# AlejandroSilvestri/os1

Measured on AMD Instinct MI355X. Metric: frames/sec extract+match, 1920x1080 @ 2000 ORB feats, higher is better.
Workload: dtype u8

## Files before the change

include/orbfe.h:

```cpp
#ifndef ORBFE_H_
#define ORBFE_H_

#include <stddef.h>
#include <stdint.h>

#ifdef __cplusplus
extern "C" {
#endif

#define ORBFE_OK 0
#define ORBFE_ERR_INVALID (-1)
#define ORBFE_ERR_NO_DEVICE (-2)
#define ORBFE_ERR_HIP (-3)
#define ORBFE_ERR_TOO_SMALL (-4)
#define ORBFE_ERR_OVERFLOW (-5)

typedef struct OrbfeKeyPoint {
  float x, y;
  float size;
  float angle;
  float response;
  int32_t octave;
  int32_t class_id;
} OrbfeKeyPoint;

typedef struct orbfe_extractor orbfe_extractor;
typedef struct orbfe_matcher orbfe_matcher;
typedef struct orbfe_vocabulary orbfe_vocabulary;
typedef struct orbfe_kfdb orbfe_kfdb;

const char* orbfe_last_error(void);
int orbfe_device_count(void);

int orbfe_device_malloc(int device_id, size_t bytes, void** out);
int orbfe_device_free(int device_id, void* ptr);
int orbfe_device_upload(int device_id, void* dst_device, const void* src_host, size_t bytes);
int orbfe_device_synchronize(int device_id);
int orbfe_host_alloc(size_t bytes, void** out);
int orbfe_host_free(void* ptr);
int orbfe_host_register(void* ptr, size_t bytes);
int orbfe_host_unregister(void* ptr);
int orbfe_device_numa_node(int device_id);
int orbfe_bind_thread_to_device(int device_id);
int orbfe_debug_h2d_rate(int device_id, const void* host, size_t bytes, int reps, double* gb_per_s);


int orbfe_extractor_create(int nfeatures, float scaleFactor, int nlevels, int iniThFAST, int minThFAST,
                           int device_id, orbfe_extractor** out);
void orbfe_extractor_destroy(orbfe_extractor* h);

int orbfe_extractor_levels(const orbfe_extractor* h);
int orbfe_extractor_device(const orbfe_extractor* h);
float orbfe_extractor_scale_factor(const orbfe_extractor* h);
int orbfe_extractor_scale_tables(const orbfe_extractor* h, float* scale, float* inv_scale, float* sigma2,
                                 float* inv_sigma2);
int orbfe_extractor_features_per_level(const orbfe_extractor* h, int32_t* out);
int orbfe_extractor_max_keypoints(const orbfe_extractor* h);
int orbfe_extractor_max_keypoints_for_size(const orbfe_extractor* h, int rows, int cols);

int orbfe_extractor_set_wait_mode(orbfe_extractor* h, int poll_us);

enum { ORBFE_INPUT_GRAY8 = 0, ORBFE_INPUT_RGB8 = 1, ORBFE_INPUT_BGR8 = 2, ORBFE_INPUT_RGBA8 = 3, ORBFE_INPUT_BGRA8 = 4 };
enum { ORBFE_GRAY_Q15 = 0, ORBFE_GRAY_Q14 = 1 };
int orbfe_extractor_set_input_format(orbfe_extractor* h, int format, int gray_variant);

enum { ORBFE_GAUSS_ED = 0, ORBFE_GAUSS_ROUNDED = 1 };
int orbfe_extractor_set_blur_variant(orbfe_extractor* h, int variant);

int orbfe_extract(orbfe_extractor* h, const uint8_t* gray, int rows, int cols, size_t stride_bytes,
                  OrbfeKeyPoint* kps, uint8_t* desc, int cap, int* n_out);

int orbfe_extract_batch(orbfe_extractor* h, int nframes, const uint8_t* const* gray, int in_device_memory,
                        int rows, int cols, size_t stride_bytes, OrbfeKeyPoint* kps, uint8_t* desc, int cap,
                        int* n_out);

int orbfe_extract_batch_submit(orbfe_extractor* h, int nframes, const uint8_t* const* gray, int in_device_memory,
                               int rows, int cols, size_t stride_bytes);
int orbfe_extract_batch_collect(orbfe_extractor* h, OrbfeKeyPoint* kps, uint8_t* desc, int cap, int* n_out);
int orbfe_extract_batch_wait(orbfe_extractor* h);

typedef struct orbfe_sfi_chain orbfe_sfi_chain;
int orbfe_sfi_chain_create(const orbfe_extractor* h, orbfe_sfi_chain** out);
void orbfe_sfi_chain_destroy(orbfe_sfi_chain* c);
int orbfe_sfi_chain_set_isolated(orbfe_sfi_chain* c, int isolated);
int orbfe_sfi_chain_restart(orbfe_sfi_chain* c);
int orbfe_extract_batch_submit_matched(orbfe_extractor* h, orbfe_sfi_chain* chain, int nframes, const uint8_t* const* gray,
                                       int in_device_memory, int rows, int cols, size_t stride_bytes, const float bounds[4],
                                       int window_size, float nnratio, int check_orientation);
int orbfe_extract_batch_collect_matched(orbfe_extractor* h, OrbfeKeyPoint* kps, uint8_t* desc, int cap, int* n_out,
                                        int32_t* matches12, int* nmatches);

int orbfe_debug_level_size(const orbfe_extractor* h, int level, int* w, int* hgt);
int orbfe_debug_level_copy(orbfe_extractor* h, int frame, int level, uint8_t* out );
int orbfe_debug_candidates(orbfe_extractor* h, int frame, int level, int32_t* xys, int cap, int* n_out);
int orbfe_debug_stage_ms(const orbfe_extractor* h, float out[5]);
int orbfe_debug_kernel_ms(orbfe_extractor* h, double out_ms[5], long long* batches, long long* frames, int reset);
int orbfe_debug_set_profiling(orbfe_extractor* h, int enable);
int orbfe_debug_fast_stamps(orbfe_extractor* h, unsigned long long out[8], int reset);
int orbfe_debug_sfi_records(orbfe_extractor* h, int32_t* out, int cap_records, int* n_out, int reset);
int orbfe_debug_sincos(orbfe_extractor* h, const float* angle_deg, int n, float* cos_out, float* sin_out);

int orbfe_debug_quadtree(const int16_t* x, const int16_t* y, const uint8_t* score, int n, int min_x, int max_x,
                         int min_y, int max_y, int n_target, int32_t* out_idx, int cap, int* n_out);
int orbfe_debug_sincos_host_check(uint32_t lo_bits, uint32_t hi_bits, uint32_t step, long long* mismatches);
int orbfe_debug_logf(orbfe_matcher* m, const float* x, int n, float* out);
int orbfe_debug_logf_host_check(uint32_t lo_bits, uint32_t hi_bits, uint32_t step, long long* mismatches);

typedef struct orbfe_stream orbfe_stream;
int orbfe_stream_create(int nfeatures, float scaleFactor, int nlevels, int iniThFAST, int minThFAST, int device_id,
                        int batch, int depth, orbfe_stream** out);
void orbfe_stream_destroy(orbfe_stream* s);
int orbfe_stream_set_matching(orbfe_stream* s, const float bounds[4], int window_size, float nnratio,
                              int check_orientation);
int orbfe_stream_set_isolated_batches(orbfe_stream* s, int isolated);
int orbfe_stream_batches_in_flight(const orbfe_stream* s);
int orbfe_stream_pop_hold(orbfe_stream* s, const OrbfeKeyPoint** kps, const uint8_t** desc, const int** n_kps, const int32_t** matches12,
                          const int** nmatches, int* ticket);
int orbfe_stream_release(orbfe_stream* s, int ticket);
int orbfe_stream_set_input_format(orbfe_stream* s, int format, int gray_variant);
int orbfe_stream_set_blur_variant(orbfe_stream* s, int variant);
int orbfe_stream_set_vocabulary(orbfe_stream* s, orbfe_vocabulary* v, int levelsup);
int orbfe_stream_bow_raw(orbfe_stream* s, int frame, const uint32_t** leaf_node, const uint32_t** level_node, int* n);
int orbfe_stream_capacity(const orbfe_stream* s);
int orbfe_stream_set_queue_slots(orbfe_stream* s, int nslots);
int orbfe_stream_queue_slots(const orbfe_stream* s);
int orbfe_stream_push(orbfe_stream* s, const uint8_t* const* gray, int in_device_memory, int rows, int cols,
                      size_t stride_bytes);
int orbfe_stream_pop(orbfe_stream* s, const OrbfeKeyPoint** kps, const uint8_t** desc, const int** n_kps,
                     const int32_t** matches12, const int** nmatches);
int orbfe_stream_stats(orbfe_stream* s, double out[4], int reset);
int orbfe_stream_kernel_ms(orbfe_stream* s, double out_ms[5], long long* batches, long long* frames, int reset);


int orbfe_hamming(const uint8_t a[32], const uint8_t b[32]);

int orbfe_matcher_create(int device_id, orbfe_matcher** out);
void orbfe_matcher_destroy(orbfe_matcher* m);
int orbfe_matcher_device(const orbfe_matcher* m);
int orbfe_matcher_upload_async(orbfe_matcher* m, void* dst_device, const void* src_host, size_t bytes);
int orbfe_matcher_synchronize(orbfe_matcher* m);

int orbfe_search_for_initialization(orbfe_matcher* m, const OrbfeKeyPoint* kps1, const uint8_t* desc1, int n1,
                                    const OrbfeKeyPoint* kps2, const uint8_t* desc2, int n2,
                                    const float bounds[4], float* prev_xy, int32_t* matches12, int window_size,
                                    float nnratio, int check_orientation, int* nmatches);

int orbfe_search_for_initialization_batch(orbfe_matcher* m, int npairs, const OrbfeKeyPoint* const* kps1,
                                          const uint8_t* const* desc1, const int* n1,
                                          const OrbfeKeyPoint* const* kps2, const uint8_t* const* desc2,
                                          const int* n2, const float bounds[4], float* const* prev_xy,
                                          int32_t* const* matches12, int window_size, float nnratio,
                                          int check_orientation, int* nmatches);

#define ORBFE_MP_IN_VIEW 1u
#define ORBFE_MP_BAD 2u
#define ORBFE_MP_CANDIDATO 4u
#define ORBFE_MP_OBSERVED 8u

int orbfe_search_by_projection(orbfe_matcher* m, const OrbfeKeyPoint* kps_un, const uint8_t* desc, int n,
                               const float bounds[4], const float* scale_factors, int nlevels,
                               const uint8_t* kp_occupied, const float* mp_proj_xy, const int32_t* mp_level,
                               const float* mp_viewcos, const uint8_t* mp_flags, const uint8_t* mp_desc, int n_mp,
                               float th, float nnratio, int32_t* kp_assigned, int* nmatches);

int orbfe_search_by_projection_uv(orbfe_matcher* m, const OrbfeKeyPoint* kps_un, const uint8_t* desc, int n,
                                  const float bounds[4], const float* scale_factors, int nlevels,
                                  const uint8_t* kp_occupied, const float* src_uv, const int32_t* src_level,
                                  const float* src_angle, const uint8_t* src_flags, const uint8_t* src_valid,
                                  const uint8_t* src_desc, int n_src, float th, int max_dist,
                                  int skip_any_occupied, int check_orientation, int32_t* kp_assigned,
                                  int* nmatches);

int orbfe_debug_matcher_ms(const orbfe_matcher* m, double out[3]);

int orbfe_window_candidates(orbfe_matcher* m, const OrbfeKeyPoint* kps_un, const uint8_t* desc, int n,
                            const float bounds[4], int nq, const float* qx, const float* qy, const float* qr,
                            const int32_t* qmin_level, const int32_t* qmax_level, const uint8_t* qdesc,
                            uint32_t* counts, uint32_t* offsets, uint32_t* pool, size_t pool_cap, size_t* pool_used);

int orbfe_search_projected(orbfe_matcher* m, const OrbfeKeyPoint* kps_un, const uint8_t* desc, int n, const float bounds[4],
                           int n_src, const float* src_uv, const float* src_radius, const int32_t* src_level,
                           const uint8_t* src_valid, const uint8_t* src_desc, const uint8_t* kp_skip, int claim,
                           const float* inv_level_sigma2, int nlevels, double chi2, int max_dist, int32_t* best_idx,
                           int32_t* best_dist, int* nmatches);

typedef struct orbfe_frame orbfe_frame;
int orbfe_frame_create(orbfe_matcher* m, const OrbfeKeyPoint* kps_un, const uint8_t* desc, int n, const float bounds[4],
                       orbfe_frame** out);
int orbfe_frame_create_from_extract(orbfe_extractor* h, int frame_index, const float bounds[4], const float* xy_un,
                                    orbfe_frame** out);
void orbfe_frame_destroy(orbfe_frame* f);
int orbfe_frame_size(const orbfe_frame* f);
int orbfe_frame_device(const orbfe_frame* f);
unsigned long long orbfe_resident_epoch(void);
unsigned long long orbfe_resident_invalidate(void);
const uint8_t* orbfe_frame_descriptors_device(orbfe_frame* f);
int orbfe_frame_download(orbfe_frame* f, OrbfeKeyPoint* kps_un, uint8_t* desc, int32_t* grid_order, int32_t* cell_start);

int orbfe_search_by_projection_frame(orbfe_matcher* m, orbfe_frame* f, const float* scale_factors, int nlevels,
                                     const uint8_t* kp_occupied, const float* mp_proj_xy, const int32_t* mp_level,
                                     const float* mp_viewcos, const uint8_t* mp_flags, const uint8_t* mp_desc, int n_mp,
                                     float th, float nnratio, int32_t* kp_assigned, int* nmatches);
int orbfe_search_by_projection_frame_rows(orbfe_matcher* m, orbfe_frame* f, const float* scale_factors, int nlevels,
                                          const uint8_t* kp_occupied, const float* mp_proj_xy, const int32_t* mp_level,
                                          const float* mp_viewcos, const uint8_t* mp_flags, const uint8_t* desc_table_device,
                                          const uint8_t* desc_table_host, const int32_t* mp_desc_row, int n_rows, int n_mp,
                                          float th, float nnratio, int32_t* kp_assigned, int* nmatches);
int orbfe_search_by_projection_uv_frame(orbfe_matcher* m, orbfe_frame* f, const float* scale_factors, int nlevels,
                                        const uint8_t* kp_occupied, const float* src_uv, const int32_t* src_level,
                                        const float* src_angle, const uint8_t* src_flags, const uint8_t* src_valid,
                                        const uint8_t* src_desc, int n_src, float th, int max_dist, int skip_any_occupied,
                                        int check_orientation, int32_t* kp_assigned, int* nmatches);
int orbfe_search_projected_frame(orbfe_matcher* m, orbfe_frame* f, int n_src, const float* src_uv, const float* src_radius,
                                 const int32_t* src_level, const uint8_t* src_valid, const uint8_t* src_desc,
                                 const uint8_t* kp_skip, int claim, const float* inv_level_sigma2, int nlevels, double chi2,
                                 int max_dist, int32_t* best_idx, int32_t* best_dist, int* nmatches);
typedef struct orbfe_local_map orbfe_local_map;
#define ORBFE_MP_SKIP 16u
typedef struct OrbfeCamera {
  float Rcw[9];
  float tcw[3];
  float Ow[3];
  float fx, fy, cx, cy;
  float logScaleFactor;
} OrbfeCamera;
int orbfe_local_map_create(orbfe_matcher* m, int capacity, orbfe_local_map** out);
void orbfe_local_map_destroy(orbfe_local_map* map);
int orbfe_local_map_capacity(const orbfe_local_map* map);
int orbfe_local_map_set_rows(orbfe_local_map* map, int n, const int32_t* rows, const float* pos, const float* normal,
                             const float* min_raw, const float* max_raw, const uint8_t* desc);
int orbfe_project_local_map(orbfe_matcher* m, orbfe_frame* f, orbfe_local_map* map, const OrbfeCamera* cam,
                            float view_cos_limit, const int32_t* rows, const uint8_t* flags, int n_mp, uint8_t* in_view,
                            float* proj_xy, int32_t* level, float* view_cos, int* n_in_view);
int orbfe_search_local_points_frame(orbfe_matcher* m, orbfe_frame* f, orbfe_local_map* map, const OrbfeCamera* cam,
                                    float view_cos_limit, const int32_t* rows, const uint8_t* flags, int n_mp,
                                    const float* scale_factors, int nlevels, const uint8_t* kp_occupied, float th, float nnratio,
                                    uint8_t* in_view, float* proj_xy, int32_t* level, float* view_cos, int32_t* kp_assigned,
                                    int* nmatches, int* n_in_view);
#define ORBFE_SRC_LAST_FRAME 0
#define ORBFE_SRC_KEYFRAME 1
int orbfe_project_sources(orbfe_matcher* m, orbfe_frame* cur_frame, orbfe_frame* src_frame, orbfe_local_map* map,
                          const OrbfeCamera* cam, int mode, const int32_t* rows, const uint8_t* flags, int n_src, uint8_t* valid,
                          float* uv, int32_t* level, int* n_valid);
int orbfe_search_by_projection_sources_frame(orbfe_matcher* m, orbfe_frame* cur_frame, orbfe_frame* src_frame,
                                             orbfe_local_map* map, const OrbfeCamera* cam, int mode, const int32_t* rows,
                                             const uint8_t* flags, int n_src, const float* scale_factors, int nlevels,
                                             const uint8_t* kp_occupied, float th, int max_dist, int check_orientation,
                                             uint8_t* valid, float* uv, int32_t* level, int32_t* kp_assigned, int* nmatches,
                                             int* n_valid);
typedef struct OrbfeKeyFrameProjection {
  float R[9];
  float t[3];
// ... 106 lines not shown
```

os1_amd/api.py:

```python
import ctypes as C
import os
import subprocess

import numpy as np

_HERE = os.path.dirname(os.path.abspath(__file__))
_SO = os.environ.get('ORBFE_LIB') or os.path.join(_HERE, 'liborbfe.so')

KP_DTYPE = np.dtype([('x', 'f4'), ('y', 'f4'), ('size', 'f4'), ('angle', 'f4'), ('response', 'f4'),
                     ('octave', 'i4'), ('class_id', 'i4')])

MP_IN_VIEW, MP_BAD, MP_CANDIDATO, MP_OBSERVED = 1, 2, 4, 8


class OrbfeError(RuntimeError):
    def __init__(self, code, msg):
        super().__init__('orbfe error %d: %s' % (code, msg))
        self.code = code


def lib_path():
    return _SO


# ... 52 lines not shown
    L.orbfe_frame_descriptors_device.restype = vp
    L.orbfe_frame_download.argtypes = [vp, vp, vp, vp, vp]
    L.orbfe_search_by_projection_frame.argtypes = [vp, vp, vp, ci, vp, vp, vp, vp, vp, vp, ci, cf, cf, vp, C.POINTER(ci)]
    L.orbfe_search_by_projection_frame_rows.argtypes = [vp, vp, vp, ci, vp, vp, vp, vp, vp, vp, vp, vp, ci, ci, cf, cf, vp,
                                                        C.POINTER(ci)]
    L.orbfe_matcher_upload_async.argtypes = [vp, vp, vp, C.c_size_t]
    L.orbfe_matcher_synchronize.argtypes = [vp]
    L.orbfe_matcher_device.argtypes = [vp]
    L.orbfe_extractor_device.argtypes = [vp]
    L.orbfe_frame_device.argtypes = [vp]
    L.orbfe_resident_epoch.restype = C.c_ulonglong
    L.orbfe_resident_invalidate.restype = C.c_ulonglong
    L.orbfe_search_by_projection_uv_frame.argtypes = [vp, vp, vp, ci, vp, vp, vp, vp, vp, vp, vp, ci, cf, ci, ci, ci, vp,
                                                      C.POINTER(ci)]
    L.orbfe_search_projected_frame.argtypes = [vp, vp, ci, vp, vp, vp, vp, vp, vp, ci, vp, ci, C.c_double, ci, vp, vp,
                                               C.POINTER(ci)]
    L.orbfe_debug_resolve_rounds.argtypes = [vp]
    L.orbfe_debug_resolve_route.argtypes = [vp]
    L.orbfe_debug_resolve_phases.argtypes = [vp, vp]
    L.orbfe_search_by_projection.argtypes = [vp, vp, vp, ci, vp, vp, ci, vp, vp, vp, vp, vp, vp, ci, cf, cf, vp,
                                             C.POINTER(ci)]
    L.orbfe_search_by_projection_uv.argtypes = [vp, vp, vp, ci, vp, vp, ci, vp, vp, vp, vp, vp, vp, vp, ci, cf, ci,
                                                ci, ci, vp, C.POINTER(ci)]
    L.orbfe_distinctive_descriptors.argtypes = [vp, ci, vp, vp, vp]
    L.orbfe_window_candidates.argtypes = [vp, vp, vp, ci, vp, ci, vp, vp, vp, vp, vp, vp, vp, vp, vp, C.c_size_t,
                                          C.POINTER(C.c_size_t)]
    L.orbfe_undistort_equidistant.argtypes = [vp, ci, cf, cf, cf, cf]
    L.orbfe_undistort_pinhole.argtypes = [vp, ci, cf, cf, cf, cf, vp, ci]
    L.orbfe_compute_image_bounds.argtypes = [ci, ci, ci, cf, cf, cf, cf, vp, ci, vp]
    L.orbfe_search_projected.argtypes = [vp, vp, vp, ci, vp, ci, vp, vp, vp, vp, vp, vp, ci, vp, ci, C.c_double, ci, vp, vp,
                                         C.POINTER(ci)]
    L.orbfe_search_for_triangulation.argtypes = [vp, vp, vp, vp, ci, vp, vp, vp, ci, vp, vp, vp, ci, vp, vp, vp, ci, vp, cf, cf,
                                                 vp, vp, ci, ci, vp, C.POINTER(ci)]
    L.orbfe_extractor_max_keypoints_for_size.argtypes = [vp, ci, ci]
    L.orbfe_extractor_set_vocabulary.argtypes = [vp, vp, ci]
    L.orbfe_extract_bow_raw.argtypes = [vp, ci, vp, vp, ci, C.POINTER(ci)]
    L.orbfe_bow_assemble.argtypes = [vp, vp, vp, ci, vp, vp, C.POINTER(ci), vp, vp, vp, C.POINTER(ci), vp]
    L.orbfe_stream_set_vocabulary.argtypes = [vp, vp, ci]
    L.orbfe_stream_bow_raw.argtypes = [vp, ci, C.POINTER(vp), C.POINTER(vp), C.POINTER(ci)]
    L.orbfe_extract_bow.argtypes = [vp, ci, vp, vp, C.POINTER(ci), vp, vp, vp, C.POINTER(ci), vp, vp]
    L.orbfe_extractor_set_input_format.argtypes = [vp, ci, ci]
    L.orbfe_stream_set_input_format.argtypes = [vp, ci, ci]
    L.orbfe_extractor_set_blur_variant.argtypes = [vp, ci]
    L.orbfe_stream_set_blur_variant.argtypes = [vp, ci]
    L.orbfe_vocabulary_create.argtypes = [ci, ci, ci, ci, ci, vp, ci, C.POINTER(vp)]
    L.orbfe_vocabulary_create_from_image.argtypes = [ci, vp, C.c_size_t, C.POINTER(vp)]
    L.orbfe_vocabulary_destroy.argtypes = [vp]
    L.orbfe_vocabulary_destroy.restype = None
    L.orbfe_vocabulary_info.argtypes = [vp] + [C.POINTER(ci)] * 6
    L.orbfe_bow_transform.argtypes = [vp, vp, ci, ci, ci, vp, vp, C.POINTER(ci), vp, vp, vp, C.POINTER(ci), vp, vp]
    L.orbfe_kfdb_create.argtypes = [ci, ci, ci, ci, ci, C.POINTER(vp)]
    L.orbfe_kfdb_destroy.argtypes = [vp]
    L.orbfe_kfdb_destroy.restype = None
    L.orbfe_kfdb_add.argtypes = [vp, C.c_uint64, vp, vp, ci]
    L.orbfe_kfdb_erase.argtypes = [vp, C.c_uint64]
    L.orbfe_kfdb_clear.argtypes = [vp]
    L.orbfe_kfdb_size.argtypes = [vp, C.POINTER(ci), C.POINTER(ci)]
    L.orbfe_kfdb_query.argtypes = [vp, vp, vp, ci, vp, vp, vp, ci, C.POINTER(ci)]
    L.orbfe_kfdb_score.argtypes = [vp, vp, vp, ci, vp, ci, vp]
    L.orbfe_search_by_bow.argtypes = [vp, vp, vp, vp, ci, vp, vp, vp, ci, vp, vp, vp, ci, vp, vp, vp, ci, cf, ci, ci, vp,
                                      C.POINTER(ci)]
    L.orbfe_search_by_bow_batch.argtypes = [vp, ci, vp, vp, vp, vp, vp, vp, vp, vp, vp, vp, vp, ci, vp, vp, vp, ci, cf, ci, ci, vp, vp]
    L.orbfe_debug_matcher_ms.argtypes = [vp, vp]
    L.orbfe_debug_features_in_area.argtypes = [vp, vp, ci, vp, cf, cf, cf, ci, ci, vp, ci, C.POINTER(ci)]
    L.orbfe_debug_kernel_ms.argtypes = [vp, vp, C.POINTER(C.c_longlong), C.POINTER(C.c_longlong), ci]
    L.orbfe_debug_set_profiling.argtypes = [vp, ci]
    L.orbfe_device_malloc.argtypes = [ci, C.c_size_t, C.POINTER(vp)]
    L.orbfe_device_free.argtypes = [ci, vp]
    L.orbfe_device_upload.argtypes = [ci, vp, vp, C.c_size_t]
    L.orbfe_host_alloc.argtypes = [C.c_size_t, C.POINTER(vp)]
    L.orbfe_host_free.argtypes = [vp]
    L.orbfe_host_register.argtypes = [vp, C.c_size_t]
    L.orbfe_host_unregister.argtypes = [vp]
    L.orbfe_device_synchronize.argtypes = [ci]
    L.orbfe_device_numa_node.argtypes = [ci]
    L.orbfe_bind_thread_to_device.argtypes = [ci]
    L.orbfe_debug_h2d_rate.argtypes = [ci, vp, C.c_size_t, ci, C.POINTER(C.c_double)]
    L.orbfe_stream_create.argtypes = [ci, cf, ci, ci, ci, ci, ci, ci, C.POINTER(vp)]
    L.orbfe_stream_destroy.argtypes = [vp]
    L.orbfe_stream_destroy.restype = None
    L.orbfe_stream_set_matching.argtypes = [vp, vp, ci, cf, ci]
    L.orbfe_stream_capacity.argtypes = [vp]
    L.orbfe_stream_set_queue_slots.argtypes = [vp, ci]
    L.orbfe_stream_queue_slots.argtypes = [vp]
    L.orbfe_stream_push.argtypes = [vp, vp, ci, ci, ci, C.c_size_t]
    L.orbfe_stream_pop.argtypes = [vp, C.POINTER(vp), C.POINTER(vp), C.POINTER(vp), C.POINTER(vp), C.POINTER(vp)]
    L.orbfe_stream_pop_hold.argtypes = [vp, C.POINTER(vp), C.POINTER(vp), C.POINTER(vp), C.POINTER(vp), C.POINTER(vp), C.POINTER(ci)]
    L.orbfe_stream_release.argtypes = [vp, ci]
    L.orbfe_stream_set_isolated_batches.argtypes = [vp, ci]
    L.orbfe_stream_batches_in_flight.argtypes = [vp]
    L.orbfe_stream_multi_create.argtypes = [ci, cf, ci, ci, ci, C.POINTER(ci), ci, ci, ci, C.POINTER(vp)]
    L.orbfe_stream_multi_destroy.argtypes = [vp]
    L.orbfe_stream_multi_destroy.restype = None
    L.orbfe_stream_multi_devices.argtypes = [vp]
    L.orbfe_stream_multi_capacity.argtypes = [vp]
    L.orbfe_stream_multi_device_of_next_push.argtypes = [vp]
    L.orbfe_stream_multi_set_matching.argtypes = [vp, vp, ci, cf, ci]
    L.orbfe_stream_multi_set_blur_variant.argtypes = [vp, ci]
    L.orbfe_stream_multi_push.argtypes = [vp, vp, ci, ci, ci, C.c_size_t]
    L.orbfe_stream_multi_pop.argtypes = [vp, C.POINTER(vp), C.POINTER(vp), C.POINTER(vp), C.POINTER(vp), C.POINTER(vp)]
    L.orbfe_stream_stats.argtypes = [vp, vp, ci]
    L.orbfe_stream_kernel_ms.argtypes = [vp, vp, C.POINTER(C.c_longlong), C.POINTER(C.c_longlong), ci]
    L.orbfe_debug_quadtree.argtypes = [vp, vp, vp, ci, ci, ci, ci, ci, ci, vp, ci, C.POINTER(ci)]
    L.orbfe_debug_sincos_host_check.argtypes = [C.c_uint32, C.c_uint32, C.c_uint32, C.POINTER(C.c_longlong)]
    L.orbfe_debug_logf.argtypes = [vp, vp, ci, vp]
    L.orbfe_debug_logf_host_check.argtypes = [C.c_uint32, C.c_uint32, C.c_uint32, C.POINTER(C.c_longlong)]
    L.orbfe_local_map_create.argtypes = [vp, ci, C.POINTER(vp)]
    L.orbfe_local_map_destroy.argtypes = [vp]
    L.orbfe_local_map_destroy.restype = None
    L.orbfe_local_map_capacity.argtypes = [vp]
    L.orbfe_local_map_set_rows.argtypes = [vp, ci, vp, vp, vp, vp, vp, vp]
    L.orbfe_project_local_map.argtypes = [vp, vp, vp, vp, cf, vp, vp, ci, vp, vp, vp, vp, C.POINTER(ci)]
    L.orbfe_search_local_points_frame.argtypes = [vp, vp, vp, vp, cf, vp, vp, ci, vp, ci, vp, cf, cf, vp, vp, vp, vp, vp,
                                                  C.POINTER(ci), C.POINTER(ci)]
    L.orbfe_project_sources.argtypes = [vp, vp, vp, vp, vp, ci, vp, vp, ci, vp, vp, vp, C.POINTER(ci)]
    L.orbfe_search_by_projection_sources_frame.argtypes = [vp, vp, vp, vp, vp, ci, vp, vp, ci, vp, ci, vp, cf, ci, ci, vp, vp, vp,
                                                           vp, C.POINTER(ci), C.POINTER(ci)]
    L.orbfe_project_keyframe.argtypes = [vp, vp, vp, vp, vp, vp, ci, vp, ci, cf, vp, vp, vp, vp, C.POINTER(ci)]
    L.orbfe_search_projected_keyframe_frame.argtypes = [vp, vp, vp, vp, vp, vp, ci, vp, ci, cf, vp, ci, vp, C.c_double, ci, vp, vp,
                                                        vp, vp, vp, C.POINTER(ci), C.POINTER(ci)]
    _lib = L
    return L


def _p(a):
    return a.ctypes.data_as(C.c_void_p)


class DeviceRows:

    def __init__(self, ptr, n):
        self.ptr, self.n = int(ptr), int(n)

    def __len__(self):
        return self.n


def _rows(a):
    if isinstance(a, DeviceRows):
        return C.c_void_p(a.ptr), a
    a = np.ascontiguousarray(a, np.uint8)
    return _p(a), a


def _check(rc):
    if rc != 0:
        raise OrbfeError(rc, load_library().orbfe_last_error().decode('utf-8', 'replace'))


def device_count():
    return load_library().orbfe_device_count()


def hamming(a, b):
    a = np.ascontiguousarray(a, np.uint8)
    b = np.ascontiguousarray(b, np.uint8)
    return load_library().orbfe_hamming(_p(a), _p(b))


class Extractor:

    def __init__(self, nfeatures=1000, scale=1.2, nlevels=8, ini_th=20, min_th=7, device=0):
        self.L = load_library()
        h = C.c_void_p()
        _check(self.L.orbfe_extractor_create(nfeatures, scale, nlevels, ini_th, min_th, device, C.byref(h)))
        self.h = h
        self.nlevels = nlevels
        self.cap = self.L.orbfe_extractor_max_keypoints(h)

    def close(self):
        if getattr(self, 'h', None):
            self.L.orbfe_extractor_destroy(self.h)
            self.h = None

    def __del__(self):
        try:
            self.close()
        except Exception:
            pass

    def tables(self):
        n = self.nlevels
        sf, isf, s2, is2 = (np.zeros(n, np.float32) for _ in range(4))
        nf = np.zeros(n, np.int32)
        _check(self.L.orbfe_extractor_scale_tables(self.h, _p(sf), _p(isf), _p(s2), _p(is2)))
        _check(self.L.orbfe_extractor_features_per_level(self.h, _p(nf)))
        return dict(sf=sf, isf=isf, s2=s2, is2=is2, nfeat=nf)

    def __call__(self, image):
        image = np.asarray(image)
        if image.size == 0:
            n = C.c_int(0)
            _check(self.L.orbfe_extract(self.h, None, 0, 0, 0, None, None, 0, C.byref(n)))
            return np.zeros(0, KP_DTYPE), np.zeros((0, 32), np.uint8)
        assert image.dtype == np.uint8 and image.ndim == 2 and image.strides[1] == 1
        cap = max(self.cap, self.L.orbfe_extractor_max_keypoints_for_size(self.h, image.shape[0], image.shape[1]))
        kps = np.zeros(cap, KP_DTYPE)
        desc = np.zeros((cap, 32), np.uint8)
        n = C.c_int(0)
        _check(self.L.orbfe_extract(self.h, _p(image), image.shape[0], image.shape[1], image.strides[0], _p(kps),
                                    _p(desc), cap, C.byref(n)))
        return kps[:n.value].copy(), desc[:n.value].copy()

    FORMATS = {'gray': 0, 'rgb': 1, 'bgr': 2, 'rgba': 3, 'bgra': 4}

    def set_blur_variant(self, variant):
        _check(self.L.orbfe_extractor_set_blur_variant(self.h, int(variant)))

    def set_input_format(self, fmt='gray', variant=0):
        _check(self.L.orbfe_extractor_set_input_format(self.h, self.FORMATS[fmt], variant))

    def extract_color(self, image):
        image = np.ascontiguousarray(image, np.uint8)
        kps = np.zeros(self.cap, KP_DTYPE)
        desc = np.zeros((self.cap, 32), np.uint8)
        n = C.c_int(0)
        _check(self.L.orbfe_extract(self.h, _p(image), image.shape[0], image.shape[1], image.strides[0], _p(kps),
                                    _p(desc), self.cap, C.byref(n)))
        return kps[:n.value].copy(), desc[:n.value].copy()

    def set_vocabulary(self, voc, levelsup=4):
        self._voc = voc
        _check(self.L.orbfe_extractor_set_vocabulary(self.h, voc.h if voc is not None else None, levelsup))

    def bow(self, frame, n):
        ids = np.zeros(max(n, 1), np.uint32)
        vals = np.zeros(max(n, 1), np.float64)
        fvn = np.zeros(max(n, 1), np.uint32)
        fvo = np.zeros(n + 1, np.uint32)
        fvf = np.zeros(max(n, 1), np.uint32)
        wof = np.zeros(max(n, 1), np.uint32)
        nof = np.zeros(max(n, 1), np.uint32)
        nw, nn = C.c_int(0), C.c_int(0)
        _check(self.L.orbfe_extract_bow(self.h, frame, _p(ids), _p(vals), C.byref(nw), _p(fvn), _p(fvo), _p(fvf), C.byref(nn),
                                        _p(wof), _p(nof)))
        nw, nn = nw.value, nn.value
        return ids[:nw], vals[:nw], (fvn[:nn], fvo[:nn + 1], fvf[:int(fvo[nn])]), wof[:n], nof[:n]

    def extract_batch_ptrs(self, ptrs, rows, cols, stride, on_device, kps=None, desc=None):
        B = len(ptrs)
        arr = (C.c_void_p * B)(*ptrs)
        if kps is None:
            kps = np.zeros((B, self.cap), KP_DTYPE)
        if desc is None:
            desc = np.zeros((B, self.cap, 32), np.uint8)
        n = np.zeros(B, np.int32)
        _check(self.L.orbfe_extract_batch(self.h, B, arr, int(on_device), rows, cols, stride, _p(kps), _p(desc),
                                          int(kps.shape[1]), _p(n)))
        return kps, desc, n

    def submit_ptrs(self, ptrs, rows, cols, stride, on_device):
        B = len(ptrs)
        self._pending = (C.c_void_p * B)(*ptrs)
        self._pendingB = B
        _check(self.L.orbfe_extract_batch_submit(self.h, B, self._pending, int(on_device), rows, cols, stride))

    def wait(self):
        _check(self.L.orbfe_extract_batch_wait(self.h))

    def collect(self, kps=None, desc=None):
        B = self._pendingB
        if kps is None:
            kps = np.zeros((B, self.cap), KP_DTYPE)
        if desc is None:
            desc = np.zeros((B, self.cap, 32), np.uint8)
        n = np.zeros(B, np.int32)
        _check(self.L.orbfe_extract_batch_collect(self.h, _p(kps), _p(desc), self.cap, _p(n)))
        return kps, desc, n

    def extract_batch(self, images):
        images = [np.ascontiguousarray(im, np.uint8) for im in images]
        rows, cols = images[0].shape
        assert all(im.shape == (rows, cols) for im in images)
        kps, desc, n = self.extract_batch_ptrs([im.ctypes.data for im in images], rows, cols, cols, False)
        return [(kps[i, :n[i]].copy(), desc[i, :n[i]].copy()) for i in range(len(images))]

    def level(self, level, frame=0):
        w, h = C.c_int(), C.c_int()
        _check(self.L.orbfe_debug_level_size(self.h, level, C.byref(w), C.byref(h)))
        out = np.zeros((h.value, w.value), np.uint8)
        _check(self.L.orbfe_debug_level_copy(self.h, frame, level, _p(out)))
        return out

    def candidates(self, level, frame=0):
        n = C.c_int(0)
        _check(self.L.orbfe_debug_candidates(self.h, frame, level, None, 0, C.byref(n)))
        out = np.zeros((max(n.value, 1), 3), np.int32)
        _check(self.L.orbfe_debug_candidates(self.h, frame, level, _p(out), n.value, C.byref(n)))
        return out[:n.value].copy()

    def stage_ms(self):
        out = np.zeros(5, np.float32)
        _check(self.L.orbfe_debug_stage_ms(self.h, _p(out)))
        return out

    def kernel_ms(self, reset=False):
        ms = np.zeros(5, np.float64)
        b, f = C.c_longlong(0), C.c_longlong(0)
        _check(self.L.orbfe_debug_kernel_ms(self.h, _p(ms), C.byref(b), C.byref(f), int(reset)))
        return ms, b.value, f.value

    def set_profiling(self, enable=True):
        _check(self.L.orbfe_debug_set_profiling(self.h, int(enable)))

    def sincos(self, angle_deg):
        a = np.ascontiguousarray(angle_deg, np.float32)
# ... 990 lines not shown
```

os1_amd/csrc/orbfe_extractor.hip:

```cpp
#include <hip/hip_runtime.h>
#include <unistd.h>
#include <sched.h>

#include <algorithm>
#include <cctype>
#include <chrono>
#include <cmath>
#include <cstdarg>
#include <cstdio>
#include <cstdlib>
#include <cstring>
#include <memory>
#include <mutex>
#include <string>
#include <thread>
#include <vector>

#include "../../include/orbfe.h"
#include "glibc_sincosf.h"
#include "host_pool.h"
#include "orbfe_internal.h"
#include "quadtree.h"

namespace orbfe {
int launch_pyramid(const PyramidParams& P, int nframes, hipStream_t st, const ConeParams* cone);
void launch_ingest(const uint8_t* src, long long sstride, uint8_t* dst, long long dpitch, int rowBytes, int rows, hipStream_t st);
void launch_to_gray(const uint8_t* const* raw, long long rawStride, const uint8_t* const* gray, long long grayPitch, int rows,
                    int cols, int channels, const int coef[3], int shift, bool aligned, int nframes, hipStream_t st);
void launch_fast(const PyramidParams& P, int nframes, hipStream_t st);
uint32_t fast_cell_geo(int wCell, int hCell);
void launch_compact(const PyramidParams& P, int nframes, hipStream_t st);
void launch_compact_local(const PyramidParams& P, int nframes, hipStream_t st, int level0, int level1);
void launch_describe(const PyramidParams& P, const SelKp* sel, int nsel, float* angle, uint8_t* desc,
                     hipStream_t st);
void launch_sincos(const float* deg, int n, float* c, float* s, hipStream_t st);
void launch_spin(unsigned long long ticks, hipStream_t st);
void launch_describe_slots(const PyramidParams& P, const SelKp* sel, int nslots, float* angle, uint8_t* desc,
                           const uint32_t* selCount, int selPerFrame, const int* selOff, hipStream_t st, bool fourWaves, float* angle2 = nullptr,
                           uint8_t* desc2 = nullptr);
int launch_quadtree(const QtParams& Q, int nframes, hipStream_t st, int ldsBudget);
int bow_launch_descend(orbfe_vocabulary* v, const uint8_t* d_desc, int n, int levelsup, uint2* d_out, hipStream_t st);
int bow_assemble(orbfe_vocabulary* v, const uint2* ln, int n, uint32_t* bow_ids, double* bow_values, int* n_words,
                 uint32_t* fv_nodes, uint32_t* fv_offsets, uint32_t* fv_features, int* n_fv_nodes,
                 uint32_t* word_of_feature, uint32_t* node_of_feature);
int bow_device(const orbfe_vocabulary* v);
void launch_sfi(const SfiParams& S, int nframes, hipStream_t st);
void launch_sfi_carry(const SfiParams& S, int lastFrame, SelKp* cSel, float* cAngle, uint8_t* cDesc, uint32_t* cCount,
                      hipStream_t st);

thread_local std::string g_err;
void set_err(const char* fmt, ...) {
  char buf[512];
  va_list ap;
  va_start(ap, fmt);
  vsnprintf(buf, sizeof buf, fmt, ap);
  va_end(ap);
  g_err = buf;
}
}

using namespace orbfe;

#define HIP_TRY(expr)                                                                        \
  do {                                                                                       \
    hipError_t e_ = (expr);                                                                  \
    if (e_ != hipSuccess) {                                                                  \
      set_err("%s failed: %s (%s:%d)", #expr, hipGetErrorString(e_), __FILE__, __LINE__);    \
      return ORBFE_ERR_HIP;                                                                  \
    }                                                                                        \
  } while (0)

namespace {
inline int cv_round_f(float v) { return (int)lrintf(v); }
inline int cv_floor_f(float v) { int i = (int)v; return i - (i > v); }
inline short sat_short(int v) { return (short)(v < -32768 ? -32768 : v > 32767 ? 32767 : v); }
inline long long align_up(long long v, long long a) { return (v + a - 1) / a * a; }
double now_ms() {
  return std::chrono::duration<double, std::milli>(std::chrono::steady_clock::now().time_since_epoch()).count();
}

template <class T>
struct DevBuf {
  T* p = nullptr;
  size_t n = 0;
  int ensure(size_t count) {
    if (count <= n) return ORBFE_OK;
    if (p) (void)hipFree(p);
    p = nullptr;
    n = 0;
    HIP_TRY(hipMalloc((void**)&p, count * sizeof(T)));
    n = count;
    return ORBFE_OK;
  }
  void release() { if (p) (void)hipFree(p); p = nullptr; n = 0; }
};
template <class T>
struct PinBuf {
  T* p = nullptr;
  size_t n = 0;
  int ensure(size_t count) {
    if (count <= n) return ORBFE_OK;
    if (p) (void)hipHostFree(p);
    p = nullptr;
    n = 0;
    HIP_TRY(hipHostMalloc((void**)&p, count * sizeof(T), hipHostMallocDefault));
    n = count;
    return ORBFE_OK;
  }
  void release() { if (p) (void)hipHostFree(p); p = nullptr; n = 0; }
};
}

struct orbfe_sfi_chain {
  int device = 0, n0cap = 0;
  DevBuf<SelKp> sel[2];
  DevBuf<float> angle[2];
  DevBuf<uint8_t> desc[2];
  DevBuf<uint32_t> count;
  hipEvent_t ready[2] = {};
  long long seq = 0;
  bool isolated = false;
  bool restart = false;
  orbfe_matcher* hostMatcher = nullptr;
  std::vector<OrbfeKeyPoint> hostPrevKps;
  std::vector<uint8_t> hostPrevDesc;
  bool hostPrevValid = false;
  ~orbfe_sfi_chain() {
    (void)hipSetDevice(device);
    if (hostMatcher) orbfe_matcher_destroy(hostMatcher);
    for (int i = 0; i < 2; i++) { sel[i].release(); angle[i].release(); desc[i].release(); if (ready[i]) (void)hipEventDestroy(ready[i]); }
    count.release();
  }
};

struct UploadLane {
  std::mutex mu;
  hipStream_t stream = nullptr;
};
static UploadLane* upload_lane(int device) {
  static std::mutex mu;
  static UploadLane* lanes[64] = {};
  if (device < 0 || device >= 64) return nullptr;
  std::lock_guard<std::mutex> lk(mu);
  if (!lanes[device]) {
    UploadLane* l = new UploadLane;
    if (hipStreamCreateWithFlags(&l->stream, hipStreamNonBlocking) != hipSuccess) { delete l; return nullptr; }
    lanes[device] = l;
  }
  return lanes[device];
}

struct orbfe_extractor {
  int nfeatures, nlevels, iniTh, minTh, device;
  double scaleFactor;
  std::vector<float> sf, isf, sigma2, isigma2;
  std::vector<int> nfeat;
  static constexpr int kMaxSub = 4;
  hipStream_t stream = nullptr;
  hipStream_t streams[kMaxSub] = {};
  static constexpr int subBatches = 4;
  hipEvent_t evUpload = nullptr;
  bool lastLocalCand = false, submitLocalCand = false;
  bool localLists = true;
  hipEvent_t evFrame0 = nullptr, evS1[kMaxSub] = {};
  int subSel[kMaxSub] = {};
  size_t candHostCap = 0;
  bool gpuQuadtree = true;
  orbfe_vocabulary* voc = nullptr;
  int vocLevelsup = 4;
  bool pendingBow = false;
  DevBuf<uint2> d_bow;
  PinBuf<uint2> h_bow;
  std::vector<std::vector<uint2>> bowKp;
  int kpPerFrameCap = 0;
  bool geomGpuQtOk = true;
  QtParams QP{};
  int selOff[kMaxLevels + 1] = {};
  int selPerFrame = 0;
  DevBuf<uint16_t> d_own;
  hipEvent_t evQt[2] = {};
  std::vector<int> frameKpBase, frameKpCount;

  int rows = 0, cols = 0, batchCap = 0;
  PyramidParams P{};
  DevBuf<uint8_t> d_tables, d_slab, d_in;
  DevBuf<ConeRange> d_coneTab, d_coneTailTab;
  ConeParams coneTail{};
  bool tailOk = false;
  int tailBase = 0, tailTile = 48;
  ConeParams cone{};
  bool coneOk = false;
  bool qtJump = true;
  int qtLdsBudget = 120 * 1024;
  int pollWaitUs = 0;
  bool zeroCopyOut = true;
  bool zeroCopyBatches = false;
  bool ingestKernel = true;
  int coneTile = 0;
  int coneMaxFrames = 2;
  DevBuf<FastCell> d_cells;
  DevBuf<uint8_t> d_zeros;
  DevBuf<uint32_t> d_cellCount, d_slots, d_cand;
  DevBuf<const uint8_t*> d_frame0;
  template <class T> struct View { T* p = nullptr; };
  DevBuf<uint8_t> d_outArena;
  PinBuf<uint8_t> h_outArena;
  size_t outArenaBytes = 0;
  View<uint32_t> d_levelStart, d_selCount, h_levelStart, h_selCount;
  View<SelKp> d_sel, h_sel;
  View<float> d_angle, h_angle;
  View<uint8_t> d_desc, h_desc;
  View<int32_t> d_m12, h_m12, d_nm, h_nm;
  DevBuf<uint16_t> d_sfiOrder;
  DevBuf<int> d_sfiOrderCount;
  DevBuf<uint32_t> d_sfiPool, d_sfiPcount;
  bool pendingMatched = false;
  DevBuf<float> d_f32tmp;
  bool profileKernels = false;
  PinBuf<const uint8_t*> h_frame0;
  PinBuf<uint32_t> h_cand;
  long long inPitch = 0;
  int inFormat = ORBFE_INPUT_GRAY8, grayVariant = ORBFE_GRAY_Q15;
  int gaussVariant = ORBFE_GAUSS_ED;
  long long grayPitch = 0;
  DevBuf<uint8_t> d_gray;
  bool inLinear = false;
  int lastFrames = 0;
  int deferredFrames = 0, deferredCap = 0;
  bool deferredMatched = false;
  std::vector<OrbfeKeyPoint> defKps;
  std::vector<uint8_t> defDesc;
  std::vector<int> defN, defNm;
  std::vector<int32_t> defM12;
  bool lastGpuQt = false, lastZeroCopy = false, submitZeroCopy = false;
  bool describe4 = true;
  float stageMs[5] = {0, 0, 0, 0, 0};
  hipEvent_t ev[kMaxSub][6] = {};
  double kernMs[5] = {0, 0, 0, 0, 0};
  long long kernBatches = 0, kernFrames = 0;

  struct Meta { int16_t x, y; uint8_t score, level; };
  struct Worker {
    QuadTree qt;
    std::vector<int16_t> qx, qy;
    std::vector<uint8_t> qs;
    std::vector<int> qsel;
  };
  std::unique_ptr<HostPool> pool;
  int hostThreads = 1;
  std::vector<Worker> workers;
  std::vector<std::vector<Meta>> taskOut;
  std::vector<Meta> meta;

  ~orbfe_extractor() {
    (void)hipSetDevice(device);
    for (auto& st : streams) if (st) (void)hipStreamSynchronize(st);
    d_bow.release(); h_bow.release();
    d_tables.release(); d_coneTab.release(); d_coneTailTab.release(); d_slab.release(); d_in.release(); d_cellCount.release();
    d_sfiOrder.release(); d_sfiOrderCount.release(); d_sfiPool.release(); d_sfiPcount.release();
    d_cells.release(); d_zeros.release(); d_slots.release(); d_cand.release(); d_frame0.release(); d_gray.release(); d_outArena.release(); h_outArena.release();
    d_f32tmp.release();
    h_frame0.release(); h_cand.release();
    for (auto& es : ev) for (auto& e : es) if (e) (void)hipEventDestroy(e);
    for (auto& e : evS1) if (e) (void)hipEventDestroy(e);
    for (auto& e : evQt) if (e) (void)hipEventDestroy(e);
    d_own.release();
    if (evFrame0) (void)hipEventDestroy(evFrame0);
    if (evUpload) (void)hipEventDestroy(evUpload);

    for (auto& st : streams) if (st) (void)hipStreamDestroy(st);
  }

  int setGeometry(int r, int c) {
    if (r == rows && c == cols) return ORBFE_OK;
    if (c > 4095 || r > 4095) {
      set_err("image %dx%d exceeds the 4095-pixel coordinate packing limit", c, r);
      return ORBFE_ERR_INVALID;
    }
    bool qtOk = true;
    int kpSum = 8;
    PyramidParams Q{};
    Q.nlevels = nlevels;
    Q.iniTh = iniTh;
// ... 286 lines not shown
    const size_t lastBytes = stride * (size_t)(r - 1) + c;
    if (nf > 1 && nf <= 64) {
      const uint8_t* lo = gray[f0];
      for (int f = f0 + 1; f < f0 + nf; f++) lo = std::min(lo, gray[f]);
      uint64_t seen = 0;
      bool tile = true;
      for (int f = f0; f < f0 + nf && tile; f++) {
        const size_t d = (size_t)(gray[f] - lo);
        const size_t k = d / frameBytes;
        tile = d % frameBytes == 0 && k < (size_t)nf && !(seen >> k & 1);
        seen |= (uint64_t)1 << k;
      }
      if (tile) {
        uint8_t* base = d_in.p + frameBytes * f0;
        HIP_TRY(hipMemcpyAsync(base, lo, frameBytes * (size_t)(nf - 1) + lastBytes, hipMemcpyHostToDevice, st));
        for (int f = f0; f < f0 + nf; f++) devAt[f] = base + (size_t)(gray[f] - lo);
        return ORBFE_OK;
      }
    }
    for (int f = f0; f < f0 + nf;) {
      int g = f + 1;
      while (g < f0 + nf && gray[g] == gray[g - 1] + frameBytes) g++;
      HIP_TRY(hipMemcpyAsync(d_in.p + frameBytes * f, gray[f], frameBytes * (size_t)(g - f - 1) + lastBytes, hipMemcpyHostToDevice, st));
      for (int k = f; k < g; k++) devAt[k] = d_in.p + frameBytes * k;
      f = g;
    }
    return ORBFE_OK;
  }

  int uploadSlots(int f0, int nf, const uint8_t* const* gray, size_t stride, int r, int c, hipStream_t st) {
    for (int f = f0; f < f0 + nf; f++) {
      if (inLinear)
        HIP_TRY(hipMemcpyAsync(d_in.p + (size_t)inPitch * rows * f, gray[f], stride * (size_t)(r - 1) + c, hipMemcpyHostToDevice, st));
      else
        HIP_TRY(hipMemcpy2DAsync(d_in.p + (size_t)inPitch * rows * f, inPitch, gray[f], stride, c, r, hipMemcpyHostToDevice, st));
    }
    return ORBFE_OK;
  }

  int runGpuQt(int nframes, const uint8_t* const* gray, bool onDevice, int r, int c, size_t stride, OrbfeKeyPoint* kps,
               uint8_t* desc, int cap, int* n_out) {
    int rc = submitGpuQt(nframes, gray, onDevice, r, c, stride);
    if (rc) return rc;
    return waitGpuQt(kps, desc, cap, n_out);
  }

  bool submitProfiled = false, fastTimed = false;
  std::vector<const uint8_t*> devAt;
  int pendingFrames = 0;
  double tSubmit0 = 0, tSubmit1 = 0;

  struct MatchSpec { orbfe_sfi_chain* chain; float bounds[4]; int window; float nnratio; int checkOri; };

  int submitGpuQt(int nframes, const uint8_t* const* gray, bool onDevice, int r, int c, size_t stride,
                  const MatchSpec* ms = nullptr) {
    if (pendingFrames) { set_err("a submitted batch has not been collected yet"); return ORBFE_ERR_INVALID; }
    HIP_TRY(hipSetDevice(device));
    int rc;
    if ((rc = setGeometry(r, c))) return rc;
    if (!geomGpuQtOk) {
      set_err("image %dx%d: a pyramid level has more than 4 (or no) quadtree root nodes; only the blocking "
              "orbfe_extract / orbfe_extract_batch calls (host quadtree path) handle such aspect ratios", c, r);
      return ORBFE_ERR_INVALID;
    }
    if ((rc = setBatch(nframes, !onDevice, stride))) return rc;
    const double t0 = now_ms();
    hipStream_t st = streams[0];
    const int ch = inChannels();
    const int rowBytes = c * ch;
    for (int f = 0; f < nframes; f++)
      if (!gray[f]) { set_err("frame %d is NULL", f); return ORBFE_ERR_INVALID; }
    devAt.resize(nframes);
    bool pinned = !onDevice;
    std::vector<const uint8_t*>& mappedAt = devAt;
    if (!onDevice) {
      const size_t extent = stride * (size_t)(r - 1) + (size_t)rowBytes;
      const int ncheck = nframes <= coneMaxFrames ? nframes : 1;
      for (int f = 0; f < ncheck && pinned; f++) {
        void* dp = nullptr;
        void* dpEnd = nullptr;
        const bool ok = hipHostGetDevicePointer(&dp, const_cast<uint8_t*>(gray[f]), 0) == hipSuccess && dp &&
                        hipHostGetDevicePointer(&dpEnd, const_cast<uint8_t*>(gray[f]) + extent - 1, 0) == hipSuccess &&
                        (const uint8_t*)dpEnd - (const uint8_t*)dp == (ptrdiff_t)(extent - 1);
        if (!ok) { (void)hipGetLastError(); pinned = false; break; }
        mappedAt[f] = static_cast<const uint8_t*>(dp);
      }
    }
    if (!onDevice && !pinned) {
      if ((rc = uploadFrames(0, nframes, gray, stride, r, rowBytes, st, devAt.data()))) return rc;
    } else if (!onDevice && ingestKernel && nframes <= coneMaxFrames &&
               ((((uintptr_t)gray[0] | (uintptr_t)gray[nframes - 1] | (uintptr_t)stride | (uintptr_t)rowBytes) & 3) == 0)) {
      for (int f = 0; f < nframes; f++) {
        uint8_t* d = d_in.p + (size_t)inPitch * rows * f;
        launch_ingest(mappedAt[f], (long long)stride, d, inPitch, rowBytes, r, st);
        devAt[f] = d;
      }
      HIP_TRY(hipGetLastError());
    } else if (!onDevice) {
      UploadLane* lane = upload_lane(device);
      if (!lane) { set_err("cannot create the upload stream"); return ORBFE_ERR_HIP; }
      std::lock_guard<std::mutex> lk(lane->mu);
      if ((rc = uploadFrames(0, nframes, gray, stride, r, rowBytes, lane->stream, devAt.data()))) return rc;
      HIP_TRY(hipEventRecord(evUpload, lane->stream));
      HIP_TRY(hipStreamWaitEvent(st, evUpload, 0));
    }
    bool rawAligned = ((onDevice ? (long long)stride : inPitch) & 3) == 0;
    for (int f = 0; f < nframes; f++) {
      const uint8_t* raw = onDevice ? gray[f] : devAt[f];
      rawAligned = rawAligned && ((uintptr_t)raw & (ch == 4 ? 15 : 3)) == 0;
      h_frame0.p[f] = ch == 1 ? raw : d_gray.p + (size_t)grayPitch * rows * f;
      h_frame0.p[nframes + f] = raw;
    }
    const long long rawStride = onDevice ? (long long)stride : inPitch;
    P.stride0 = ch == 1 ? rawStride : grayPitch;
    P.frameBase = 0;
    P.gaussVariant = gaussVariant;
    if (ch == 1 && nframes <= 2) {
      P.frame0 = nullptr;
      P.frameInline[0] = h_frame0.p[0];
      P.frameInline[1] = h_frame0.p[nframes - 1];
    } else {
      P.frame0 = d_frame0.p;
      HIP_TRY(hipMemcpyAsync(d_frame0.p, h_frame0.p, sizeof(void*) * nframes * (ch == 1 ? 1 : 2), hipMemcpyHostToDevice, st));
    }
    if (ch > 1) {
      const bool q15 = grayVariant == ORBFE_GRAY_Q15;
      const int cr = q15 ? 9798 : 4899, cg = q15 ? 19235 : 9617, cb = q15 ? 3735 : 1868;
      const bool rgb = inFormat == ORBFE_INPUT_RGB8 || inFormat == ORBFE_INPUT_RGBA8;
      const int coef[3] = {rgb ? cr : cb, cg, rgb ? cb : cr};
      launch_to_gray(d_frame0.p + nframes, rawStride, d_frame0.p, grayPitch, r, c, ch, coef, q15 ? 15 : 14, rawAligned, nframes, st);
    }
    const bool prof = profileKernels;
    QP.cand = d_cand.p; QP.levelStart = d_levelStart.p; QP.candCap = P.candCap; QP.nlevels = nlevels; QP.frameBase = 0;
    QP.own = d_own.p;
    QP.sel = d_sel.p; QP.selCount = d_selCount.p; QP.selPerFrame = selPerFrame;
    const bool small = nframes <= coneMaxFrames;
    const bool zeroCopy = zeroCopyOut && small && !voc && !(ms && ms->chain);
    submitZeroCopy = zeroCopy;
    QP.jump = qtJump ? 1 : 0;
    const bool kernelOut = zeroCopyBatches && !small;
    QP.selHost = (zeroCopy || kernelOut) ? h_sel.p : nullptr;
    QP.selCountHost = (zeroCopy || kernelOut) ? h_selCount.p : nullptr;
    for (int l = 0; l < nlevels; l++) {
      QP.levW[l] = P.lv[l].w; QP.levH[l] = P.lv[l].h; QP.nfeat[l] = nfeat[l]; QP.selOff[l] = selOff[l];
      QP.candBase[l] = P.lv[l].slotBase;
    }
    float* angOut = zeroCopy ? h_angle.p : d_angle.p;
    uint8_t* descOut = zeroCopy ? h_desc.p : d_desc.p;
    const int qtLds = small ? qtLdsBudget : 0;
    const bool four = describe4 && small;
    const bool localCand = small && localLists;
    submitLocalCand = localCand;
    QP.levelLocal = localCand ? 1 : 0;
    {
      if (prof) HIP_TRY(hipEventRecord(ev[0][0], st));
      if (launch_pyramid(P, nframes, st, coneOk && small ? &cone : (tailOk && !small ? &coneTail : nullptr))) { set_err("cannot configure the pyramid kernel"); return ORBFE_ERR_HIP; }
      const bool timeFast = prof || !small;
      fastTimed = timeFast;
      if (timeFast) HIP_TRY(hipEventRecord(ev[0][1], st));
      launch_fast(P, nframes, st);
      if (timeFast) HIP_TRY(hipEventRecord(ev[0][2], st));
      if (localCand) launch_compact_local(P, nframes, st, 0, nlevels);
      else launch_compact(P, nframes, st);
      if (prof) HIP_TRY(hipEventRecord(ev[0][3], st));
      if (prof) HIP_TRY(hipEventRecord(evQt[0], st));
      if (launch_quadtree(QP, nframes, st, qtLds)) { set_err("cannot configure the quadtree kernel"); return ORBFE_ERR_HIP; }
      if (prof) HIP_TRY(hipEventRecord(evQt[1], st));
      if (prof) HIP_TRY(hipEventRecord(ev[0][4], st));
      launch_describe_slots(P, d_sel.p, nframes * selPerFrame, angOut, descOut, d_selCount.p, selPerFrame, selOff, st, four,
                            kernelOut ? h_angle.p : nullptr, kernelOut ? h_desc.p : nullptr);
      if (prof) HIP_TRY(hipEventRecord(ev[0][5], st));
      HIP_TRY(hipGetLastError());
    }
    const int nslots = nframes * selPerFrame;
    pendingBow = false;
    if (voc) {
      if ((rc = d_bow.ensure(nslots)) || (rc = h_bow.ensure(nslots))) return rc;
      if ((rc = bow_launch_descend(voc, d_desc.p, nslots, vocLevelsup, d_bow.p, st))) return rc;
      HIP_TRY(hipMemcpyAsync(h_bow.p, d_bow.p, sizeof(uint2) * nslots, hipMemcpyDeviceToHost, st));
      pendingBow = true;
    }
    pendingMatched = false;
    if (ms && ms->chain) {
      orbfe_sfi_chain& ch = *ms->chain;
      const int n0cap = selOff[1] - selOff[0];
      if (ch.n0cap != n0cap || ch.device != device) { set_err("match chain belongs to a different extractor configuration"); return ORBFE_ERR_INVALID; }
      if ((rc = d_sfiOrder.ensure((size_t)batchCap * n0cap))) return rc;
      if ((rc = d_sfiOrderCount.ensure(batchCap))) return rc;
      if ((rc = d_sfiPool.ensure((size_t)batchCap * n0cap * n0cap))) return rc;
      if ((rc = d_sfiPcount.ensure((size_t)batchCap * n0cap))) return rc;
      SfiParams SP{};
      SP.sel = d_sel.p; SP.angle = d_angle.p; SP.desc = d_desc.p; SP.selCount = d_selCount.p;
      SP.selPerFrame = selPerFrame; SP.n0cap = n0cap; SP.frameBase = 0;
      const int prev = (int)((ch.seq + 1) & 1), cur = (int)(ch.seq & 1);
      SP.carrySel = ch.sel[prev].p; SP.carryAngle = ch.angle[prev].p; SP.carryDesc = ch.desc[prev].p;
      const bool iso = ch.isolated;
      SP.carryCount = ch.count.p + ((ch.seq == 0 || iso || ch.restart) ? 2 : prev);
      ch.restart = false;
      SP.minX = ms->bounds[0]; SP.minY = ms->bounds[2];
      SP.invW = static_cast<float>(64) / static_cast<float>(ms->bounds[1] - ms->bounds[0]);
      SP.invH = static_cast<float>(48) / static_cast<float>(ms->bounds[3] - ms->bounds[2]);
      SP.window = (float)ms->window; SP.nnratio = ms->nnratio; SP.checkOri = ms->checkOri;
      SP.order = d_sfiOrder.p; SP.orderCount = d_sfiOrderCount.p; SP.pool = d_sfiPool.p; SP.pcount = d_sfiPcount.p;
      SP.matches12 = kernelOut ? h_m12.p : d_m12.p; SP.nmatches = kernelOut ? h_nm.p : d_nm.p;
      if (ch.seq > 0 && !iso) HIP_TRY(hipStreamWaitEvent(st, ch.ready[prev], 0));
      launch_sfi(SP, nframes, st);
      HIP_TRY(hipGetLastError());
      if (!iso) {
        launch_sfi_carry(SP, nframes - 1, ch.sel[cur].p, ch.angle[cur].p, ch.desc[cur].p, ch.count.p + cur, st);
        HIP_TRY(hipGetLastError());
        HIP_TRY(hipEventRecord(ch.ready[cur], st));
      }
      ch.seq++;
      pendingMatched = true;
    }
    if (!zeroCopy && !kernelOut) HIP_TRY(hipMemcpyAsync(h_outArena.p, d_outArena.p, outArenaBytes, hipMemcpyDeviceToHost, st));
    submitProfiled = prof;
    tSubmit0 = t0;
    tSubmit1 = now_ms();
    pendingFrames = nframes;
    return ORBFE_OK;
  }

  int waitOnly() {
    if (!pendingFrames) return ORBFE_OK;
    HIP_TRY(hipSetDevice(device));
    hipStream_t st = streams[0];
    if (pollWaitUs > 0) {
      hipError_t q;
      while ((q = hipStreamQuery(st)) == hipErrorNotReady) usleep((useconds_t)pollWaitUs);
      if (q != hipSuccess) HIP_TRY(q);
    }
    HIP_TRY(hipStreamSynchronize(st));
    return ORBFE_OK;
  }

  int waitGpuQt(OrbfeKeyPoint* kps, uint8_t* desc, int cap, int* n_out, int32_t* matches12 = nullptr,
                int* nmatches = nullptr) {
    if (!pendingFrames) { set_err("no submitted batch to collect"); return ORBFE_ERR_INVALID; }
    HIP_TRY(hipSetDevice(device));
    const int nframes = pendingFrames;
    pendingFrames = 0;
    hipStream_t st = streams[0];
    const double t0 = tSubmit0, t1 = tSubmit1;
    const double t1b = now_ms();
    if (pollWaitUs > 0) {
      hipError_t q;
      while ((q = hipStreamQuery(st)) == hipErrorNotReady) usleep((useconds_t)pollWaitUs);
      if (q != hipSuccess) HIP_TRY(q);
    }
    HIP_TRY(hipStreamSynchronize(st));
    const double t2 = now_ms();
    {
      float ms = 0;
      if (fastTimed && hipEventElapsedTime(&ms, ev[0][1], ev[0][2]) == hipSuccess) kernMs[1] += ms;
      if (submitProfiled) {
        if (hipEventElapsedTime(&ms, ev[0][0], ev[0][1]) == hipSuccess) kernMs[0] += ms;
        if (hipEventElapsedTime(&ms, ev[0][2], ev[0][3]) == hipSuccess) kernMs[2] += ms;
        if (hipEventElapsedTime(&ms, ev[0][4], ev[0][5]) == hipSuccess) kernMs[3] += ms;
        if (hipEventElapsedTime(&ms, evQt[0], evQt[1]) == hipSuccess) kernMs[4] += ms;
      }
      if (fastTimed) {
        kernBatches++;
        kernFrames += nframes;
      }
    }
    int status = ORBFE_OK;
    if (pendingBow) bowKp.resize(nframes);
    else bowKp.clear();
    for (int f = 0; f < nframes; f++) {
      OrbfeKeyPoint* ko = kps + (size_t)f * cap;
      uint8_t* dout = desc + (size_t)f * cap * 32;
      if (pendingBow) bowKp[f].clear();
      int n = 0;
      for (int l = 0; l < nlevels; l++) {
        const int cnt = (int)h_selCount.p[(size_t)f * kMaxLevels + l];
        const size_t base = (size_t)f * selPerFrame + selOff[l];
        const float scale = sf[l];
        const float size = (float)(int)(31 * sf[l]);
        for (int i = 0; i < cnt; i++) {
          if (n >= cap) { n++; continue; }
          const SelKp s = h_sel.p[base + i];
          OrbfeKeyPoint kp;
          kp.x = (float)(s.xy & 0xffff);
          kp.y = (float)(s.xy >> 16);
          if (l != 0) { kp.x *= scale; kp.y *= scale; }
          kp.size = size;
          kp.angle = h_angle.p[base + i];
          kp.response = (float)(s.lf >> 24);
          kp.octave = l;
          kp.class_id = -1;
          ko[n] = kp;
          memcpy(dout + (size_t)n * 32, h_desc.p + (base + i) * 32, 32);
          if (pendingBow) bowKp[f].push_back(h_bow.p[base + i]);
          n++;
        }
      }
      n_out[f] = n;
      if (n > cap) {
        set_err("frame %d produced %d keypoints, cap is %d", f, n, cap);
        status = ORBFE_ERR_OVERFLOW;
      }
    }
    if (matches12 && nmatches) {
      const int n0cap = selOff[1] - selOff[0];
      for (int f = 0; f < nframes; f++) {
        int32_t* row = matches12 + (size_t)f * cap;
        const int m = std::min(cap, n0cap);
        if (pendingMatched) {
          memcpy(row, h_m12.p + (size_t)f * n0cap, sizeof(int32_t) * m);
          nmatches[f] = h_nm.p[f];
        } else {
          nmatches[f] = 0;
        }
        for (int i = pendingMatched ? m : 0; i < cap; i++) row[i] = -1;
      }
    }
    const double t3 = now_ms();
    stageMs[0] = (float)(t1 - t0);
    stageMs[1] = (float)(t2 - t1b);
    stageMs[2] = 0;
    stageMs[3] = (float)(t3 - t2);
    stageMs[4] = (float)(t3 - t0);
    lastFrames = nframes;
    lastGpuQt = true;
    lastZeroCopy = submitZeroCopy;
    lastLocalCand = submitLocalCand;
    return status;
  }

  int run(int nframes, const uint8_t* const* gray, bool onDevice, int r, int c, size_t stride, OrbfeKeyPoint* kps,
          uint8_t* desc, int cap, int* n_out) {
    if (pendingFrames) { set_err("a submitted batch has not been collected yet"); return ORBFE_ERR_INVALID; }
    HIP_TRY(hipSetDevice(device));
    int rc;
    if ((rc = setGeometry(r, c))) return rc;
    if ((rc = setBatch(nframes, !onDevice, stride))) return rc;
    const double t0 = now_ms();
    if (!pool) {
      pool.reset(new HostPool(hostThreads));
      workers.resize(hostThreads);
    }
    if (inChannels() != 1) { set_err("colour input needs the GPU quadtree path (unset ORBFE_HOST_QUADTREE)"); return ORBFE_ERR_INVALID; }
    const int nsub = std::min(nframes, std::min(kMaxSub, std::max(1, subBatches)));
    const int maxKp = kpPerFrameCap;
    if ((rc = ensureSubStreams(nsub))) return rc;
    int subF0[kMaxSub + 1];
    for (int s = 0; s <= nsub; s++) subF0[s] = (int)((long long)nframes * s / nsub);

    devAt.resize(nframes);
    for (int f = 0; f < nframes; f++) {
      if (!gray[f]) { set_err("frame %d is NULL", f); return ORBFE_ERR_INVALID; }
      h_frame0.p[f] = onDevice ? gray[f] : d_in.p + (size_t)inPitch * rows * f;
    }
    P.stride0 = onDevice ? (long long)stride : inPitch;
    P.gaussVariant = gaussVariant;
    P.frame0 = d_frame0.p;
    HIP_TRY(hipMemcpyAsync(d_frame0.p, h_frame0.p, sizeof(void*) * nframes, hipMemcpyHostToDevice, streams[0]));
    HIP_TRY(hipEventRecord(evFrame0, streams[0]));
    for (int s = 0; s < nsub; s++) {
      hipStream_t st = streams[s];
      const int f0 = subF0[s], nf = subF0[s + 1] - f0;
      if (s) HIP_TRY(hipStreamWaitEvent(st, evFrame0, 0));
      if (!onDevice && (rc = uploadSlots(f0, nf, gray, stride, r, c, st))) return rc;
      PyramidParams Q = P;
      Q.frameBase = f0;
// ... 325 lines not shown
  h->batchCap = 0;
  return ORBFE_OK;
}

int orbfe_extractor_create(int nfeatures, float scaleFactor, int nlevels, int iniThFAST, int minThFAST, int device_id,
                           orbfe_extractor** out) {
  if (!out) { set_err("out is NULL"); return ORBFE_ERR_INVALID; }
  *out = nullptr;
  if (nfeatures <= 0 || nlevels < 1 || nlevels > kMaxLevels || !(scaleFactor > 1.0f) || iniThFAST < 1 ||
      minThFAST < 1 || iniThFAST > 255 || minThFAST > 255) {
    set_err("invalid extractor parameters (nfeatures=%d scale=%g nlevels=%d ini=%d min=%d; nlevels<=%d)", nfeatures,
            scaleFactor, nlevels, iniThFAST, minThFAST, kMaxLevels);
    return ORBFE_ERR_INVALID;
  }
  int ndev = 0;
  if (hipGetDeviceCount(&ndev) != hipSuccess || ndev <= 0 || device_id < 0 || device_id >= ndev) {
    set_err("no usable HIP device (count=%d, requested %d): this library has no CPU fallback", ndev, device_id);
    return ORBFE_ERR_NO_DEVICE;
  }
  HIP_TRY(hipSetDevice(device_id));
  orbfe_extractor* h = new orbfe_extractor();
  h->nfeatures = nfeatures;
  h->scaleFactor = scaleFactor;
  h->nlevels = nlevels;
  h->iniTh = iniThFAST;
  h->minTh = minThFAST;
  h->device = device_id;
  h->sf.resize(nlevels);
  h->sigma2.resize(nlevels);
  h->sf[0] = 1.0f;
  h->sigma2[0] = 1.0f;
  for (int i = 1; i < nlevels; i++) {
    h->sf[i] = (float)(h->sf[i - 1] * h->scaleFactor);
    h->sigma2[i] = h->sf[i] * h->sf[i];
  }
  h->isf.resize(nlevels);
  h->isigma2.resize(nlevels);
  for (int i = 0; i < nlevels; i++) {
    h->isf[i] = 1.0f / h->sf[i];
    h->isigma2[i] = 1.0f / h->sigma2[i];
  }
  h->nfeat.resize(nlevels);
  const float factor = (float)(1.0f / h->scaleFactor);
  float nDesired = nfeatures * (1 - factor) / (1 - (float)pow((double)factor, (double)nlevels));
  int sum = 0;
  for (int l = 0; l < nlevels - 1; l++) {
    h->nfeat[l] = cv_round_f(nDesired);
    sum += h->nfeat[l];
    nDesired *= factor;
  }
  h->nfeat[nlevels - 1] = nfeatures - sum > 0 ? nfeatures - sum : 0;
  {
    hipError_t e = hipStreamCreateWithFlags(&h->streams[0], hipStreamNonBlocking);
    if (e != hipSuccess) {
      set_err("hipStreamCreate failed: %s", hipGetErrorString(e));
      delete h;
      return ORBFE_ERR_HIP;
    }
  }
  h->stream = h->streams[0];
  bool evOk = hipEventCreate(&h->evFrame0) == hipSuccess &&
              hipEventCreateWithFlags(&h->evUpload, hipEventDisableTiming) == hipSuccess;
  for (auto& e : h->evS1) evOk = evOk && hipEventCreateWithFlags(&e, hipEventDisableTiming) == hipSuccess;
  for (auto& es : h->ev) for (auto& e : es) evOk = evOk && hipEventCreate(&e) == hipSuccess;
  if (!evOk) { set_err("hipEventCreate failed"); delete h; return ORBFE_ERR_HIP; }
  for (auto& e : h->evQt) evOk = evOk && hipEventCreate(&e) == hipSuccess;
  if (!evOk) { set_err("hipEventCreate failed"); delete h; return ORBFE_ERR_HIP; }
  if (const char* hv = getenv("ORBFE_HOST_QUADTREE")) h->gpuQuadtree = atoi(hv) == 0;
  if (const char* cv = getenv("ORBFE_CONE_MAX_FRAMES")) h->coneMaxFrames = atoi(cv);
  if (const char* pv = getenv("ORBFE_POLL_WAIT_US")) h->pollWaitUs = atoi(pv);
  if (const char* dw = ORBFE_EXP_ENV("ORBFE_DESCRIBE_WAVES")) h->describe4 = atoi(dw) != 1;
  if (const char* zv = getenv("ORBFE_ZERO_COPY")) { h->zeroCopyOut = atoi(zv) != 0; h->zeroCopyBatches = atoi(zv) == 2; }
  if (const char* iv = getenv("ORBFE_INGEST_KERNEL")) h->ingestKernel = atoi(iv) != 0;
  if (const char* gv = ORBFE_EXP_ENV("ORBFE_LOCAL_LISTS")) h->localLists = atoi(gv) != 0;
  if (const char* qv = getenv("ORBFE_QT_LDS_BYTES")) h->qtLdsBudget = atoi(qv);
  if (const char* qj = getenv("ORBFE_QT_JUMP")) h->qtJump = atoi(qj) != 0;
  if (const char* tb = ORBFE_EXP_ENV("ORBFE_TAIL_CONE_BASE")) h->tailBase = atoi(tb);
  if (const char* tt = ORBFE_EXP_ENV("ORBFE_TAIL_CONE_TILE")) h->tailTile = std::max(8, atoi(tt)) & ~3;
  if (const char* cv = ORBFE_EXP_ENV("ORBFE_CONE_TILE")) h->coneTile = atoi(cv) <= 0 ? 0 : std::max(8, atoi(cv));
  if (const char* pv = ORBFE_EXP_ENV("ORBFE_PROFILE_KERNELS")) h->profileKernels = atoi(pv) != 0;
  if (const char* gv = getenv("ORBFE_GAUSS_VARIANT")) h->gaussVariant = atoi(gv) == ORBFE_GAUSS_ROUNDED ? ORBFE_GAUSS_ROUNDED : ORBFE_GAUSS_ED;
  h->selPerFrame = 0;
  for (int l = 0; l < nlevels; l++) {
    h->selOff[l] = h->selPerFrame;
    h->selPerFrame += std::max(h->nfeat[l] + 4, 16);
    if (h->nfeat[l] + 4 > kQtNodeCap) h->gpuQuadtree = false;
  }
  h->selOff[nlevels] = h->selPerFrame;
  int nthreads = (int)std::thread::hardware_concurrency();
  if (nthreads > 16) nthreads = 16;
  if (const char* ev = getenv("ORBFE_HOST_THREADS")) nthreads = atoi(ev);
  if (nthreads < 1) nthreads = 1;
  h->hostThreads = nthreads;
  *out = h;
  return ORBFE_OK;
}

void orbfe_extractor_destroy(orbfe_extractor* h) { delete h; }
int orbfe_extractor_levels(const orbfe_extractor* h) { return h ? h->nlevels : 0; }
int orbfe_extractor_device(const orbfe_extractor* h) { return h ? h->device : -1; }

extern "C++" int orbfe_concurrent_streams(orbfe_extractor* const* hs, int n) {
  if (!hs || n < 1) return ORBFE_ERR_INVALID;
  HIP_TRY(hipSetDevice(hs[0]->device));
  constexpr unsigned long long kTicks = 20000;
  for (int i = 0; i < n; i++) launch_spin(100, hs[i]->streams[0]);
  for (int i = 0; i < n; i++) HIP_TRY(hipStreamSynchronize(hs[i]->streams[0]));
  auto overlap = [&](int k, bool& yes) -> int {
    double best = 1e30;
    for (int rep = 0; rep < 3 && best >= 0.2 * 1.6; rep++) {
      const double t0 = now_ms();
      for (int i = 0; i < k; i++) launch_spin(kTicks, hs[i]->streams[0]);
      HIP_TRY(hipGetLastError());
      for (int i = 0; i < k; i++) HIP_TRY(hipStreamSynchronize(hs[i]->streams[0]));
      best = std::min(best, now_ms() - t0);
    }
    yes = best < 0.2 * 1.6;
    return ORBFE_OK;
  };
  int k = 1;
  while (k < n) {
    bool yes = false;
    int rc = overlap(k + 1, yes);
    if (rc) return rc;
    for (int attempt = 0; !yes && attempt < 6; attempt++) {
      orbfe_extractor* h = hs[k];
      hipStream_t fresh = nullptr;
      HIP_TRY(hipStreamCreateWithFlags(&fresh, hipStreamNonBlocking));
      HIP_TRY(hipStreamSynchronize(h->streams[0]));
      (void)hipStreamDestroy(h->streams[0]);
      h->streams[0] = fresh;
      h->stream = fresh;
      launch_spin(100, fresh);
      HIP_TRY(hipStreamSynchronize(fresh));
      if ((rc = overlap(k + 1, yes))) return rc;
    }
    if (!yes) break;
    k++;
  }
  return k;
}
extern "C++" { namespace orbfe { int fast_stamps(unsigned long long out[8], int reset); } }
int orbfe_debug_fast_stamps(orbfe_extractor* h, unsigned long long out[8], int reset) {
  if (!h || !out) { set_err("NULL argument"); return ORBFE_ERR_INVALID; }
  HIP_TRY(hipSetDevice(h->device));
  HIP_TRY(hipDeviceSynchronize());
#ifndef ORBFE_EXPERIMENTS
  set_err("orbfe_debug_fast_stamps needs a library built with make EXPERIMENTS=1");
  return ORBFE_ERR_INVALID;
#endif
  if (orbfe::fast_stamps(out, reset)) { set_err("reading the stamp counters failed"); return ORBFE_ERR_HIP; }
  return ORBFE_OK;
}
extern "C++" { namespace orbfe { int sfi_debug_read(int* out, int capRecords, int reset); } }
int orbfe_debug_sfi_records(orbfe_extractor* h, int32_t* out, int cap_records, int* n_out, int reset) {
  if (!h || !out || !n_out || cap_records < 0) { set_err("NULL argument"); return ORBFE_ERR_INVALID; }
  HIP_TRY(hipSetDevice(h->device));
  HIP_TRY(hipDeviceSynchronize());
  const int n = orbfe::sfi_debug_read(out, cap_records, reset);
  if (n < 0) { set_err("reading the SearchForInitialization records failed"); return ORBFE_ERR_HIP; }
  *n_out = n;
  return ORBFE_OK;
}
float orbfe_extractor_scale_factor(const orbfe_extractor* h) { return h ? (float)h->scaleFactor : 0.f; }
int orbfe_extractor_scale_tables(const orbfe_extractor* h, float* a, float* b, float* c, float* d) {
  if (!h) { set_err("handle is NULL"); return ORBFE_ERR_INVALID; }
  for (int i = 0; i < h->nlevels; i++) {
    if (a) a[i] = h->sf[i];
    if (b) b[i] = h->isf[i];
    if (c) c[i] = h->sigma2[i];
    if (d) d[i] = h->isigma2[i];
  }
  return ORBFE_OK;
}
int orbfe_extractor_features_per_level(const orbfe_extractor* h, int32_t* out) {
  if (!h || !out) { set_err("NULL argument"); return ORBFE_ERR_INVALID; }
  for (int i = 0; i < h->nlevels; i++) out[i] = h->nfeat[i];
  return ORBFE_OK;
}
int orbfe_extractor_max_keypoints(const orbfe_extractor* h) {
  if (!h) return 0;
  int n = 0;
  for (int l = 0; l < h->nlevels; l++) n += std::max(h->nfeat[l] + 2, 16);
  return n;
}

int orbfe_extractor_set_vocabulary(orbfe_extractor* h, orbfe_vocabulary* v, int levelsup) {
  if (!h) { set_err("extractor is NULL"); return ORBFE_ERR_INVALID; }
  if (h->pendingFrames) { set_err("a submitted batch has not been collected yet"); return ORBFE_ERR_INVALID; }
  if (v && bow_device(v) != h->device) { set_err("vocabulary lives on device %d, extractor on %d", bow_device(v), h->device); return ORBFE_ERR_INVALID; }
  if (v && !h->gpuQuadtree) { set_err("the fused bag-of-words path needs the GPU quadtree path"); return ORBFE_ERR_INVALID; }
  h->voc = v;
  h->vocLevelsup = levelsup;
  return ORBFE_OK;
}

int orbfe_extract_bow(orbfe_extractor* h, int frame, uint32_t* bow_ids, double* bow_values, int* n_words, uint32_t* fv_nodes,
                      uint32_t* fv_offsets, uint32_t* fv_features, int* n_fv_nodes, uint32_t* word_of_feature,
                      uint32_t* node_of_feature) {
  if (!h || !bow_ids || !bow_values || !n_words || !fv_nodes || !fv_offsets || !fv_features || !n_fv_nodes) {
    set_err("bad argument");
    return ORBFE_ERR_INVALID;
  }
  if (!h->voc || frame < 0 || frame >= (int)h->bowKp.size()) {
    set_err("no bag-of-words result for frame %d (set a vocabulary before extracting)", frame);
    return ORBFE_ERR_INVALID;
  }
  const std::vector<uint2>& ln = h->bowKp[frame];
  return bow_assemble(h->voc, ln.data(), (int)ln.size(), bow_ids, bow_values, n_words, fv_nodes, fv_offsets, fv_features,
                      n_fv_nodes, word_of_feature, node_of_feature);
}

int orbfe_extract_bow_raw(orbfe_extractor* h, int frame, uint32_t* leaf_node, uint32_t* level_node, int cap, int* n_out) {
  if (!h || !leaf_node || !level_node || !n_out || cap < 0) { set_err("bad argument"); return ORBFE_ERR_INVALID; }
  if (!h->voc || frame < 0 || frame >= (int)h->bowKp.size()) {
    set_err("no bag-of-words result for frame %d (set a vocabulary before extracting)", frame);
    return ORBFE_ERR_INVALID;
  }
  const std::vector<uint2>& ln = h->bowKp[frame];
  *n_out = (int)ln.size();
  const int m = std::min(cap, (int)ln.size());
  for (int i = 0; i < m; i++) { leaf_node[i] = ln[i].x; level_node[i] = ln[i].y; }
  return ORBFE_OK;
}

int orbfe_extractor_max_keypoints_for_size(const orbfe_extractor* h, int rows, int cols) {
  if (!h || rows <= 0 || cols <= 0) return 0;
  int n = 0;
  for (int l = 0; l < h->nlevels; l++) {
    const int w = cv_round_f((float)cols * h->isf[l]), hh = cv_round_f((float)rows * h->isf[l]);
    int roots = hh > 2 * kBorder ? (int)roundf(static_cast<float>(w - 2 * kBorder) / (hh - 2 * kBorder)) : 0;
    if (roots < 0) roots = 0;
    n += std::max(h->nfeat[l] + 2, 4 * roots);
  }
  return n;
}

int orbfe_extract_batch(orbfe_extractor* h, int nframes, const uint8_t* const* gray, int in_device_memory, int rows,
                        int cols, size_t stride_bytes, OrbfeKeyPoint* kps, uint8_t* desc, int cap, int* n_out) {
  if (!h || !n_out) { set_err("NULL argument"); return ORBFE_ERR_INVALID; }
  if (nframes <= 0) return ORBFE_OK;
  for (int f = 0; f < nframes; f++) n_out[f] = 0;
  if (rows == 0 || cols == 0 || !gray) return ORBFE_OK;
  if (rows < 0 || cols < 0 || stride_bytes < (size_t)cols * h->inChannels() || !kps || !desc || cap <= 0) {
    set_err("invalid image / output arguments");
    return ORBFE_ERR_INVALID;
  }
  if (h->pendingFrames) { set_err("a submitted batch has not been collected yet"); return ORBFE_ERR_INVALID; }
  {
    HIP_TRY(hipSetDevice(h->device));
    const int rc = h->setGeometry(rows, cols);
    if (rc) return rc;
  }
  if (h->gpuQuadtree && h->geomGpuQtOk)
    return h->runGpuQt(nframes, gray, in_device_memory != 0, rows, cols, stride_bytes, kps, desc, cap, n_out);
  return h->run(nframes, gray, in_device_memory != 0, rows, cols, stride_bytes, kps, desc, cap, n_out);
}

static bool gpu_route_ok(orbfe_extractor* h, int rows, int cols, int* rc) {
  *rc = ORBFE_OK;
  if (!h->gpuQuadtree) return false;
  if (hipSetDevice(h->device) != hipSuccess) { set_err("hipSetDevice failed"); *rc = ORBFE_ERR_HIP; return false; }
  if (h->pendingFrames || h->deferredFrames) return true;
  *rc = h->setGeometry(rows, cols);
  return *rc == ORBFE_OK && h->geomGpuQtOk;
}

static int deferred_extract(orbfe_extractor* h, int nframes, const uint8_t* const* gray, int in_device_memory, int rows, int cols,
                            size_t stride_bytes) {
  if (h->pendingFrames || h->deferredFrames) { set_err("a submitted batch has not been collected yet"); return ORBFE_ERR_INVALID; }
  const int cap = orbfe_extractor_max_keypoints_for_size(h, rows, cols);
  h->deferredCap = cap;
  h->defKps.resize((size_t)nframes * cap);
  h->defDesc.resize((size_t)nframes * cap * 32);
  h->defN.assign(nframes, 0);
  const int rc = orbfe_extract_batch(h, nframes, gray, in_device_memory, rows, cols, stride_bytes, h->defKps.data(), h->defDesc.data(),
                                     cap, h->defN.data());
  if (rc) return rc;
  h->deferredFrames = nframes;
  h->deferredMatched = false;
  return ORBFE_OK;
}

static int deferred_collect(orbfe_extractor* h, OrbfeKeyPoint* kps, uint8_t* desc, int cap, int* n_out, int32_t* matches12,
                            int* nmatches) {
  const int nframes = h->deferredFrames, dcap = h->deferredCap;
  h->deferredFrames = 0;
  int status = ORBFE_OK;
  for (int f = 0; f < nframes; f++) {
    const int n = h->defN[f];
    n_out[f] = n;
    if (n > cap) { set_err("frame %d produced %d keypoints, cap is %d", f, n, cap); status = ORBFE_ERR_OVERFLOW; }
    const int m = std::min(n, cap);
    memcpy(kps + (size_t)f * cap, h->defKps.data() + (size_t)f * dcap, sizeof(OrbfeKeyPoint) * (size_t)m);
    memcpy(desc + (size_t)f * cap * 32, h->defDesc.data() + (size_t)f * dcap * 32, 32 * (size_t)m);
    if (matches12 && nmatches) {
      int32_t* row = matches12 + (size_t)f * cap;
      for (int i = 0; i < cap; i++) row[i] = -1;
      nmatches[f] = 0;
      if (h->deferredMatched) {
        memcpy(row, h->defM12.data() + (size_t)f * dcap, sizeof(int32_t) * (size_t)std::min(cap, dcap));
        nmatches[f] = h->defNm[f];
      }
    }
  }
  return status;
}

int orbfe_extract_batch_submit(orbfe_extractor* h, int nframes, const uint8_t* const* gray, int in_device_memory,
                               int rows, int cols, size_t stride_bytes) {
  if (!h || !gray || nframes <= 0 || rows <= 0 || cols <= 0 || stride_bytes < (size_t)cols * h->inChannels()) {
    set_err("invalid arguments");
    return ORBFE_ERR_INVALID;
  }
  int rc;
  if (!gpu_route_ok(h, rows, cols, &rc)) {
    if (rc) return rc;
    return deferred_extract(h, nframes, gray, in_device_memory, rows, cols, stride_bytes);
  }
  if (h->deferredFrames) { set_err("a submitted batch has not been collected yet"); return ORBFE_ERR_INVALID; }
  return h->submitGpuQt(nframes, gray, in_device_memory != 0, rows, cols, stride_bytes);
}

int orbfe_extract_batch_wait(orbfe_extractor* h) {
  if (!h) { set_err("invalid arguments"); return ORBFE_ERR_INVALID; }
  if (h->deferredFrames) return ORBFE_OK;
  return h->waitOnly();
}

int orbfe_extract_batch_collect(orbfe_extractor* h, OrbfeKeyPoint* kps, uint8_t* desc, int cap, int* n_out) {
  if (!h || !kps || !desc || !n_out || cap <= 0) { set_err("invalid arguments"); return ORBFE_ERR_INVALID; }
  if (h->deferredFrames) return deferred_collect(h, kps, desc, cap, n_out, nullptr, nullptr);
  return h->waitGpuQt(kps, desc, cap, n_out);
}

int orbfe_sfi_chain_create(const orbfe_extractor* h, orbfe_sfi_chain** out) {
  if (!h || !out) { set_err("NULL argument"); return ORBFE_ERR_INVALID; }
  *out = nullptr;
  HIP_TRY(hipSetDevice(h->device));
  orbfe_sfi_chain* c = new orbfe_sfi_chain();
  c->device = h->device;
  c->n0cap = h->selOff[1] - h->selOff[0];
  int rc = ORBFE_OK;
  for (int i = 0; i < 2 && rc == ORBFE_OK; i++) {
    if ((rc = c->sel[i].ensure(c->n0cap))) break;
    if ((rc = c->angle[i].ensure(c->n0cap))) break;
    if ((rc = c->desc[i].ensure((size_t)c->n0cap * 32))) break;
    if (hipEventCreateWithFlags(&c->ready[i], hipEventDisableTiming) != hipSuccess) { set_err("hipEventCreate failed"); rc = ORBFE_ERR_HIP; }
  }
  if (rc == ORBFE_OK) rc = c->count.ensure(4);
  if (rc == ORBFE_OK) {
    const uint32_t init[4] = {0xffffffffu, 0xffffffffu, 0xffffffffu, 0xffffffffu};
    if (hipMemcpy(c->count.p, init, sizeof init, hipMemcpyHostToDevice) != hipSuccess) { set_err("hipMemcpy failed"); rc = ORBFE_ERR_HIP; }
  }
  if (rc != ORBFE_OK) { delete c; return rc; }
  *out = c;
  return ORBFE_OK;
}

void orbfe_sfi_chain_destroy(orbfe_sfi_chain* c) { delete c; }

int orbfe_sfi_chain_set_isolated(orbfe_sfi_chain* c, int isolated) {
  if (!c) { set_err("chain is NULL"); return ORBFE_ERR_INVALID; }
  if (c->isolated != (isolated != 0)) {
    c->seq = 0;
    c->hostPrevValid = false;
  }
  c->isolated = isolated != 0;
  return ORBFE_OK;
}

int orbfe_sfi_chain_restart(orbfe_sfi_chain* c) {
  if (!c) { set_err("chain is NULL"); return ORBFE_ERR_INVALID; }
  c->restart = true;
  return ORBFE_OK;
}

int orbfe_extract_batch_submit_matched(orbfe_extractor* h, orbfe_sfi_chain* chain, int nframes, const uint8_t* const* gray,
                                       int in_device_memory, int rows, int cols, size_t stride_bytes, const float bounds[4],
                                       int window_size, float nnratio, int check_orientation) {
  if (!h || !chain || !gray || !bounds || nframes <= 0 || rows <= 0 || cols <= 0 || stride_bytes < (size_t)cols * h->inChannels() || window_size <= 0) {
    set_err("invalid arguments");
    return ORBFE_ERR_INVALID;
  }
  int rc;
  if (!gpu_route_ok(h, rows, cols, &rc)) {
    if (rc) return rc;
    if ((rc = deferred_extract(h, nframes, gray, in_device_memory, rows, cols, stride_bytes))) return rc;
    if (!chain->hostMatcher && (rc = orbfe_matcher_create(h->device, &chain->hostMatcher))) { h->deferredFrames = 0; return rc; }
    const int cap = h->deferredCap;
    h->defM12.assign((size_t)nframes * cap, -1);
    h->defNm.assign(nframes, 0);
    std::vector<const OrbfeKeyPoint*> k1, k2;
    std::vector<const uint8_t*> d1, d2;
    std::vector<int> n1, n2, frameOf, nm;
    std::vector<std::vector<float>> pxy;
    std::vector<float*> prev;
    std::vector<int32_t*> m12;
    for (int f = 0; f < nframes; f++) {
      const OrbfeKeyPoint* pk;
      const uint8_t* pd;
      int pn;
      if (f == 0) {
        if (!chain->hostPrevValid || chain->isolated || chain->restart) continue;
        pk = chain->hostPrevKps.data(); pd = chain->hostPrevDesc.data(); pn = (int)chain->hostPrevKps.size();
      } else {
        pk = h->defKps.data() + (size_t)(f - 1) * cap; pd = h->defDesc.data() + (size_t)(f - 1) * cap * 32; pn = h->defN[f - 1];
      }
      pxy.emplace_back((size_t)std::max(pn, 1) * 2);
      for (int j = 0; j < pn; j++) { pxy.back()[2 * j] = pk[j].x; pxy.back()[2 * j + 1] = pk[j].y; }
      k1.push_back(pk); d1.push_back(pd); n1.push_back(pn);
      k2.push_back(h->defKps.data() + (size_t)f * cap); d2.push_back(h->defDesc.data() + (size_t)f * cap * 32); n2.push_back(h->defN[f]);
      m12.push_back(h->defM12.data() + (size_t)f * cap);
      frameOf.push_back(f);
    }
    for (auto& v : pxy) prev.push_back(v.data());
    nm.assign(k1.size(), 0);
    if (!k1.empty()) {
      rc = orbfe_search_for_initialization_batch(chain->hostMatcher, (int)k1.size(), k1.data(), d1.data(), n1.data(), k2.data(), d2.data(),
                                                 n2.data(), bounds, prev.data(), m12.data(), window_size, nnratio, check_orientation,
                                                 nm.data());
      if (rc) { h->deferredFrames = 0; return rc; }
      for (size_t p = 0; p < frameOf.size(); p++) h->defNm[frameOf[p]] = nm[p];
    }
    const int last = nframes - 1, ln = h->defN[last];
    chain->hostPrevKps.assign(h->defKps.begin() + (size_t)last * cap, h->defKps.begin() + (size_t)last * cap + ln);
    chain->hostPrevDesc.assign(h->defDesc.begin() + (size_t)last * cap * 32, h->defDesc.begin() + ((size_t)last * cap + ln) * 32);
    chain->hostPrevValid = !chain->isolated;
    chain->restart = false;
    h->deferredMatched = true;
    return ORBFE_OK;
  }
  if (h->deferredFrames) { set_err("a submitted batch has not been collected yet"); return ORBFE_ERR_INVALID; }
  orbfe_extractor::MatchSpec ms;
  ms.chain = chain;
  memcpy(ms.bounds, bounds, sizeof ms.bounds);
  ms.window = window_size;
  ms.nnratio = nnratio;
  ms.checkOri = check_orientation;
  return h->submitGpuQt(nframes, gray, in_device_memory != 0, rows, cols, stride_bytes, &ms);
}

int orbfe_extract_batch_collect_matched(orbfe_extractor* h, OrbfeKeyPoint* kps, uint8_t* desc, int cap, int* n_out,
                                        int32_t* matches12, int* nmatches) {
  if (!h || !kps || !desc || !n_out || !matches12 || !nmatches || cap <= 0) { set_err("invalid arguments"); return ORBFE_ERR_INVALID; }
  if (h->deferredFrames) return deferred_collect(h, kps, desc, cap, n_out, matches12, nmatches);
  return h->waitGpuQt(kps, desc, cap, n_out, matches12, nmatches);
}

int orbfe_extract(orbfe_extractor* h, const uint8_t* gray, int rows, int cols, size_t stride_bytes, OrbfeKeyPoint* kps,
                  uint8_t* desc, int cap, int* n_out) {
  if (!n_out) { set_err("n_out is NULL"); return ORBFE_ERR_INVALID; }
  *n_out = 0;
  if (!gray || rows == 0 || cols == 0) return ORBFE_OK;
  const uint8_t* frames[1] = {gray};
  return orbfe_extract_batch(h, 1, frames, 0, rows, cols, stride_bytes, kps, desc, cap, n_out);
}

int orbfe_debug_level_size(const orbfe_extractor* h, int level, int* w, int* hgt) {
  if (!h || level < 0 || level >= h->nlevels || h->rows == 0) { set_err("bad level / no frame yet"); return ORBFE_ERR_INVALID; }
  *w = h->P.lv[level].w;
  *hgt = h->P.lv[level].h;
  return ORBFE_OK;
}

int orbfe_debug_level_copy(orbfe_extractor* h, int frame, int level, uint8_t* out) {
  if (!h || level < 0 || level >= h->nlevels || frame < 0 || frame >= h->lastFrames) {
    set_err("bad frame/level");
    return ORBFE_ERR_INVALID;
  }
  HIP_TRY(hipSetDevice(h->device));
  const LevelGeom& L = h->P.lv[level];
  const uint8_t* src;
  size_t pitch;
  if (level == 0) {
    src = h->h_frame0.p[frame];
    pitch = (size_t)h->P.stride0;
  } else {
    src = h->d_slab.p + (size_t)h->P.slabBytes * frame + L.off;
    pitch = L.pitch;
  }
  HIP_TRY(hipMemcpy2D(out, L.w, src, pitch, L.w, L.h, hipMemcpyDeviceToHost));
  return ORBFE_OK;
}

int orbfe_debug_candidates(orbfe_extractor* h, int frame, int level, int32_t* xys, int cap, int* n_out) {
  if (!h || !n_out || level < 0 || level >= h->nlevels || frame < 0 || frame >= h->lastFrames) {
    set_err("bad frame/level");
    return ORBFE_ERR_INVALID;
  }
  HIP_TRY(hipSetDevice(h->device));
  uint32_t ls[kMaxLevels + 1];
  HIP_TRY(hipMemcpy(ls, h->d_levelStart.p + (size_t)frame * (kMaxLevels + 1), sizeof(ls), hipMemcpyDeviceToHost));
  const size_t start = h->lastLocalCand ? (size_t)h->P.lv[level].slotBase : (size_t)ls[level];
  const int n = h->lastLocalCand ? (int)ls[level] : (int)(ls[level + 1] - ls[level]);
  *n_out = n;
  if (n <= 0 || !xys) return ORBFE_OK;
  std::vector<uint32_t> tmp(n);
  HIP_TRY(hipMemcpy(tmp.data(), h->d_cand.p + (size_t)h->P.candCap * frame + start, sizeof(uint32_t) * n,
                    hipMemcpyDeviceToHost));
  for (int i = 0; i < n && i < cap; i++) {
    xys[3 * i] = (int)(tmp[i] & 0xfff) - kBorder;
    xys[3 * i + 1] = (int)((tmp[i] >> 12) & 0xfff) - kBorder;
    xys[3 * i + 2] = (int)(tmp[i] >> 24);
  }
// ... 73 lines not shown
```

os1_amd/csrc/orbfe_internal.h:

```cpp
#pragma once
#include <cstddef>
#include <cstdint>

namespace orbfe {

constexpr int kMaxLevels = 12;
constexpr int kEdge = 19;
constexpr int kBorder = 16;
constexpr int kHalfPatch = 15;
constexpr int kBlurRad = 18;
constexpr int kRawRad = kBlurRad + 3;

struct LevelGeom {
  int w, h;
  int pitch;
  long long off;
  int nCols, nRows;
  int wCell, hCell;
  int cellBase;
  int slotCap;
  long long slotBase;
  const int* xofs;
  const short* xalpha;
  const int* yofs;
  const short* ybeta;
  const unsigned* yofc;
  int rzPitch, rzRows;
};

struct FastCell {
  uint16_t ex0, ey0;
  uint8_t ew, pad0;
  uint8_t eh, level;
  uint32_t cell;
  uint32_t slotOff;
  uint32_t roiOff;
  uint32_t pitch;
  uint8_t wCell, hCell;
  uint16_t pad1;
  uint32_t geo;
};
static_assert(sizeof(FastCell) == 32, "one s_load_dwordx8 per FAST wave");

struct PyramidParams {
  LevelGeom lv[kMaxLevels];
  int nlevels;
  int ncells;
  long long slabBytes;
  long long slotsPerFrame;
  long long candCap;
  const uint8_t* const* frame0;
  const uint8_t* frameInline[2];
  long long stride0;
  uint8_t* slab;
  uint32_t* cellCount;
  uint32_t* slots;
  uint32_t* cand;
  uint32_t* levelStart;
  const FastCell* cells;
  const uint8_t* zeros;
  int iniTh, minTh;
  int frameBase;
  int gaussVariant;
  int fastLean;
};

struct ConeRange { int lo, hi; };
struct ConeParams {
  int base, top;
  int tile, tilesX, tilesY;
  int offB, offH, offC, coefLen;
  int ldsBytes;
  const ConeRange* regX;
  const ConeRange* regY;
};

#ifdef ORBFE_EXPERIMENTS
#define ORBFE_EXP_ENV(name) getenv(name)
#else
#define ORBFE_EXP_ENV(name) (static_cast<const char*>(nullptr))
#endif
#ifdef __HIPCC__
__device__ __forceinline__ const uint8_t* level0_of(const PyramidParams& P, int f) {
  const uint8_t* p = P.frame0 ? P.frame0[f] : P.frameInline[f & 1];
  const unsigned long long v = reinterpret_cast<unsigned long long>(p);
  const unsigned lo = __builtin_amdgcn_readfirstlane((unsigned)v), hi = __builtin_amdgcn_readfirstlane((unsigned)(v >> 32));
  return reinterpret_cast<const uint8_t*>(((unsigned long long)hi << 32) | lo);
}
#endif

struct SelKp {
  uint32_t xy;
  uint32_t lf;
};

struct ExtractView {
  const SelKp* sel;
  const float* angle;
  const uint8_t* desc;
  int selOff[kMaxLevels + 1];
  int count[kMaxLevels];
  float sf[kMaxLevels];
  int nlevels, n, device;
  void* stream;
};

struct SfiParams {
  const SelKp* sel;
  const float* angle;
  const uint8_t* desc;
  const uint32_t* selCount;
  int selPerFrame, n0cap, frameBase;
  const SelKp* carrySel;
  const float* carryAngle;
  const uint8_t* carryDesc;
  const uint32_t* carryCount;
  float minX, minY, invW, invH;
  float window, nnratio;
  int checkOri;
  uint16_t* order;
  int* orderCount;
  uint32_t* pool;
  uint32_t* pcount;
  int32_t* matches12;
  int32_t* nmatches;
};

constexpr int kQtNodeCap = 2048;

struct QtParams {
  const uint32_t* cand;
  const uint32_t* levelStart;
  long long candCap;
  int nlevels, frameBase;
  int levW[kMaxLevels], levH[kMaxLevels], nfeat[kMaxLevels];
  int selOff[kMaxLevels];
  int selPerFrame;
  uint16_t* own;
  SelKp* sel;
  uint32_t* selCount;
  SelKp* selHost;
  uint32_t* selCountHost;
  int jump;
  int levelLocal;
  long long candBase[kMaxLevels];
};


}
```

os1_amd/csrc/orbfe_kernels.hip:

```cpp
#include <mutex>
#include <hip/hip_runtime.h>

#include <type_traits>

#include "glibc_sincosf.h"
#include "orbfe_internal.h"

namespace orbfe {

__device__ __forceinline__ int m24(int a, int b) { return __mul24(a, b); }
__device__ __forceinline__ unsigned mulu24(unsigned a, unsigned b) {
  unsigned r;
  asm("v_mul_u32_u24 %0, %1, %2" : "=v"(r) : "v"(a), "v"(b));
  return r;
}

constexpr int kRzTile = 64;

__global__ __launch_bounds__(256) void k_resize(PyramidParams P, int level) {
  extern __shared__ __align__(16) uint8_t rz[];
  const LevelGeom& D = P.lv[level];
  const LevelGeom& S = P.lv[level - 1];
  const int f = P.frameBase + blockIdx.z;
  const int tx0 = blockIdx.x * kRzTile, ty0 = blockIdx.y * kRzTile;
// ... 606 lines not shown
  if (y < 0) a = 360.f - a;
  return a;
}

__device__ __forceinline__ int reflect101(int i, int n) {
  if (i < 0) i = -i;
  if (i >= n) i = 2 * n - 2 - i;
  return i;
}

constexpr int kRawW = 2 * kRawRad + 1;
constexpr int kBlurW = 2 * kBlurRad + 1;
constexpr int kRawP = 48;
constexpr int kHPT = 50;
constexpr int kBPT = 40;

constexpr int kIcCount = 749;
constexpr int kIcItems = 31 * 8;
struct IcW { uint32_t w1, w2, w3, pad; };
struct IcTab { IcW e[256]; };
constexpr IcTab make_ic_tab() {
  IcTab t{};
  const int um[16] = {15, 15, 15, 15, 14, 14, 14, 13, 13, 12, 11, 10, 9, 8, 6, 3};
  for (int r = 0; r < 31; r++) {
    const int v = r - 15, d = um[v < 0 ? -v : v];
    for (int k = 0; k < 8; k++) {
      uint32_t w1 = 0, w2 = 0, w3 = 0;
      for (int j = 0; j < 4; j++) {
        const int u = 4 * k + j - 15;
        if (u >= -d && u <= d) {
          w1 |= 1u << (8 * j);
          w2 |= (uint32_t)(u + 15) << (8 * j);
          w3 |= (uint32_t)(v + 15) << (8 * j);
        }
      }
      t.e[r * 8 + k] = IcW{w1, w2, w3, 0};
    }
  }
  return t;
}
constexpr int ic_count() {
  const IcTab t = make_ic_tab();
  int n = 0;
  for (int i = 0; i < kIcItems; i++)
    for (int j = 0; j < 4; j++) n += (t.e[i].w1 >> (8 * j)) & 1;
  return n;
}
static_assert(ic_count() == kIcCount, "circular patch must have 749 pixels");
__constant__ IcTab c_icTab = make_ic_tab();

constexpr int kDiscR2x4 = 1458;
constexpr bool in_disc(int x, int yb) { return 4 * ((x - kBlurRad) * (x - kBlurRad) + (yb - kBlurRad) * (yb - kBlurRad)) <= kDiscR2x4; }
struct BlurItems { uint16_t h[448]; uint16_t v[320]; int nh, nv; };
constexpr BlurItems make_blur_items() {
  BlurItems t{};
  bool vneed[kBlurW][10] = {};
  for (int x = 0; x < kBlurW; x++)
    for (int yq = 0; yq < 10; yq++)
      for (int j = 0; j < 4; j++)
        if (4 * yq + j < kBlurW && in_disc(x, 4 * yq + j)) vneed[x][yq] = true;
  for (int x = 0; x < kBlurW; x++)
    for (int yq = 0; yq < 10; yq++)
      if (vneed[x][yq]) t.v[t.nv++] = (uint16_t)(x << 4 | yq);
  bool hneed[kRawW][10] = {};
  for (int x = 0; x < kBlurW; x++)
    for (int yb = 0; yb < kBlurW; yb++)
      if (in_disc(x, yb))
        for (int r = yb; r < yb + 7; r++) hneed[r][x >> 2] = true;
  for (int r = 0; r < kRawW; r++)
    for (int g = 0; g < 10; g++)
      if (hneed[r][g]) t.h[t.nh++] = (uint16_t)(r << 4 | g);
  for (int i = t.nh; i < 448; i++) t.h[i] = t.h[0];
  for (int i = t.nv; i < 320; i++) t.v[i] = t.v[0];
  return t;
}
constexpr BlurItems kBlurItemsHost = make_blur_items();
static_assert(kBlurItemsHost.nh == 368 && kBlurItemsHost.nv == 308, "blur item lists: 6 and 5 wave iterations");
struct BlurCodes { uint32_t h[512], v[512]; };
constexpr BlurCodes make_blur_codes() {
  BlurCodes t{};
  const BlurItems b = make_blur_items();
  for (int i = 0; i < 512; i++) {
    const int hc = b.h[i < b.nh ? i : 0], y = hc >> 4, g = hc & 15;
    t.h[i] = (uint32_t)(y * kRawP + 4 * g) | ((uint32_t)((4 * g * kHPT + y) * 2) << 16);
    const int vc = b.v[i < b.nv ? i : 0], x = vc >> 4, yq = vc & 15;
    t.v[i] = (uint32_t)((x * kHPT + 4 * yq) * 2) | ((uint32_t)(x * kBPT + 4 * yq) << 16);
  }
  return t;
}
__constant__ BlurCodes c_blurCodes = make_blur_codes();


template <int GAUSS> constexpr unsigned blur_tap(int t) {
  constexpr unsigned ed[7] = {18, 34, 48, 56, 48, 34, 18}, rounded[7] = {18, 34, 49, 55, 49, 34, 18};
  return GAUSS == 1 ? rounded[t] : ed[t];
}
template <int GAUSS> constexpr unsigned blur_tap_word(int s, int q) {
  unsigned w = 0;
  for (int b = 0; b < 4; b++) {
    const int t = 4 * q + b - s;
    if (t >= 0 && t <= 6) w |= blur_tap<GAUSS>(t) << (8 * b);
  }
  return w;
}

template <int S, int GAUSS>
__device__ __forceinline__ unsigned blur_row_out(const uint32_t (&d)[4]) {
  constexpr unsigned w0 = blur_tap_word<GAUSS>(S, 0), w1 = blur_tap_word<GAUSS>(S, 1), w2 = blur_tap_word<GAUSS>(S, 2), w3 = blur_tap_word<GAUSS>(S, 3);
  unsigned acc = 0u;
  if constexpr (w0 != 0u) acc = __builtin_amdgcn_udot4(d[0], w0, acc, false);
  if constexpr (w1 != 0u) acc = __builtin_amdgcn_udot4(d[1], w1, acc, false);
  if constexpr (w2 != 0u) acc = __builtin_amdgcn_udot4(d[2], w2, acc, false);
  if constexpr (w3 != 0u) acc = __builtin_amdgcn_udot4(d[3], w3, acc, false);
  return acc;
}

__device__ __forceinline__ int wave_sum_i32(int v) {
  v += __builtin_amdgcn_update_dpp(v, v, 0x128, 0xf, 0xf, false);
  v += __builtin_amdgcn_update_dpp(v, v, 0x124, 0xf, 0xf, false);
  v += __builtin_amdgcn_update_dpp(v, v, 0x122, 0xf, 0xf, false);
  v += __builtin_amdgcn_update_dpp(v, v, 0x121, 0xf, 0xf, false);
  return __builtin_amdgcn_readlane(v, 0) + __builtin_amdgcn_readlane(v, 16) + __builtin_amdgcn_readlane(v, 32) +
         __builtin_amdgcn_readlane(v, 48);
}

__device__ __forceinline__ void wave_sum3_i32(int& a, int& b, int& c) {
#define ORBFE_ROR3(n)                                                          \
  "v_add_u32_dpp %0, %0, %0 row_ror:" #n " row_mask:0xf bank_mask:0xf\n\t"     \
  "v_add_u32_dpp %1, %1, %1 row_ror:" #n " row_mask:0xf bank_mask:0xf\n\t"     \
  "v_add_u32_dpp %2, %2, %2 row_ror:" #n " row_mask:0xf bank_mask:0xf\n\t"
  asm volatile("s_nop 1\n\t" ORBFE_ROR3(8) ORBFE_ROR3(4) ORBFE_ROR3(2) ORBFE_ROR3(1) : "+v"(a), "+v"(b), "+v"(c));
#undef ORBFE_ROR3
  a = __builtin_amdgcn_readlane(a, 0) + __builtin_amdgcn_readlane(a, 16) + __builtin_amdgcn_readlane(a, 32) + __builtin_amdgcn_readlane(a, 48);
  b = __builtin_amdgcn_readlane(b, 0) + __builtin_amdgcn_readlane(b, 16) + __builtin_amdgcn_readlane(b, 32) + __builtin_amdgcn_readlane(b, 48);
  c = __builtin_amdgcn_readlane(c, 0) + __builtin_amdgcn_readlane(c, 16) + __builtin_amdgcn_readlane(c, 32) + __builtin_amdgcn_readlane(c, 48);
}

struct SlotInfo {
  const uint32_t* selCount;
  int selPerFrame;
  int selOff[kMaxLevels + 1];
  int nlevels;
};

struct DescribeLevel { int w, h, pitch, pad; long long off, pad2; };
struct DescribeArgs {
  DescribeLevel lv[kMaxLevels];
  const SelKp* sel;
  const uint32_t* selCount;
  float* angleOut;
  uint8_t* descOut;
  float* angleOut2;
  uint8_t* descOut2;
  const uint8_t* const* frame0;
  const uint8_t* frameInline[2];
  long long stride0;
  uint8_t* slab;
  long long slabBytes;
  int nsel, selPerFrame, nlevels, frameBase, dma;
  int selOff[kMaxLevels + 1];
  int gauss;
};

template <int WAVES, int GAUSS>
__global__ __launch_bounds__(64 * WAVES) void k_describe(DescribeArgs A) {
  constexpr int NT = 64 * WAVES;
  constexpr int NIC = (kIcItems + NT - 1) / NT, NH = (kBlurItemsHost.nh + NT - 1) / NT, NV = (kBlurItemsHost.nv + NT - 1) / NT;
  static_assert(NIC * NT <= 256 && NH * NT <= 512 && NV <= NH, "table padding");
  uint32_t icw[NIC][3], bh[NH], bv[NV];
#pragma unroll
  for (int it = 0; it < NIC; it++) {
    const IcW w = c_icTab.e[it * NT + threadIdx.x];
    icw[it][0] = w.w1; icw[it][1] = w.w2; icw[it][2] = w.w3;
  }
#pragma unroll
  for (int it = 0; it < NH; it++) bh[it] = c_blurCodes.h[it * NT + threadIdx.x];
#pragma unroll
  for (int it = 0; it < NV; it++) bv[it] = c_blurCodes.v[it * NT + threadIdx.x];
  __shared__ int icSum[3 * WAVES];
  __shared__ __align__(16) uint8_t raw[kRawW * kRawP + 16];
  __shared__ __align__(16) uint16_t hbT[40 * kHPT];
  static_assert(kBlurW * kBPT <= kRawW * kRawP, "the blurred patch must fit into the raw patch");
  uint8_t* blT = raw;
  asm volatile("" ::"s"(A.sel), "s"(A.selCount), "s"(A.angleOut), "s"(A.descOut), "s"(A.frame0), "s"(A.frameInline[0]), "s"(A.frameInline[1]),
               "s"(A.stride0), "s"(A.slab), "s"(A.slabBytes), "s"(A.nsel), "s"(A.selPerFrame), "s"(A.nlevels), "s"(A.frameBase), "s"(A.dma),
               "s"(A.selOff[1]), "s"(A.selOff[2]), "s"(A.selOff[3]), "s"(A.selOff[4]), "s"(A.selOff[5]), "s"(A.selOff[6]), "s"(A.selOff[7]));
  const int nsel = A.nsel, dma = A.dma;
  const SelKp* sel = A.sel;
  float* angleOut = A.angleOut;
  uint8_t* descOut = A.descOut;
  const int chunk = (nsel + 7) >> 3;
  const int k = (blockIdx.x & 7) * chunk + (blockIdx.x >> 3);
  if (k >= nsel) return;
  const int tid = threadIdx.x, lane = tid & 63, wave = WAVES == 1 ? 0 : __builtin_amdgcn_readfirstlane(tid >> 6);
  typedef uint32_t u32x2 __attribute__((ext_vector_type(2)));
  typedef uint32_t u32x8 __attribute__((ext_vector_type(8)));
  const char __attribute__((address_space(4)))* ka = (const char __attribute__((address_space(4)))*)__builtin_amdgcn_kernarg_segment_ptr();
  int level, f;
  u32x2 sw, fpw = {0u, 0u};
  u32x8 lw;
  auto frame_ptr_words = [&](int fa) -> u32x2 {
    u32x2 r;
    if (A.frame0) {
      r = *reinterpret_cast<const u32x2 __attribute__((address_space(4)))*>(reinterpret_cast<uintptr_t>(A.frame0 + fa));
    } else {
      const unsigned long long v = reinterpret_cast<unsigned long long>((fa & 1) ? A.frameInline[1] : A.frameInline[0]);
      r.x = (uint32_t)v;
      r.y = (uint32_t)(v >> 32);
    }
    return r;
  };
  if (A.selCount) {
    const int fr = k / A.selPerFrame, within = k - fr * A.selPerFrame;
    int l = 0, lbase = 0;
#pragma unroll
    for (int j = 1; j < kMaxLevels; j++) {
      const int o = A.selOff[j];
      if (j < A.nlevels && within >= o) { l = j; lbase = o; }
    }
    level = l;
    f = A.frameBase + fr;
    const uint32_t live = *reinterpret_cast<const uint32_t __attribute__((address_space(4)))*>(
        reinterpret_cast<uintptr_t>(A.selCount + (long long)f * kMaxLevels + l));
    sw = *reinterpret_cast<const u32x2 __attribute__((address_space(4)))*>(reinterpret_cast<uintptr_t>(sel + k));
    fpw = frame_ptr_words(f);
    lw = *reinterpret_cast<const u32x8 __attribute__((address_space(4)))*>(ka + offsetof(DescribeArgs, lv) + 32 * (unsigned)l);
    asm volatile("" ::"s"(sw.x), "s"(live), "s"(fpw.x), "s"(lw[0]));
    if ((uint32_t)(within - lbase) >= live) return;
  } else {
    sw = *reinterpret_cast<const u32x2 __attribute__((address_space(4)))*>(reinterpret_cast<uintptr_t>(sel + k));
    level = (int)(sw.y & 0xffu);
    f = (int)((sw.y >> 8) & 0xffffu);
    fpw = frame_ptr_words(f);
    lw = *reinterpret_cast<const u32x8 __attribute__((address_space(4)))*>(ka + offsetof(DescribeArgs, lv) + 32 * (unsigned)level);
  }
  const int cx = (int)(sw.x & 0xffffu), cy = (int)(sw.x >> 16);
  struct { int w, h; } L = {(int)lw[0], (int)lw[1]};
  const uint8_t* img;
  long long stride;
  if (level == 0) {
    img = reinterpret_cast<const uint8_t*>(((unsigned long long)fpw.y << 32) | fpw.x);
    stride = A.stride0;
  } else {
    img = A.slab + (long long)f * A.slabBytes + (long long)(((unsigned long long)lw[5] << 32) | lw[4]);
    stride = (long long)(int)lw[2];
  }
  int pa = 0;
  const int istr = (int)stride;
  const bool interior = cx >= kRawRad && cy >= kRawRad && cx + kRawRad < L.w && cy + kRawRad < L.h && (stride & 3) == 0;
  if (interior && dma && (level != 0 || cy + kRawRad < L.h - 1)) {
    const uint8_t* rbase = uniform_ptr(img + m24(cy - kRawRad, istr) + (cx - kRawRad));
    pa = (int)(reinterpret_cast<uintptr_t>(rbase) & 3);
    const uint8_t* gb = rbase - pa;
    constexpr int RPI = WAVES == 1 ? 21 : 11, NI = WAVES == 1 ? 3 : 1;
    static_assert(RPI * NI * WAVES >= kRawW && 3 * RPI <= 64 && kRawP == 48, "LDS-DMA patch layout");
    const int lrow = (lane * 171) >> 9, lcol = lane - 3 * lrow;
    const unsigned voff = (unsigned)(m24(lrow, istr) + 16 * lcol);
#pragma unroll
    for (int u = 0; u < NI; u++) {
      const int r = (wave * NI + u) * RPI;
      if (lrow < RPI && r + lrow < kRawW)
        __builtin_amdgcn_global_load_lds((const __attribute__((address_space(1))) void*)(gb + (voff + (unsigned)m24(r, istr))),
                                         (__attribute__((address_space(3))) void*)(raw + r * kRawP), 16, 0, 0);
    }
    asm volatile("s_waitcnt vmcnt(0)" ::: "memory");
  } else if (interior) {
    const uint8_t* rbase = img + m24(cy - kRawRad, istr) + (cx - kRawRad);
    pa = (int)(reinterpret_cast<uintptr_t>(rbase) & 3);
    const int ndw = (pa + kRawW + 3) >> 2;
    constexpr int RS = NT / 16, NL = (kRawW + RS - 1) / RS;
    const int c = tid & 15, r0 = tid >> 4;
    if (c < ndw) {
      const uint8_t* g = rbase - pa + 4 * c + m24(r0, istr);
      uint8_t* l = raw + 4 * c + m24(r0, kRawP);
      const int gstep = RS * istr;
      uint32_t v[NL];
#pragma unroll
      for (int u = 0; u < NL; u++) v[u] = (r0 + RS * u < kRawW) ? *reinterpret_cast<const uint32_t*>(g + u * gstep) : 0u;
#pragma unroll
      for (int u = 0; u < NL; u++)
        if (r0 + RS * u < kRawW) *reinterpret_cast<uint32_t*>(l + u * RS * kRawP) = v[u];
    }
  } else {
    for (int i0 = tid; i0 < kRawW * kRawW; i0 += NT * 8) {
      uint8_t v[8];
#pragma unroll
      for (int u = 0; u < 8; u++) {
        const int i = i0 + u * NT;
        v[u] = 0;
        if (i < kRawW * kRawW) {
          const int y = i / kRawW, x = i - y * kRawW;
          const int gx = reflect101(cx - kRawRad + x, L.w), gy = reflect101(cy - kRawRad + y, L.h);
          v[u] = img[m24(gy, istr) + gx];
        }
      }
#pragma unroll
      for (int u = 0; u < 8; u++) {
        const int i = i0 + u * NT;
        if (i < kRawW * kRawW) {
          const int y = i / kRawW, x = i - y * kRawW;
          raw[y * kRawP + x] = v[u];
        }
      }
    }
  }
  __syncthreads();

  const int sIc = (pa + 6) & 3, qIc = (pa + 6) & ~3;
  int S1 = 0, S2 = 0, S3 = 0;
  const uint8_t* icBase = raw + m24((tid >> 3) + (kRawRad - 15), kRawP) + qIc + 4 * (tid & 7);
#pragma unroll
  for (int it = 0; it < NIC; it++) {
    const uint32_t* rp = reinterpret_cast<const uint32_t*>(icBase + it * (NT / 8) * kRawP);
    const uint32_t e = __builtin_amdgcn_alignbyte(rp[1], rp[0], sIc);
    S1 = (int)__builtin_amdgcn_udot4(e, icw[it][0], (unsigned)S1, false);
    S2 = (int)__builtin_amdgcn_udot4(e, icw[it][1], (unsigned)S2, false);
    S3 = (int)__builtin_amdgcn_udot4(e, icw[it][2], (unsigned)S3, false);
  }
  wave_sum3_i32(S1, S2, S3);
  if (WAVES > 1) {
    if (lane == 0) { icSum[3 * wave] = S1; icSum[3 * wave + 1] = S2; icSum[3 * wave + 2] = S3; }
    __syncthreads();
    S1 = 0; S2 = 0; S3 = 0;
#pragma unroll
    for (int w = 0; w < WAVES; w++) { S1 += icSum[3 * w]; S2 += icSum[3 * w + 1]; S3 += icSum[3 * w + 2]; }
  }
  const int m10 = S2 - 15 * S1, m01 = S3 - 15 * S1;
  const float angle = fast_atan2_deg((float)m01, (float)m10);

  {
    auto hpass = [&](auto paTag) {
      constexpr int PA = decltype(paTag)::value;
#pragma unroll
      for (int it = 0; it < NH; it++) {
        if ((it + 1) * NT > kBlurItemsHost.nh && it * NT + tid >= kBlurItemsHost.nh) break;
        const uint32_t* rp = reinterpret_cast<const uint32_t*>(raw + (bh[it] & 0xffffu));
        const uint32_t d[4] = {rp[0], rp[1], rp[2], rp[3]};
        uint16_t* o = reinterpret_cast<uint16_t*>(reinterpret_cast<uint8_t*>(hbT) + (bh[it] >> 16));
        o[0] = (uint16_t)blur_row_out<PA + 0, GAUSS>(d);
        o[kHPT] = (uint16_t)blur_row_out<PA + 1, GAUSS>(d);
        o[2 * kHPT] = (uint16_t)blur_row_out<PA + 2, GAUSS>(d);
        o[3 * kHPT] = (uint16_t)blur_row_out<PA + 3, GAUSS>(d);
      }
    };
    switch (pa) {
      case 0: hpass(std::integral_constant<int, 0>{}); break;
      case 1: hpass(std::integral_constant<int, 1>{}); break;
      case 2: hpass(std::integral_constant<int, 2>{}); break;
      default: hpass(std::integral_constant<int, 3>{}); break;
    }
  }
  __syncthreads();
  {
    constexpr uint16_t T0 = blur_tap<GAUSS>(0), T1 = blur_tap<GAUSS>(1), T2 = blur_tap<GAUSS>(2), T3 = blur_tap<GAUSS>(3);
    const u16x2 E0 = {T0, T1}, E1 = {T2, T3}, E2 = {T2, T1}, E3 = {T0, 0};
    const u16x2 O0 = {0, T0}, O1 = {T1, T2}, O2 = {T3, T2}, O3 = {T1, T0};
#pragma unroll
    for (int it = 0; it < NV; it++) {
      if ((it + 1) * NT > kBlurItemsHost.nv && it * NT + tid >= kBlurItemsHost.nv) break;
      const uint32_t* cp = reinterpret_cast<const uint32_t*>(reinterpret_cast<const uint8_t*>(hbT) + (bv[it] & 0xffffu));
      u16x2 p[5];
#pragma unroll
      for (int t = 0; t < 5; t++) p[t] = as_u16x2(cp[t]);
      unsigned r4[4];
#pragma unroll
      for (int h = 0; h < 2; h++) {
        unsigned e = 32768u, o = 32768u;
        e = __builtin_amdgcn_udot2(p[h], E0, e, false);     o = __builtin_amdgcn_udot2(p[h], O0, o, false);
        e = __builtin_amdgcn_udot2(p[h + 1], E1, e, false); o = __builtin_amdgcn_udot2(p[h + 1], O1, o, false);
        e = __builtin_amdgcn_udot2(p[h + 2], E2, e, false); o = __builtin_amdgcn_udot2(p[h + 2], O2, o, false);
        e = __builtin_amdgcn_udot2(p[h + 3], E3, e, false); o = __builtin_amdgcn_udot2(p[h + 3], O3, o, false);
        if constexpr (GAUSS == 1) {
          e = e < 0x00ffffffu ? e : 0x00ffffffu;
          o = o < 0x00ffffffu ? o : 0x00ffffffu;
        }
        r4[2 * h] = e;
        r4[2 * h + 1] = o;
      }
      const unsigned packed = __builtin_amdgcn_perm(r4[1], r4[0], 0x0c0c0602u) | __builtin_amdgcn_perm(r4[3], r4[2], 0x06020c0cu);
      *reinterpret_cast<uint32_t*>(blT + (bv[it] >> 16)) = packed;
    }
  }
  __syncthreads();

  const float factorPI = (float)(3.1415926535897932384626433832795 / 180.f);
  float a, b;
  const float rad = __builtin_bit_cast(float, __builtin_amdgcn_readfirstlane(__builtin_bit_cast(int, angle * factorPI)));
  sincosf_glibc(rad, &b, &a);
  const uint8_t* center = blT + kBlurRad * kBPT + kBlurRad;
  typedef float f32x2 __attribute__((ext_vector_type(2)));
  const f32x2 AB = {a, b}, NBA = {-b, a}, kRoundMagic = {12582912.0f, 12582912.0f};
  unsigned long long words[4] = {0ull, 0ull, 0ull, 0ull};
#pragma unroll
  for (int j = 0; j < 4; j++) {
    if (WAVES == 4 && j != wave) continue;
    const int bit = j * 64 + lane;
    const float4 p = *reinterpret_cast<const float4*>(&c_patternF.v[4 * bit]);
    const f32x2 c1 = (f32x2){p.x, p.x} * AB + (f32x2){p.y, p.y} * NBA + kRoundMagic;
    const f32x2 c2 = (f32x2){p.z, p.z} * AB + (f32x2){p.w, p.w} * NBA + kRoundMagic;
    constexpr unsigned K = 0x400000u * (unsigned)kBPT + 0x4B400000u;
    const float c1x = c1.x, c1y = c1.y, c2x = c2.x, c2y = c2.y;
    const int i1 = (int)(__umul24(__float_as_uint(c1x), (unsigned)kBPT) + __float_as_uint(c1y) - K);
    const int i2 = (int)(__umul24(__float_as_uint(c2x), (unsigned)kBPT) + __float_as_uint(c2y) - K);
    const int t0 = center[i1], t1 = center[i2];
    words[j] = __ballot(t0 < t1);
  }
  uint8_t* descOut2 = A.descOut2;
  if (WAVES == 4) {
    if (lane == 0) {
      reinterpret_cast<unsigned long long*>(descOut + (long long)k * 32)[wave] = words[wave];
      if (descOut2) reinterpret_cast<unsigned long long*>(descOut2 + (long long)k * 32)[wave] = words[wave];
    }
  } else if (lane < 4) {
    reinterpret_cast<unsigned long long*>(descOut + (long long)k * 32)[lane] = words[lane];
    if (descOut2) reinterpret_cast<unsigned long long*>(descOut2 + (long long)k * 32)[lane] = words[lane];
  }
  if (tid == 0) {
    angleOut[k] = angle;
    if (A.angleOut2) A.angleOut2[k] = angle;
  }
}

__global__ void k_sincos(const float* deg, int n, float* c, float* s) {
  const int i = blockIdx.x * blockDim.x + threadIdx.x;
  if (i >= n) return;
  const float factorPI = (float)(3.1415926535897932384626433832795 / 180.f);
  sincosf_glibc(deg[i] * factorPI, &s[i], &c[i]);
}

template <int CH>
__global__ void __launch_bounds__(256) k_to_gray(const uint8_t* const* __restrict__ raw, long long rawStride,
                                                 const uint8_t* const* __restrict__ gray, long long grayPitch, int cols,
                                                 int c0, int c1, int c2, int shift, int aligned) {
  const int x = (int)(blockIdx.x * 256 + threadIdx.x) * 4;
  if (x >= cols) return;
  const int y = blockIdx.y, f = blockIdx.z;
  const uint8_t* src = raw[f] + (long long)y * rawStride + (long long)x * CH;
  uint8_t* dst = const_cast<uint8_t*>(gray[f]) + (long long)y * grayPitch + x;
  const int rnd = 1 << (shift - 1);
  if (aligned && x + 4 <= cols) {
    uint32_t w[CH];
    if (CH == 3) {
      const uint32_t* s32 = (const uint32_t*)src;
      w[0] = s32[0]; w[1] = s32[1]; w[2] = s32[2];
    } else {
      const uint4 q = *(const uint4*)src;
      w[0] = q.x; w[1] = q.y; w[2] = q.z; w[CH - 1] = q.w;
    }
    uint32_t out = 0;
#pragma unroll
    for (int i = 0; i < 4; i++) {
      uint32_t a, b, c;
      if (CH == 3) {
        a = (w[(3 * i) >> 2] >> (((3 * i) & 3) * 8)) & 255u;
        b = (w[(3 * i + 1) >> 2] >> (((3 * i + 1) & 3) * 8)) & 255u;
        c = (w[(3 * i + 2) >> 2] >> (((3 * i + 2) & 3) * 8)) & 255u;
      } else {
        a = w[i] & 255u; b = (w[i] >> 8) & 255u; c = (w[i] >> 16) & 255u;
      }
      out |= ((uint32_t)(m24((int)a, c0) + m24((int)b, c1) + m24((int)c, c2) + rnd) >> shift) << (8 * i);
    }
    *(uint32_t*)dst = out;
  } else {
    for (int i = 0; i < 4 && x + i < cols; i++)
      dst[i] = (uint8_t)((m24(src[CH * i], c0) + m24(src[CH * i + 1], c1) + m24(src[CH * i + 2], c2) + rnd) >> shift);
  }
}

void launch_to_gray(const uint8_t* const* raw, long long rawStride, const uint8_t* const* gray, long long grayPitch, int rows,
                    int cols, int channels, const int coef[3], int shift, bool aligned, int nframes, hipStream_t st) {
  dim3 grid((cols + 1023) / 1024, rows, nframes);
  if (channels == 3)
    hipLaunchKernelGGL(k_to_gray<3>, grid, dim3(256), 0, st, raw, rawStride, gray, grayPitch, cols, coef[0], coef[1], coef[2],
                       shift, aligned ? 1 : 0);
  else
    hipLaunchKernelGGL(k_to_gray<4>, grid, dim3(256), 0, st, raw, rawStride, gray, grayPitch, cols, coef[0], coef[1], coef[2],
                       shift, aligned ? 1 : 0);
}

static int lds_dma_enabled() {
  static const int v = [] { const char* e = getenv("ORBFE_LDS_DMA"); return e ? (atoi(e) != 0 ? 1 : 0) : 1; }();
  return v;
}

template <int V, int U>
__global__ __launch_bounds__(256) void k_ingest(const uint8_t* __restrict__ src, long long sstride, uint8_t* __restrict__ dst, long long dpitch,
                                                int rowBytes, int rows) {
  typedef uint32_t u32x4 __attribute__((ext_vector_type(4)));
  typedef typename std::conditional<V == 16, u32x4, typename std::conditional<V == 4, uint32_t, uint8_t>::type>::type T;
  const int perRow = (rowBytes + V - 1) / V;
  const int total = perRow * rows;
  const float rcpRow = 1.0f / (float)perRow;
  const int i0 = blockIdx.x * 256 + threadIdx.x, step = gridDim.x * 256;
  long long so[U], dof[U];
  bool ok[U];
  T v[U];
#pragma unroll
  for (int u = 0; u < U; u++) {
    const int i = i0 + u * step;
    ok[u] = i < total;
    const int ii = ok[u] ? i : 0;
    int yy = (int)(((float)ii + 0.5f) * rcpRow);
    int xx = ii - yy * perRow;
    if (xx < 0) { yy--; xx += perRow; }
    if (xx >= perRow) { yy++; xx -= perRow; }
    so[u] = (long long)yy * sstride + (long long)V * xx;
    dof[u] = (long long)yy * dpitch + (long long)V * xx;
  }
#pragma unroll
  for (int u = 0; u < U; u++)
    if (ok[u]) v[u] = __builtin_nontemporal_load(reinterpret_cast<const T*>(src + so[u]));
#pragma unroll
  for (int u = 0; u < U; u++)
    if (ok[u]) *reinterpret_cast<T*>(dst + dof[u]) = v[u];
}

void launch_ingest(const uint8_t* src, long long sstride, uint8_t* dst, long long dpitch, int rowBytes, int rows, hipStream_t st) {
  const uintptr_t all = (uintptr_t)src | (uintptr_t)dst | (uintptr_t)sstride | (uintptr_t)dpitch | (uintptr_t)rowBytes;
  const int V = (all & 15) == 0 ? 16 : (all & 3) == 0 ? 4 : 1;
  constexpr int U = 4;
  const long long total = (long long)((rowBytes + V - 1) / V) * rows;
  const int blocks = (int)std::max<long long>(1, (total + 256 * U - 1) / (256 * U));
#define ORBFE_INGEST(VV, UU) hipLaunchKernelGGL((k_ingest<VV, UU>), dim3(blocks), dim3(256), 0, st, src, sstride, dst, dpitch, rowBytes, rows)
  if (V == 16) ORBFE_INGEST(16, 4);
  else if (V == 4) ORBFE_INGEST(4, 4);
  else ORBFE_INGEST(1, 4);
#undef ORBFE_INGEST
}

int launch_pyramid(const PyramidParams& P, int nframes, hipStream_t st, const ConeParams* cone) {
  const int last = cone ? cone->base : P.nlevels - 1;
  if (cone) {
    static std::mutex mu;
    static int attrBytes[64] = {};
    int dev = 0;
    if (hipGetDevice(&dev) != hipSuccess || dev < 0 || dev >= 64) return 1;
    std::lock_guard<std::mutex> lk(mu);
    if (cone->ldsBytes > attrBytes[dev]) {
      if (hipFuncSetAttribute(reinterpret_cast<const void*>(k_pyramid_cone), hipFuncAttributeMaxDynamicSharedMemorySize,
                              cone->ldsBytes) != hipSuccess)
        return 1;
      attrBytes[dev] = cone->ldsBytes;
    }
  }
  for (int l = 1; l <= last; l++) {
    dim3 grid((P.lv[l].w + kRzTile - 1) / kRzTile, (P.lv[l].h + kRzTile - 1) / kRzTile, nframes);
    if (P.lv[l].rzPitch <= 96 && P.lv[l].rzRows <= 80 && grid.x >= 2) {
      const int tilesX = (int)grid.x, ntiles = (int)(grid.x * grid.y);
      const unsigned rcp = (unsigned)(0x100000000ull / (unsigned)tilesX) + 1u;
      if ((unsigned long long)ntiles * tilesX < (1ull << 31)) {
        const int dma = lds_dma_enabled();
        ResizeLevel R{};
        R.dw = P.lv[l].w; R.dh = P.lv[l].h; R.dpitch = P.lv[l].pitch;
        R.sw = P.lv[l - 1].w; R.sh = P.lv[l - 1].h;
        R.sstride = l == 1 ? P.stride0 : (long long)P.lv[l - 1].pitch;
        R.doff = P.lv[l].off; R.soff = P.lv[l - 1].off;
        R.xofs = P.lv[l].xofs; R.xalpha = P.lv[l].xalpha; R.yofc = P.lv[l].yofc; R.ybeta = P.lv[l].ybeta;
        R.frame0 = P.frame0; R.frameInline[0] = P.frameInline[0]; R.frameInline[1] = P.frameInline[1];
        R.slab = P.slab; R.slabBytes = P.slabBytes; R.frameBase = P.frameBase; R.fromLevel0 = l == 1;
        hipLaunchKernelGGL((k_resize_fixed<96, 80>), dim3(8 * ((ntiles + 7) / 8), nframes), dim3(256), 0, st, R, tilesX, ntiles, rcp, dma);
        continue;
      }
    }
    hipLaunchKernelGGL(k_resize, grid, dim3(256), (((size_t)P.lv[l].rzPitch * P.lv[l].rzRows + 15) & ~(size_t)15) + (size_t)P.lv[l].rzRows * 64 * 2, st,
                       P, l);
  }
  if (cone)
    hipLaunchKernelGGL(k_pyramid_cone, dim3(cone->tilesX, cone->tilesY, nframes), dim3(kConeThreads), cone->ldsBytes, st, P, *cone);
  return 0;
}

void launch_compact(const PyramidParams& P, int nframes, hipStream_t st) {
  hipLaunchKernelGGL(k_compact, dim3((P.ncells + 63) / 64, nframes), dim3(64), 0, st, P);
}
void launch_compact_local(const PyramidParams& P, int nframes, hipStream_t st, int level0, int level1) {
  if (level1 > P.nlevels) level1 = P.nlevels;
  int maxCells = 0;
  for (int l = level0; l < level1; l++) maxCells = std::max(maxCells, P.lv[l].nCols * P.lv[l].nRows);
  if (maxCells <= 0) return;
  hipLaunchKernelGGL(k_compact_local, dim3((maxCells + 63) / 64, level1 - level0, nframes), dim3(64), 0, st, P, level0);
}

static DescribeArgs describe_args(const PyramidParams& P, const SelKp* sel, int nsel, float* angle, uint8_t* desc) {
  DescribeArgs A{};
  for (int l = 0; l < kMaxLevels; l++) {
    A.lv[l].w = P.lv[l].w; A.lv[l].h = P.lv[l].h; A.lv[l].pitch = P.lv[l].pitch; A.lv[l].off = P.lv[l].off;
  }
  A.sel = sel; A.selCount = nullptr; A.angleOut = angle; A.descOut = desc; A.angleOut2 = nullptr; A.descOut2 = nullptr;
  A.frame0 = P.frame0; A.frameInline[0] = P.frameInline[0]; A.frameInline[1] = P.frameInline[1];
  A.stride0 = P.stride0; A.slab = P.slab; A.slabBytes = P.slabBytes;
  A.nsel = nsel; A.selPerFrame = 1; A.nlevels = P.nlevels; A.frameBase = P.frameBase; A.dma = lds_dma_enabled();
  A.gauss = P.gaussVariant;
  return A;
}

void launch_describe(const PyramidParams& P, const SelKp* sel, int nsel, float* angle, uint8_t* desc,
                     hipStream_t st) {
  if (nsel <= 0) return;
  const DescribeArgs A = describe_args(P, sel, nsel, angle, desc);
  if (A.gauss == 1) hipLaunchKernelGGL((k_describe<1, 1>), dim3(8 * ((nsel + 7) / 8)), dim3(64), 0, st, A);
  else hipLaunchKernelGGL((k_describe<1, 0>), dim3(8 * ((nsel + 7) / 8)), dim3(64), 0, st, A);
}

void launch_describe_slots(const PyramidParams& P, const SelKp* sel, int nslots, float* angle, uint8_t* desc,
                           const uint32_t* selCount, int selPerFrame, const int* selOff, hipStream_t st, bool fourWaves, float* angle2,
                           uint8_t* desc2) {
  if (nslots <= 0) return;
  DescribeArgs A = describe_args(P, sel, nslots, angle, desc);
  A.angleOut2 = angle2;
  A.descOut2 = desc2;
  A.selCount = selCount;
  A.selPerFrame = selPerFrame;
  for (int l = 0; l <= P.nlevels; l++) A.selOff[l] = selOff[l];
  const dim3 grid(8 * ((nslots + 7) / 8));
  if (fourWaves) {
    if (A.gauss == 1) hipLaunchKernelGGL((k_describe<4, 1>), grid, dim3(256), 0, st, A);
    else hipLaunchKernelGGL((k_describe<4, 0>), grid, dim3(256), 0, st, A);
  } else {
    if (A.gauss == 1) hipLaunchKernelGGL((k_describe<1, 1>), grid, dim3(64), 0, st, A);
    else hipLaunchKernelGGL((k_describe<1, 0>), grid, dim3(64), 0, st, A);
  }
}

__global__ void k_spin(unsigned long long ticks, unsigned* sink) {
  const unsigned long long t0 = __builtin_amdgcn_s_memrealtime();
  unsigned n = 0;
  while (__builtin_amdgcn_s_memrealtime() - t0 < ticks) { __builtin_amdgcn_s_sleep(32); n++; }
  if (sink && n == 0xffffffffu) *sink = n;
}
void launch_spin(unsigned long long ticks, hipStream_t st) {
  hipLaunchKernelGGL(k_spin, dim3(1), dim3(64), 0, st, ticks, (unsigned*)nullptr);
}

void launch_sincos(const float* deg, int n, float* c, float* s, hipStream_t st) {
  if (n <= 0) return;
  hipLaunchKernelGGL(k_sincos, dim3((n + 255) / 256), dim3(256), 0, st, deg, n, c, s);
}

}

#ifdef ORBFE_EXPERIMENTS
extern "C" int orbfe_exp_cone_stamps(unsigned long long* out ) {
  if (hipDeviceSynchronize() != hipSuccess) return 1;
  return hipMemcpyFromSymbol(out, HIP_SYMBOL(orbfe::g_coneStamps), sizeof(unsigned long long) * 32) == hipSuccess ? 0 : 1;
}
#endif
```

os1_amd/csrc/orbfe_quadtree.hip:

```cpp
#include <mutex>
#include <hip/hip_runtime.h>

#include <cstdlib>

#include "orbfe_internal.h"

namespace orbfe {

constexpr int kQt3Threads = 512;

#ifdef ORBFE_EXPERIMENTS
__device__ unsigned long long g_qtStamps[kMaxLevels][32];
#define QT_STAMP(i)                                                                                         \
  do {                                                                                                      \
    if (threadIdx.x == 0 && blockIdx.y == 0) g_qtStamps[blockIdx.x][i] = __builtin_amdgcn_s_memrealtime(); \
  } while (0)
#else
#define QT_STAMP(i) ((void)0)
#endif
constexpr int kQtEpt = 8;

struct Qt3Node {
  short x0, x1, y0, y1;
  uint32_t size;
  uint32_t seq;
};

template <int CAP>
struct Qt3Shared {
  Qt3Node nodes[2][CAP];
  unsigned short proc[CAP];
  uint32_t ninfo[CAP];
  uint16_t cpos[CAP][4];
  alignas(16) uint32_t cnt[CAP * 4];
  alignas(16) unsigned long long sortKeys[CAP];
  short tproc[CAP];
  int wsumI[kQt3Threads / 64];
  int s_int[4];
};

__device__ __forceinline__ int wave_incl_scan_i(int x) {
  x += __builtin_amdgcn_update_dpp(0, x, 0x111, 0xf, 0xf, true);
  x += __builtin_amdgcn_update_dpp(0, x, 0x112, 0xf, 0xf, true);
  x += __builtin_amdgcn_update_dpp(0, x, 0x114, 0xf, 0xf, true);
  x += __builtin_amdgcn_update_dpp(0, x, 0x118, 0xf, 0xf, true);
  x += __builtin_amdgcn_update_dpp(0, x, 0x142, 0xa, 0xf, false);
  x += __builtin_amdgcn_update_dpp(0, x, 0x143, 0xc, 0xf, false);
  return x;
}

template <int CAP>
__device__ int blockScanInt3(Qt3Shared<CAP>& sh, int v, int& total) {
  const int lane = threadIdx.x & 63, wv = threadIdx.x >> 6;
  const int iv = wave_incl_scan_i(v);
  __syncthreads();
  if (lane == 63) sh.wsumI[wv] = iv;
  __syncthreads();
  int base = 0, tot = 0;
#pragma unroll
  for (int w = 0; w < kQt3Threads / 64; w++) {
    if (w < wv) base += sh.wsumI[w];
    tot += sh.wsumI[w];
  }
  total = tot;
  return base + iv - v;
}

template <int CAP>
__device__ void blockSortDesc3(Qt3Shared<CAP>& sh, int n) {
  int m = 1;
  while (m < n) m <<= 1;
  if (n <= kQt3Threads) {
    const int t = threadIdx.x, i = t & (m - 1), part = t / m, parts = kQt3Threads / m;
    const unsigned long long key = i < n ? sh.sortKeys[i] : 0ull;
    uint32_t* rankAcc = sh.cnt;
    if (t < n) rankAcc[t] = 0u;
    __syncthreads();
    if (i < n) {
      const int per = ((n + parts - 1) / parts + 15) & ~15;
      const int j1 = min(n, (part + 1) * per);
      int rank = 0;
      for (int j0 = part * per; j0 < j1; j0 += 16) {
        ulonglong2 kk[8];
#pragma unroll
        for (int u = 0; u < 8; u++) kk[u] = *reinterpret_cast<const ulonglong2*>(&sh.sortKeys[min(j0 + 2 * u, CAP - 2)]);
#pragma unroll
        for (int u = 0; u < 8; u++) {
          rank += (j0 + 2 * u < j1) && (kk[u].x > key);
          rank += (j0 + 2 * u + 1 < j1) && (kk[u].y > key);
        }
      }
      if (rank) atomicAdd(&rankAcc[i], (uint32_t)rank);
    }
    __syncthreads();
    const int pos = (t < n) ? (int)rankAcc[t] : 0;
    const unsigned long long mine = (t < n) ? sh.sortKeys[t] : 0ull;
    __syncthreads();
    if (t < n) sh.sortKeys[pos] = mine;
    __syncthreads();
    return;
  }
  for (int i = n + threadIdx.x; i < m; i += kQt3Threads) sh.sortKeys[i] = 0ull;
  __syncthreads();
  for (int k = 2; k <= m; k <<= 1) {
    for (int j = k >> 1; j > 0; j >>= 1) {
      for (int i = threadIdx.x; i < m; i += kQt3Threads) {
        const int p = i ^ j;
        if (p > i) {
          const unsigned long long a = sh.sortKeys[i], b = sh.sortKeys[p];
          const bool desc = ((i & k) == 0);
          if (desc ? (a < b) : (a > b)) { sh.sortKeys[i] = b; sh.sortKeys[p] = a; }
        }
      }
      __syncthreads();
    }
  }
}

template <bool LC>
struct Qt3Cands {
  const uint32_t* cg;
  uint16_t* og;
  uint32_t* cl;
  uint16_t* ol;
  __device__ __forceinline__ uint32_t cand(int p) const { return LC ? cl[p] : cg[p]; }
  __device__ __forceinline__ unsigned own(int p) const { return LC ? ol[p] : og[p]; }
  __device__ __forceinline__ void setOwn(int p, unsigned v) const {
    if (LC) ol[p] = (uint16_t)v;
    else og[p] = (uint16_t)v;
  }
};

template <int CAP, bool LC>
__device__ __forceinline__ void qt3_problem(const QtParams& Q, Qt3Shared<CAP>& sh, uint32_t* candL, uint16_t* ownL, const int level, const int f,
                                            const long long first, const int n) {
  constexpr int IPT = CAP >= kQt3Threads ? CAP / kQt3Threads : 1;
  const int tid = threadIdx.x;
  const int N = Q.nfeat[level];
  uint32_t* selCount = Q.selCount + (long long)f * kMaxLevels + level;
  uint32_t* selCountHost = Q.selCountHost ? Q.selCountHost + (long long)f * kMaxLevels + level : nullptr;
  SelKp* selHost = Q.selHost ? Q.selHost + (long long)f * Q.selPerFrame + Q.selOff[level] : nullptr;
  SelKp* selOut = Q.sel + (long long)f * Q.selPerFrame + Q.selOff[level];
  QT_STAMP(0);
  if (n <= 0) {
    if (tid == 0) {
      *selCount = 0;
      if (selCountHost) *selCountHost = 0;
    }
    return;
  }
  const long long eo = (long long)f * Q.candCap + first;
  const uint32_t* cand = Q.cand + eo;
  const Qt3Cands<LC> ca{cand, Q.own + eo, candL, ownL};
  Qt3Node* cur = sh.nodes[0];
  Qt3Node* nxt = sh.nodes[1];
  unsigned short* proc = sh.proc;
  const int maxX = Q.levW[level] - kBorder, maxY = Q.levH[level] - kBorder;
  const int nIni = (int)roundf(static_cast<float>(maxX - kBorder) / (maxY - kBorder));
  const float hX = static_cast<float>(maxX - kBorder) / nIni;
  int rootB[3];
#pragma unroll
  for (int k = 1; k <= 3; k++) {
    int b = 0x7fffffff;
    if (k < nIni) {
      b = (int)(hX * static_cast<float>(k));
      while (b > 0 && (int)((float)(b - 1) / hX) >= k) b--;
      while ((int)((float)b / hX) < k) b++;
    }
    rootB[k - 1] = b;
  }
  auto rootOf = [&](int x) { return (x >= rootB[0]) + (x >= rootB[1]) + (x >= rootB[2]); };
  int m = 0;
  uint32_t seq = 0;
  bool finalPhase = false;
  int nRec = 0;
  bool jumped = false;
  int T = 0, mT = nIni;
  if (Q.jump) {
    int mt = nIni;
    while (T < 3 && (T == 0 || 4 * mt <= N) && mt * 4 <= CAP) { mt *= 4; T++; }
    mT = mt;
  }
  QT_STAMP(1);
  if (T >= 2 && n >= 8 * mT) {
    int rl = 5;
    while (rl > 0 && (mT << rl) > CAP * 4) rl--;
    for (int i = tid; i < (mT << rl); i += kQt3Threads) sh.cnt[i] = 0u;
    const int yTop = maxY - kBorder;
    uint8_t* lutX = reinterpret_cast<uint8_t*>(sh.nodes[1]);
    uint8_t* lutY = lutX + ((Q.levW[level] + 15) & ~15);
    static_assert(sizeof(sh.nodes[1]) >= 8192 || CAP < 512, "axis tables of a 4095-pixel level");
    uint16_t* lutC = reinterpret_cast<uint16_t*>(sh.proc);
    const bool lutFits = ((Q.levW[level] + 15) & ~15) + Q.levH[level] <= (int)sizeof(sh.nodes[1]);
    uint32_t vNext[kQtEpt];
    auto loadJump = [&](int b) {
#pragma unroll
      for (int j = 0; j < kQtEpt; j++) vNext[j] = cand[min(b + j * kQt3Threads + tid, n - 1)];
    };
    loadJump(0);
    if (lutFits) {
      for (int xr = kBorder + tid; xr < maxX; xr += kQt3Threads) {
        const int x = xr - kBorder, r = rootOf(x);
        int x0 = (int)(hX * static_cast<float>(r)), x1 = (int)(hX * static_cast<float>(r + 1)), bits = 0;
        for (int t = 1; t <= T; t++) {
          const int midX = x0 + ((x1 - x0 + 1) >> 1), qx = x < midX ? 0 : 1;
          x0 = qx ? midX : x0; x1 = qx ? x1 : midX;
          bits = bits * 2 + qx;
        }
        lutX[xr] = (uint8_t)((r << 3) | bits);
      }
      for (int yr = kBorder + tid; yr < maxY; yr += kQt3Threads) {
        const int y = yr - kBorder;
        int y0 = 0, y1 = yTop, bits = 0;
        for (int t = 1; t <= T; t++) {
          const int midY = y0 + ((y1 - y0 + 1) >> 1), qy = y < midY ? 0 : 1;
          y0 = qy ? midY : y0; y1 = qy ? y1 : midY;
          bits = bits * 2 + qy;
        }
        lutY[yr] = (uint8_t)bits;
      }
      if (tid < 256) {
        const int r = tid >> 6, bx = (tid >> 3) & 7, by = tid & 7;
        int pos = r, mt = nIni, created = 0;
        for (int t = 1; t <= T; t++) {
          const int q = ((bx >> (T - t)) & 1) + 2 * ((by >> (T - t)) & 1);
          created = 4 * pos + q;
          mt *= 4;
          if (t < T) pos = (mt - 1) - created;
        }
        lutC[tid] = (uint16_t)created;
      }
    }
    __syncthreads();
    for (int b = 0; b < n; b += kQtEpt * kQt3Threads) {
      uint32_t v[kQtEpt];
#pragma unroll
      for (int j = 0; j < kQtEpt; j++) v[j] = vNext[j];
      if (b + kQtEpt * kQt3Threads < n) loadJump(b + kQtEpt * kQt3Threads);
      if (lutFits) {
        unsigned ex[kQtEpt], ey[kQtEpt], cr[kQtEpt];
#pragma unroll
        for (int j = 0; j < kQtEpt; j++) { ex[j] = lutX[v[j] & 0xfff]; ey[j] = lutY[(v[j] >> 12) & 0xfff]; }
#pragma unroll
        for (int j = 0; j < kQtEpt; j++) cr[j] = lutC[((ex[j] << 3) | ey[j]) & 255u];
#pragma unroll
        for (int j = 0; j < kQtEpt; j++) {
          const int p = b + j * kQt3Threads + tid;
          if (p < n) {
            if (LC) candL[p] = v[j];
            ca.setOwn(p, cr[j]);
            atomicAdd(&sh.cnt[(((unsigned)(mT - 1) - cr[j]) << rl) + (tid & ((1 << rl) - 1))], 1u);
          }
        }
        continue;
      }
#pragma unroll
      for (int j = 0; j < kQtEpt; j++) {
        const int p = b + j * kQt3Threads + tid;
        if (p < n) {
          const int x = (int)(v[j] & 0xfff) - kBorder, y = (int)((v[j] >> 12) & 0xfff) - kBorder;
          const int r = rootOf(x);
          int x0 = (int)(hX * static_cast<float>(r)), x1 = (int)(hX * static_cast<float>(r + 1)), y0 = 0, y1 = yTop;
          int pos = r, mt = nIni, created = 0, q = 0;
          for (int t = 1; t <= T; t++) {
            const int midX = x0 + ((x1 - x0 + 1) >> 1), midY = y0 + ((y1 - y0 + 1) >> 1);
            const int qx = x < midX ? 0 : 1, qy = y < midY ? 0 : 1;
            q = qx + 2 * qy;
            x0 = qx ? midX : x0; x1 = qx ? x1 : midX; y0 = qy ? midY : y0; y1 = qy ? y1 : midY;
            created = 4 * pos + q;
            mt *= 4;
            if (t < T) pos = (mt - 1) - created;
          }
          if (LC) candL[p] = v[j];
          ca.setOwn(p, (unsigned)created);
          atomicAdd(&sh.cnt[(((mT - 1) - created) << rl) + (tid & ((1 << rl) - 1))], 1u);
        }
      }
    }
    __syncthreads();
    QT_STAMP(2);
    int empty = 0;
    for (int g = tid; g < mT; g += kQt3Threads) {
      uint32_t t = 0;
      for (int k = 0; k < (1 << rl); k++) t += sh.cnt[(g << rl) + k];
      sh.cnt[g << rl] = t;
      empty |= t == 0u;
    }
    jumped = __syncthreads_or(empty) == 0;
    QT_STAMP(3);
    if (jumped) {
      const int mPrev = mT >> 2;
      uint32_t seqBase = (uint32_t)nIni;
      for (int t = 1, mt = nIni; t < T; t++) { mt *= 4; seqBase += (uint32_t)mt; }
      for (int p = tid; p < mT; p += kQt3Threads) {
        int digits[3], c = (mT - 1) - p, mt = mT;
        for (int t = T; t >= 1; t--) {
          digits[t - 1] = c & 3;
          const int parentPos = c >> 2;
          mt >>= 2;
          c = t > 1 ? (mt - 1) - parentPos : parentPos;
        }
        const int r = c;
// ... 207 lines not shown
#pragma unroll
      for (int k = 0; k < IPT; k++) {
        const int t = IPT * tid + k;
        if (t < nproc) {
          g += C[k] - 1;
          if (prevSize + g >= N) atomicMin(&sh.s_int[0], t);
        }
      }
      __syncthreads();
      cutT = sh.s_int[0];
    }
    if (tid == 0) sh.s_int[1] = 0;
    __syncthreads();
    {
      int pc = exC;
#pragma unroll
      for (int k = 0; k < IPT; k++) {
        const int t = IPT * tid + k;
        if (t < nproc) {
          if (t == cutT) sh.s_int[1] = pc + C[k];
          pc += C[k];
        }
      }
    }
    __syncthreads();
    const int T = sh.s_int[1];
    int keptFlag[IPT], locK = 0;
#pragma unroll
    for (int k = 0; k < IPT; k++) {
      const int i = IPT * tid + k;
      keptFlag[k] = 0;
      if (i < m) {
        const int t = sh.tproc[i];
        keptFlag[k] = (t < 0 || t > cutT) ? 1 : 0;
      }
      locK += keptFlag[k];
    }
    int totK;
    int exK = blockScanInt3<CAP>(sh, locK, totK);
    const int mNew = T + totK;
    {
      int pc = exC;
#pragma unroll
      for (int k = 0; k < IPT; k++) {
        const int t = IPT * tid + k;
        if (t < nproc) {
          const int id = proc[t];
          if (t <= cutT) {
            const Qt3Node nd = cur[id];
            const int midX = nd.x0 + ((nd.x1 - nd.x0 + 1) >> 1), midY = nd.y0 + ((nd.y1 - nd.y0 + 1) >> 1);
            uint32_t c[4];
            int nonEmptyAfter = 0;
            for (int q = 0; q < 4; q++) { c[q] = sh.cnt[(id * 4 + q) << rlog]; nonEmptyAfter += c[q] > 0; }
            const int groupBase = T - pc - C[k];
            int before = 0;
            for (int q = 0; q < 4; q++) {
              if (c[q] == 0) { sh.cpos[id][q] = 0xffff; continue; }
              nonEmptyAfter--;
              const int pos = groupBase + nonEmptyAfter;
              Qt3Node ch;
              ch.x0 = (q & 1) ? (short)midX : nd.x0;
              ch.x1 = (q & 1) ? nd.x1 : (short)midX;
              ch.y0 = (q & 2) ? (short)midY : nd.y0;
              ch.y1 = (q & 2) ? nd.y1 : (short)midY;
              ch.size = c[q];
              ch.seq = seq + (uint32_t)(pc + before);
              nxt[pos] = ch;
              sh.cpos[id][q] = (uint16_t)pos;
              before++;
            }
          }
          pc += C[k];
        }
      }
#pragma unroll
      for (int k = 0; k < IPT; k++) {
        const int i = IPT * tid + k;
        if (i < m && keptFlag[k]) {
          const int pos = T + exK++;
          nxt[pos] = cur[i];
          for (int q = 0; q < 4; q++) sh.cpos[i][q] = (uint16_t)pos;
        }
      }
    }
    __syncthreads();
    { Qt3Node* t2 = cur; cur = nxt; nxt = t2; }
    m = mNew;
    seq += (uint32_t)T;
    int recFlag[IPT], locR = 0;
#pragma unroll
    for (int k = 0; k < IPT; k++) {
      const int i = IPT * tid + k;
      recFlag[k] = (i < T && cur[i].size > 1) ? 1 : 0;
      locR += recFlag[k];
    }
    int totR;
    int exR = blockScanInt3<CAP>(sh, locR, totR);
#pragma unroll
    for (int k = 0; k < IPT; k++) {
      const int i = IPT * tid + k;
      if (recFlag[k]) {
        const Qt3Node nd = cur[i];
        sh.sortKeys[exR++] = ((unsigned long long)nd.size << 40) | ((unsigned long long)nd.seq << 16) | (unsigned long long)i;
      }
    }
    nRec = totR;
    __syncthreads();
    if (iter < 2) QT_STAMP(9 + 5 * iter);
    if (m >= N || m == prevSize) break;
    if (!finalPhase && m + 3 * totR > N) finalPhase = true;
    if (finalPhase && nRec == 0) break;
  }

  QT_STAMP(15);
  __syncthreads();
  for (int i = tid; i < m * 4; i += kQt3Threads) sh.cnt[i] = 0u;
  __syncthreads();
  for (int b = 0; b < n; b += kQtEpt * kQt3Threads) {
    uint32_t v[kQtEpt];
    unsigned ow[kQtEpt];
#pragma unroll
    for (int j = 0; j < kQtEpt; j++) {
      const int p = b + j * kQt3Threads + tid;
      v[j] = 0u;
      ow[j] = 0u;
      if (p < n) { ow[j] = ca.own(p); v[j] = ca.cand(p); }
    }
    unsigned id[kQtEpt];
#pragma unroll
    for (int j = 0; j < kQtEpt; j++) id[j] = (&sh.cpos[0][0])[ow[j] & (CAP * 4 - 1)];
#pragma unroll
    for (int j = 0; j < kQtEpt; j++) {
      const int p = b + j * kQt3Threads + tid;
      if (p < n) atomicMax(&sh.cnt[id[j] * 4 + (tid & 3)], ((v[j] >> 24) << 24) | (0xffffffu - (uint32_t)p));
    }
  }
  __syncthreads();
  QT_STAMP(16);
  for (int i = tid; i < m; i += kQt3Threads) {
    const uint4 b4 = *reinterpret_cast<const uint4*>(&sh.cnt[i * 4]);
    const uint32_t best = max(max(b4.x, b4.y), max(b4.z, b4.w));
    const uint32_t c = ca.cand((int)(0xffffffu - (best & 0xffffffu)));
    SelKp s;
    s.xy = (c & 0xfff) | (((c >> 12) & 0xfff) << 16);
    s.lf = (uint32_t)level | ((uint32_t)f << 8) | ((c >> 24) << 24);
    selOut[i] = s;
    if (selHost) selHost[i] = s;
  }
  QT_STAMP(17);
  if (tid == 0) {
    *selCount = (uint32_t)m;
    if (selCountHost) *selCountHost = (uint32_t)m;
  }
}

template <int CAP>
__global__ __launch_bounds__(kQt3Threads) void k_quadtree3(QtParams Q, int ldsCand) {
  __shared__ Qt3Shared<CAP> sh;
  extern __shared__ __align__(16) uint32_t qtDyn[];
  const int level = blockIdx.x, f = Q.frameBase + blockIdx.y;
  const uint32_t* ls = Q.levelStart + (long long)f * (kMaxLevels + 1);
  const long long first = Q.levelLocal ? Q.candBase[level] : (long long)ls[level];
  const int n = Q.levelLocal ? (int)ls[level] : (int)(ls[level + 1] - ls[level]);
  if (n <= ldsCand) qt3_problem<CAP, true>(Q, sh, qtDyn, reinterpret_cast<uint16_t*>(qtDyn + ldsCand), level, f, first, n);
  else qt3_problem<CAP, false>(Q, sh, nullptr, nullptr, level, f, first, n);
}

template <int CAP>
static int launch_qt3(const QtParams& Q, int nframes, hipStream_t st, int ldsBudget) {
  int ldsCand = 0;
  const int room = 156 * 1024 - (int)sizeof(Qt3Shared<CAP>);
  if (ldsBudget > room) ldsBudget = room;
  if (ldsBudget >= 6 * 1024) ldsCand = (ldsBudget / 6) & ~3;
  const int dynBytes = ldsCand * 6;
  if (dynBytes) {
    static std::mutex mu;
    static int attrBytes[64] = {};
    int dev = 0;
    if (hipGetDevice(&dev) != hipSuccess || dev < 0 || dev >= 64) return 1;
    std::lock_guard<std::mutex> lk(mu);
    if (dynBytes > attrBytes[dev]) {
      if (hipFuncSetAttribute(reinterpret_cast<const void*>(k_quadtree3<CAP>), hipFuncAttributeMaxDynamicSharedMemorySize,
                              dynBytes) != hipSuccess)
        return 1;
      attrBytes[dev] = dynBytes;
    }
  }
  hipLaunchKernelGGL(k_quadtree3<CAP>, dim3(Q.nlevels, nframes), dim3(kQt3Threads), dynBytes, st, Q, ldsCand);
  return 0;
}

int launch_quadtree(const QtParams& Q, int nframes, hipStream_t st, int ldsBudget) {
  int maxN = 0;
  for (int l = 0; l < Q.nlevels; l++) maxN = Q.nfeat[l] > maxN ? Q.nfeat[l] : maxN;
  if (maxN + 4 <= 512) return launch_qt3<512>(Q, nframes, st, ldsBudget);
  if (maxN + 4 <= 1024) return launch_qt3<1024>(Q, nframes, st, ldsBudget);
  return launch_qt3<2048>(Q, nframes, st, ldsBudget);
}

}

#ifdef ORBFE_EXPERIMENTS
extern "C" int orbfe_exp_qt_stamps(unsigned long long* out , int reset) {
  if (hipDeviceSynchronize() != hipSuccess) return 1;
  if (hipMemcpyFromSymbol(out, HIP_SYMBOL(orbfe::g_qtStamps), sizeof(unsigned long long) * orbfe::kMaxLevels * 32) != hipSuccess) return 1;
  if (reset) {
    static unsigned long long zeros[orbfe::kMaxLevels][32] = {};
    if (hipMemcpyToSymbol(HIP_SYMBOL(orbfe::g_qtStamps), zeros, sizeof zeros) != hipSuccess) return 1;
  }
  return 0;
}
#endif
```

os1_amd/csrc/orbfe_sfi.hip:

```cpp
#include <hip/hip_runtime.h>

#include <cstdlib>

#include "orbfe_internal.h"

namespace orbfe {

constexpr int kSfiGridCols = 64, kSfiGridRows = 48;
constexpr int kSfiThLow = 50, kSfiHisto = 30;

struct SfiFrame {
  const SelKp* sel;
  const float* angle;
  const uint8_t* desc;
  int n;
};

__device__ __forceinline__ SfiFrame sfi_frame(const SfiParams& S, int f) {
  SfiFrame F;
  if (f < 0) {
    F.sel = S.carrySel; F.angle = S.carryAngle; F.desc = S.carryDesc;
    F.n = S.carryCount ? (int)*S.carryCount : -1;
    if (F.n > S.n0cap) F.n = -1;
  } else {
    const long long base = (long long)f * S.selPerFrame;
    F.sel = S.sel + base; F.angle = S.angle + base; F.desc = S.desc + base * 32;
    F.n = (int)S.selCount[(long long)f * kMaxLevels];
  }
  return F;
}

__global__ __launch_bounds__(256) void k_sfi_sort(SfiParams S) {
  constexpr int kCells = kSfiGridCols * kSfiGridRows, kPer = kCells / 256;
  static_assert(kCells % 256 == 0, "cells per thread");
  extern __shared__ int dyn[];
  int* cellOf = dyn;
  int* arrival = dyn + S.n0cap;
  int* bucket = dyn + 2 * S.n0cap;
  __shared__ int start[kCells + 1];
  __shared__ int wsum[4];
  const int f = S.frameBase + blockIdx.x, tid = threadIdx.x;
  const SfiFrame F = sfi_frame(S, f);
  for (int c = tid; c <= kCells; c += 256) start[c] = 0;
  __syncthreads();
  for (int k = tid; k < F.n; k += 256) {
    const uint32_t xy = F.sel[k].xy;
    const float x = (float)(xy & 0xffff), y = (float)(xy >> 16);
    const int px = (int)roundf((x - S.minX) * S.invW), py = (int)roundf((y - S.minY) * S.invH);
    const int c = (px < 0 || px >= kSfiGridCols || py < 0 || py >= kSfiGridRows) ? -1 : px * kSfiGridRows + py;
    cellOf[k] = c;
    if (c >= 0) arrival[k] = atomicAdd(&start[c], 1);
  }
  __syncthreads();
  int loc[kPer], sum = 0;
#pragma unroll
  for (int i = 0; i < kPer; i++) { loc[i] = start[tid * kPer + i]; sum += loc[i]; }
  int incl = sum;
#pragma unroll
  for (int o = 1; o < 64; o <<= 1) {
    const int t = __shfl_up(incl, o, 64);
    if ((tid & 63) >= o) incl += t;
  }
  if ((tid & 63) == 63) wsum[tid >> 6] = incl;
  __syncthreads();
  int base = incl - sum;
  for (int w = 0; w < (tid >> 6); w++) base += wsum[w];
#pragma unroll
  for (int i = 0; i < kPer; i++) { start[tid * kPer + i] = base; base += loc[i]; }
  if (tid == 255) start[kCells] = base;
  __syncthreads();
  for (int k = tid; k < F.n; k += 256) {
    const int c = cellOf[k];
    if (c >= 0) bucket[start[c] + arrival[k]] = k;
  }
  __syncthreads();
  uint16_t* order = S.order + (long long)f * S.n0cap;
  for (int k = tid; k < F.n; k += 256) {
    const int c = cellOf[k];
    if (c < 0) continue;
    const int b0 = start[c], b1 = start[c + 1];
    int rank = 0;
    for (int j = b0; j < b1; j++) rank += bucket[j] < k;
    order[b0 + rank] = (uint16_t)k;
  }
  if (tid == 0) S.orderCount[f] = start[kCells];
}

__global__ __launch_bounds__(64) void k_sfi_candidates(SfiParams S) {
  const int i1 = blockIdx.x, fr = blockIdx.y, lane = threadIdx.x;
  const int f = S.frameBase + fr;
  const SfiFrame F2 = sfi_frame(S, f);
  const SfiFrame F1 = sfi_frame(S, fr == 0 ? -1 : f - 1);
  uint32_t* cnt = S.pcount + (long long)f * S.n0cap + i1;
  if (F1.n < 0 || i1 >= F1.n) {
    if (lane == 0 && i1 < S.n0cap) *cnt = 0;
    return;
  }
  const uint32_t qxy = F1.sel[i1].xy;
  const float x = (float)(qxy & 0xffff), y = (float)(qxy >> 16), r = S.window;
  uint32_t qd[8];
  const uint32_t* qp = reinterpret_cast<const uint32_t*>(F1.desc + (long long)i1 * 32);
#pragma unroll
  for (int w = 0; w < 8; w++) qd[w] = qp[w];
  const uint16_t* order = S.order + (long long)f * S.n0cap;
  const int nin = S.orderCount[f];
  uint32_t* pool = S.pool + ((long long)f * S.n0cap + i1) * S.n0cap;
  const unsigned long long below = (1ull << lane) - 1ull;
  int run = 0;
  for (int e0 = 0; e0 < nin; e0 += 64) {
    const int e = e0 + lane;
    bool ok = false;
    int i2 = 0;
    if (e < nin) {
      i2 = order[e];
      const uint32_t xy = F2.sel[i2].xy;
      const float dx = (float)(xy & 0xffff) - x, dy = (float)(xy >> 16) - y;
      ok = fabsf(dx) < r && fabsf(dy) < r;
    }
    const unsigned long long m = __ballot(ok);
    if (ok) {
      const uint32_t* dp = reinterpret_cast<const uint32_t*>(F2.desc + (long long)i2 * 32);
      int d = 0;
#pragma unroll
      for (int w = 0; w < 8; w++) d += __popc(dp[w] ^ qd[w]);
      pool[run + __popcll(m & below)] = (uint32_t)i2 | ((uint32_t)d << 16);
    }
    run += __popcll(m);
  }
  if (lane == 0) *cnt = (uint32_t)run;
}

__device__ __forceinline__ int sfi_rot_bin(float a1, float a2) {
  const float factor = 1.0f / kSfiHisto;
  float rot = a1 - a2;
  if (rot < 0.0f) rot += 360.0f;
  int bin = (int)roundf(rot * factor);
  if (bin == kSfiHisto) bin = 0;
  return bin;
}


__device__ int* g_sfiDbg;
constexpr int kSfiDbgRecords = 1 << 16;

template <class PoolAt>
__device__ void sfi_serial_outcomes(int lane, int n1, const int* pcnt, PoolAt poolAt, float nnratio, int* vmd, int* M) {
  for (int i1 = 0; i1 < n1; i1++) {
    const int cnt = pcnt[i1];
    int bestDist = 0x7fffffff, bestDist2 = 0x7fffffff, bestIdx2 = -1;
    for (int c0 = 0; c0 < cnt; c0 += 64) {
      int d = 0x7fffffff, i2 = -1;
      if (c0 + lane < cnt) {
        const uint32_t entry = poolAt(i1, c0 + lane);
        i2 = (int)(entry & 0xffff);
        const int dist = (int)(entry >> 16);
        if (!(vmd[i2] <= dist)) d = dist;
      }
      const unsigned dd = (d == 0x7fffffff) ? 511u : (unsigned)d;
      unsigned long long c1 = ~0ull;
#pragma unroll
      for (int b = 8; b >= 0; b--) {
        const unsigned long long z = __ballot(((dd >> b) & 1u) == 0u) & c1;
        if (z) c1 = z;
      }
      const int ml = (int)__builtin_ctzll(c1);
      const unsigned d1 = (unsigned)__shfl((int)dd, ml, 64);
      unsigned long long c2 = ~(1ull << ml);
#pragma unroll
      for (int b = 8; b >= 0; b--) {
        const unsigned long long z = __ballot(((dd >> b) & 1u) == 0u) & c2;
        if (z) c2 = z;
      }
      const unsigned d2 = (unsigned)__shfl((int)dd, (int)__builtin_ctzll(c2), 64);
      const int md = d1 >= 511u ? 0x7fffffff : (int)d1;
      const int sd = d2 >= 511u ? 0x7fffffff : (int)d2;
      const int mi2 = __shfl(i2, ml, 64);
      if (md < bestDist) { bestDist2 = min(bestDist, sd); bestDist = md; bestIdx2 = mi2; }
      else bestDist2 = min(bestDist2, md);
    }
    int m = -1;
    if (bestDist <= kSfiThLow && (float)bestDist < (float)bestDist2 * nnratio) {
      m = bestIdx2 | (bestDist << 16);
      if (lane == 0) vmd[bestIdx2] = bestDist;
    }
    if (lane == 0) M[i1] = m;
    asm volatile("s_waitcnt lgkmcnt(0)" ::: "memory");
  }
}

template <int kSfiThreads>
__global__ __launch_bounds__(kSfiThreads) void k_sfi_resolve(SfiParams S, int ldsPool, int maxRounds) {
  extern __shared__ int sm[];
  const int fr = blockIdx.x, tid = threadIdx.x;
  const unsigned long long tStart = g_sfiDbg ? __builtin_amdgcn_s_memtime() : 0ull;
  int dbgSerial = 0;
  const int f = S.frameBase + fr;
  const SfiFrame F2 = sfi_frame(S, f);
  const SfiFrame F1 = sfi_frame(S, fr == 0 ? -1 : f - 1);
  int32_t* out = S.matches12 + (long long)f * S.n0cap;
  if (F1.n < 0) {
    for (int i = tid; i < S.n0cap; i += kSfiThreads) out[i] = -1;
    if (tid == 0) S.nmatches[f] = 0;
    return;
  }
  const int n1 = F1.n, n2 = F2.n, cap = S.n0cap;
  int* Mbuf[2] = {sm, sm + cap};
  int* head = sm + 2 * cap;
  int* next = sm + 3 * cap;
  int* off = sm + 4 * cap;
  int* pcnt = sm + 5 * cap + 1;
  int* hist = sm + 6 * cap + 1;
  int* misc = hist + 32;
  uint32_t* lpool = reinterpret_cast<uint32_t*>(misc + 2);
  for (int i = tid; i < cap; i += kSfiThreads) {
    Mbuf[0][i] = -1;
    pcnt[i] = i < n1 ? (int)S.pcount[(long long)f * cap + i] : 0;
  }
  if (tid < 32) hist[tid] = 0;
  if (tid == 32) misc[0] = 0;
  __syncthreads();
  if (tid < 64) {
    int run = 0;
    for (int b = 0; b < cap; b += 64) {
      const int v = b + tid < cap ? pcnt[b + tid] : 0;
      int s = v;
#pragma unroll
      for (int o = 1; o < 64; o <<= 1) {
        const int t = __shfl_up(s, o, 64);
        if (tid >= o) s += t;
      }
      if (b + tid < cap) off[b + tid] = run + s - v;
      run += __shfl(s, 63, 64);
    }
    if (tid == 0) off[cap] = run;
  }
  __syncthreads();
  const uint32_t* gpool = S.pool + (long long)f * cap * cap;
  const int total = off[cap];
  const bool inLds = total <= ldsPool;
  if (inLds) {
    for (int e = tid; e < total; e += kSfiThreads) {
      int lo = 0, hi = n1 - 1;
      while (lo < hi) {
        const int mid = (lo + hi + 1) >> 1;
        if (off[mid] <= e) lo = mid; else hi = mid - 1;
      }
      lpool[e] = gpool[(long long)lo * cap + (e - off[lo])];
    }
  }
  __syncthreads();
  int cur = 0, rounds = 0;
  for (;;) {
    const int* M = Mbuf[cur];
    int* Mn = Mbuf[cur ^ 1];
    for (int i = tid; i < n2; i += kSfiThreads) head[i] = -1;
    __syncthreads();
    for (int j = tid; j < n1; j += kSfiThreads) {
      const int m = M[j];
      if (m >= 0) next[j] = atomicExch(&head[m & 0xffff], j);
    }
    __syncthreads();
    int changed = 0;
    for (int i1 = tid; i1 < n1; i1 += kSfiThreads) {
      const int cnt = pcnt[i1];
      int bestDist = 0x7fffffff, bestDist2 = 0x7fffffff, bestIdx2 = -1;
      for (int c = 0; c < cnt; c++) {
        const uint32_t entry = inLds ? lpool[off[i1] + c] : gpool[(long long)i1 * cap + c];
        const int i2 = (int)(entry & 0xffff), dist = (int)(entry >> 16);
        int vmd = 0x7fffffff;
        for (int j = head[i2]; j >= 0; j = next[j])
          if (j < i1) vmd = min(vmd, M[j] >> 16);
        if (vmd <= dist) continue;
        if (dist < bestDist) { bestDist2 = bestDist; bestDist = dist; bestIdx2 = i2; }
        else if (dist < bestDist2) bestDist2 = dist;
      }
      int m = -1;
      if (bestDist <= kSfiThLow && (float)bestDist < (float)bestDist2 * S.nnratio) m = bestIdx2 | (bestDist << 16);
      Mn[i1] = m;
      changed |= m != M[i1];
    }
    const int any = __syncthreads_or(changed);
    cur ^= 1;
    if (!any) break;
    if (++rounds >= maxRounds) {
      dbgSerial = 1;
      int* M2 = Mbuf[cur];
      int* vmd = head;
      for (int i = tid; i < n2; i += kSfiThreads) vmd[i] = 0x7fffffff;
      __syncthreads();
      if (tid < 64) {
        if (inLds) sfi_serial_outcomes(tid, n1, pcnt, [&](int q, int c) { return lpool[off[q] + c]; }, S.nnratio, vmd, M2);
        else sfi_serial_outcomes(tid, n1, pcnt, [&](int q, int c) { return gpool[(long long)q * cap + c]; }, S.nnratio, vmd, M2);
      }
      __syncthreads();
      for (int i = tid; i < n2; i += kSfiThreads) head[i] = -1;
      __syncthreads();
      for (int j = tid; j < n1; j += kSfiThreads) {
        const int m = M2[j];
        if (m >= 0) next[j] = atomicExch(&head[m & 0xffff], j);
      }
      __syncthreads();
      break;
    }
  }
  const int* M = Mbuf[cur];
  int* vn12 = Mbuf[cur ^ 1];
  int* binOf = off;
  __syncthreads();
  for (int j = tid; j < n1; j += kSfiThreads) {
    const int m = M[j];
    int v = -1, bin = -1;
    if (m >= 0) {
      const int i2 = m & 0xffff;
      bool last = true;
      for (int k = head[i2]; k >= 0; k = next[k]) last = last && k <= j;
      if (last) v = i2;
      if (S.checkOri) {
        bin = sfi_rot_bin(F1.angle[j], F2.angle[i2]);
        atomicAdd(&hist[bin], 1);
      }
    }
    vn12[j] = v;
    binOf[j] = bin;
  }
  __syncthreads();
  int ind1 = -1, ind2 = -1, ind3 = -1;
  if (S.checkOri) {
    int max1 = 0, max2 = 0, max3 = 0;
    for (int i = 0; i < kSfiHisto; i++) {
      const int s = hist[i];
      if (s > max1) { max3 = max2; max2 = max1; max1 = s; ind3 = ind2; ind2 = ind1; ind1 = i; }
      else if (s > max2) { max3 = max2; max2 = s; ind3 = ind2; ind2 = i; }
      else if (s > max3) { max3 = s; ind3 = i; }
    }
    if (max2 < 0.1f * (float)max1) { ind2 = -1; ind3 = -1; }
    else if (max3 < 0.1f * (float)max1) { ind3 = -1; }
  }
  int nm = 0;
  for (int i = tid; i < cap; i += kSfiThreads) {
    int v = -1;
    if (i < n1) {
      v = vn12[i];
      const int b = binOf[i];
      if (S.checkOri && b >= 0 && b != ind1 && b != ind2 && b != ind3) v = -1;
    }
    out[i] = v;
    nm += v >= 0;
  }
#pragma unroll
  for (int o = 32; o > 0; o >>= 1) nm += __shfl_xor(nm, o, 64);
  if ((tid & 63) == 0 && nm) atomicAdd(&misc[0], nm);
  __syncthreads();
  if (tid == 0) S.nmatches[f] = misc[0];
  if (g_sfiDbg && tid == 0) {
    const int r = atomicAdd(&g_sfiDbg[0], 1);
    if (r < kSfiDbgRecords) {
      int* rec = g_sfiDbg + 8 + 8 * r;
      rec[0] = f; rec[1] = rounds; rec[2] = total; rec[3] = dbgSerial;
      rec[4] = (int)(__builtin_amdgcn_s_memtime() - tStart); rec[5] = n1; rec[6] = n2; rec[7] = inLds;
    }
  }
}

static int* s_sfiDbg = nullptr;
static void sfi_debug_setup() {
  static bool done = false;
  if (done) return;
  done = true;
  if (!ORBFE_EXP_ENV("ORBFE_SFI_DEBUG")) return;
  if (hipMalloc((void**)&s_sfiDbg, sizeof(int) * (8 + 8 * kSfiDbgRecords)) != hipSuccess) { s_sfiDbg = nullptr; return; }
  (void)hipMemset(s_sfiDbg, 0, sizeof(int) * (8 + 8 * kSfiDbgRecords));
  (void)hipMemcpyToSymbol(HIP_SYMBOL(g_sfiDbg), &s_sfiDbg, sizeof s_sfiDbg);
}
int sfi_debug_read(int* out, int capRecords, int reset) {
  if (!s_sfiDbg) return 0;
  int n = 0;
  if (hipMemcpy(&n, s_sfiDbg, sizeof(int), hipMemcpyDeviceToHost) != hipSuccess) return -1;
  n = std::min(std::min(n, kSfiDbgRecords), capRecords);
  if (n > 0 && hipMemcpy(out, s_sfiDbg + 8, sizeof(int) * 8 * (size_t)n, hipMemcpyDeviceToHost) != hipSuccess) return -1;
  if (reset) (void)hipMemset(s_sfiDbg, 0, sizeof(int));
  return n;
}

__global__ __launch_bounds__(256) void k_sfi_carry(SfiParams S, int lastFrame, SelKp* cSel, float* cAngle, uint8_t* cDesc,
                                                   uint32_t* cCount) {
  const long long base = (long long)lastFrame * S.selPerFrame;
  const int i = blockIdx.x * 256 + threadIdx.x;
  if (i < S.n0cap) {
    cSel[i] = S.sel[base + i];
    cAngle[i] = S.angle[base + i];
  }
  if (i < S.n0cap * 8)
    reinterpret_cast<uint32_t*>(cDesc)[i] = reinterpret_cast<const uint32_t*>(S.desc + base * 32)[i];
  if (i == 0) *cCount = S.selCount[(long long)lastFrame * kMaxLevels];
}

void launch_sfi_carry(const SfiParams& S, int lastFrame, SelKp* cSel, float* cAngle, uint8_t* cDesc, uint32_t* cCount,
                      hipStream_t st) {
  hipLaunchKernelGGL(k_sfi_carry, dim3((S.n0cap * 8 + 255) / 256), dim3(256), 0, st, S, lastFrame, cSel, cAngle, cDesc, cCount);
}

void launch_sfi(const SfiParams& S, int nframes, hipStream_t st) {
  sfi_debug_setup();
  hipLaunchKernelGGL(k_sfi_sort, dim3(nframes), dim3(256), sizeof(int) * 3 * S.n0cap, st, S);
  hipLaunchKernelGGL(k_sfi_candidates, dim3(S.n0cap, nframes), dim3(64), 0, st, S);
  const int fixedWords = 6 * S.n0cap + 1 + 32 + 2;
  int ldsPool = (60 * 1024 / 4) - fixedWords;
  if (ldsPool > 8192) ldsPool = 8192;
  if (const char* e = ORBFE_EXP_ENV("ORBFE_SFI_LDS_POOL")) ldsPool = std::min(ldsPool, std::max(0, atoi(e)));
  if (ldsPool < 0) ldsPool = 0;
  int maxRounds = 32;
  if (const char* e = getenv("ORBFE_SFI_MAX_ROUNDS")) maxRounds = atoi(e) < 1 ? 1 : atoi(e);
  static const int threads = [] { const char* e = ORBFE_EXP_ENV("ORBFE_SFI_THREADS"); return e ? atoi(e) : 512; }();
  if (threads == 256)
    hipLaunchKernelGGL(k_sfi_resolve<256>, dim3(nframes), dim3(256), sizeof(int) * (fixedWords + ldsPool), st, S, ldsPool, maxRounds);
  else
    hipLaunchKernelGGL(k_sfi_resolve<512>, dim3(nframes), dim3(512), sizeof(int) * (fixedWords + ldsPool), st, S, ldsPool, maxRounds);
}

}
```

Measured before the change: 89320.

## Fuse SFI grid sort into quadtree and carry copy into describe kernel

The per-cell grid ordering of level-0 keypoints for the matcher now happens inside the quadtree kernel on large images, so the separate k_sfi_sort launch is skipped there. The describe kernel writes the last frame's keypoints, angles and descriptors straight into the chain carry buffers, and quadtree writes the carry count, which removes the k_sfi_carry kernel. The carry ring grows from 2 to 8 slots with consumed/ready events, so extraction of the next batch can overlap matching of the previous one. The cost is extra work and LDS reuse inside quadtree, more event bookkeeping, and a new debug counter.

Result: slower. 88410 (-1.0%).

```diff
diff --git a/include/orbfe.h b/include/orbfe.h
--- a/include/orbfe.h
+++ b/include/orbfe.h
@@ -98,6 +98,7 @@
 int orbfe_debug_set_profiling(orbfe_extractor* h, int enable);
 int orbfe_debug_fast_stamps(orbfe_extractor* h, unsigned long long out[8], int reset);
 int orbfe_debug_sfi_records(orbfe_extractor* h, int32_t* out, int cap_records, int* n_out, int reset);
+int orbfe_debug_sfi_serial_finishes(int device, long long* count, int reset);
 int orbfe_debug_sincos(orbfe_extractor* h, const float* angle_deg, int n, float* cos_out, float* sin_out);
 
 int orbfe_debug_quadtree(const int16_t* x, const int16_t* y, const uint8_t* score, int n, int min_x, int max_x,
diff --git a/os1_amd/api.py b/os1_amd/api.py
--- a/os1_amd/api.py
+++ b/os1_amd/api.py
@@ -228,6 +228,14 @@
     return load_library().orbfe_device_count()
 
 
+def sfi_serial_finishes(device=0, reset=False):
+    L = load_library()
+    L.orbfe_debug_sfi_serial_finishes.argtypes = [C.c_int, C.POINTER(C.c_longlong), C.c_int]
+    n = C.c_longlong()
+    _check(L.orbfe_debug_sfi_serial_finishes(int(device), C.byref(n), int(reset)))
+    return n.value
+
+
 def hamming(a, b):
     a = np.ascontiguousarray(a, np.uint8)
     b = np.ascontiguousarray(b, np.uint8)
diff --git a/os1_amd/csrc/orbfe_extractor.hip b/os1_amd/csrc/orbfe_extractor.hip
--- a/os1_amd/csrc/orbfe_extractor.hip
+++ b/os1_amd/csrc/orbfe_extractor.hip
@@ -37,16 +37,14 @@
 void launch_spin(unsigned long long ticks, hipStream_t st);
 void launch_describe_slots(const PyramidParams& P, const SelKp* sel, int nslots, float* angle, uint8_t* desc,
                            const uint32_t* selCount, int selPerFrame, const int* selOff, hipStream_t st, bool fourWaves, float* angle2 = nullptr,
-                           uint8_t* desc2 = nullptr);
+                           uint8_t* desc2 = nullptr, const DescribeCarry* carry = nullptr);
 int launch_quadtree(const QtParams& Q, int nframes, hipStream_t st, int ldsBudget);
 int bow_launch_descend(orbfe_vocabulary* v, const uint8_t* d_desc, int n, int levelsup, uint2* d_out, hipStream_t st);
 int bow_assemble(orbfe_vocabulary* v, const uint2* ln, int n, uint32_t* bow_ids, double* bow_values, int* n_words,
                  uint32_t* fv_nodes, uint32_t* fv_offsets, uint32_t* fv_features, int* n_fv_nodes,
                  uint32_t* word_of_feature, uint32_t* node_of_feature);
 int bow_device(const orbfe_vocabulary* v);
-void launch_sfi(const SfiParams& S, int nframes, hipStream_t st);
-void launch_sfi_carry(const SfiParams& S, int lastFrame, SelKp* cSel, float* cAngle, uint8_t* cDesc, uint32_t* cCount,
-                      hipStream_t st);
+void launch_sfi(const SfiParams& S, int nframes, hipStream_t st, bool sorted);
 
 thread_local std::string g_err;
 void set_err(const char* fmt, ...) {
@@ -112,13 +110,16 @@
 }
 
 struct orbfe_sfi_chain {
+  static constexpr int kSlots = 8;
   int device = 0, n0cap = 0;
-  DevBuf<SelKp> sel[2];
-  DevBuf<float> angle[2];
-  DevBuf<uint8_t> desc[2];
+  DevBuf<SelKp> sel[kSlots];
+  DevBuf<float> angle[kSlots];
+  DevBuf<uint8_t> desc[kSlots];
   DevBuf<uint32_t> count;
-  hipEvent_t ready[2] = {};
+  hipEvent_t ready[kSlots] = {}, consumed[kSlots] = {};
+  bool consumedRecorded[kSlots] = {};
   long long seq = 0;
+  long long ring = 0;
   bool isolated = false;
   bool restart = false;
   orbfe_matcher* hostMatcher = nullptr;
@@ -128,7 +129,11 @@
   ~orbfe_sfi_chain() {
     (void)hipSetDevice(device);
     if (hostMatcher) orbfe_matcher_destroy(hostMatcher);
-    for (int i = 0; i < 2; i++) { sel[i].release(); angle[i].release(); desc[i].release(); if (ready[i]) (void)hipEventDestroy(ready[i]); }
+    for (int i = 0; i < kSlots; i++) {
+      sel[i].release(); angle[i].release(); desc[i].release();
+      if (ready[i]) (void)hipEventDestroy(ready[i]);
+      if (consumed[i]) (void)hipEventDestroy(consumed[i]);
+    }
     count.release();
   }
 };
@@ -721,6 +726,44 @@
     const bool localCand = small && localLists;
     submitLocalCand = localCand;
     QP.levelLocal = localCand ? 1 : 0;
+    orbfe_sfi_chain* chain = ms ? ms->chain : nullptr;
+    SfiParams SP{};
+    DescribeCarry carry{};
+    QP.sfiOrder = nullptr; QP.sfiOrderCount = nullptr; QP.sfiN0cap = 0; QP.carryCount = nullptr; QP.carryFrame = -1;
+    int slotCur = 0, slotPrev = 0;
+    bool chainOut = false, chainIn = false;
+    if (chain) {
+      orbfe_sfi_chain& ch = *chain;
+      constexpr int kSlots = orbfe_sfi_chain::kSlots;
+      const int n0cap = selOff[1] - selOff[0];
+      if (ch.n0cap != n0cap || ch.device != device) { set_err("match chain belongs to a different extractor configuration"); return ORBFE_ERR_INVALID; }
+      if ((rc = d_sfiOrder.ensure((size_t)batchCap * n0cap))) return rc;
+      if ((rc = d_sfiOrderCount.ensure(batchCap))) return rc;
+      if ((rc = d_sfiPool.ensure((size_t)batchCap * n0cap * n0cap))) return rc;
+      if ((rc = d_sfiPcount.ensure((size_t)batchCap * n0cap))) return rc;
+      SP.sel = d_sel.p; SP.angle = d_angle.p; SP.desc = d_desc.p; SP.selCount = d_selCount.p;
+      SP.selPerFrame = selPerFrame; SP.n0cap = n0cap; SP.frameBase = 0;
+      slotCur = (int)(ch.ring % kSlots); slotPrev = (int)((ch.ring + kSlots - 1) % kSlots);
+      SP.carrySel = ch.sel[slotPrev].p; SP.carryAngle = ch.angle[slotPrev].p; SP.carryDesc = ch.desc[slotPrev].p;
+      const bool iso = ch.isolated;
+      chainOut = !iso;
+      chainIn = ch.seq > 0 && !iso && !ch.restart;
+      SP.carryCount = ch.count.p + (chainIn ? slotPrev : kSlots);
+      SP.minX = ms->bounds[0]; SP.minY = ms->bounds[2];
+      SP.invW = static_cast<float>(64) / static_cast<float>(ms->bounds[1] - ms->bounds[0]);
+      SP.invH = static_cast<float>(48) / static_cast<float>(ms->bounds[3] - ms->bounds[2]);
+      SP.window = (float)ms->window; SP.nnratio = ms->nnratio; SP.checkOri = ms->checkOri;
+      SP.order = d_sfiOrder.p; SP.orderCount = d_sfiOrderCount.p; SP.pool = d_sfiPool.p; SP.pcount = d_sfiPcount.p;
+      SP.matches12 = kernelOut ? h_m12.p : d_m12.p; SP.nmatches = kernelOut ? h_nm.p : d_nm.p;
+      if (!small) {
+        QP.sfiOrder = SP.order; QP.sfiOrderCount = SP.orderCount; QP.sfiN0cap = n0cap;
+        QP.sfiMinX = SP.minX; QP.sfiMinY = SP.minY; QP.sfiInvW = SP.invW; QP.sfiInvH = SP.invH;
+      }
+      if (chainOut) {
+        QP.carryCount = ch.count.p + slotCur; QP.carryFrame = nframes - 1;
+        carry.sel = ch.sel[slotCur].p; carry.angle = ch.angle[slotCur].p; carry.desc = ch.desc[slotCur].p; carry.frame = nframes - 1;
+      }
+    }
     {
       if (prof) HIP_TRY(hipEventRecord(ev[0][0], st));
       if (launch_pyramid(P, nframes, st, coneOk && small ? &cone : (tailOk && !small ? &coneTail : nullptr))) { set_err("cannot configure the pyramid kernel"); return ORBFE_ERR_HIP; }
@@ -732,14 +775,16 @@
       if (localCand) launch_compact_local(P, nframes, st, 0, nlevels);
       else launch_compact(P, nframes, st);
       if (prof) HIP_TRY(hipEventRecord(ev[0][3], st));
+      if (chainOut && chain->consumedRecorded[slotCur]) HIP_TRY(hipStreamWaitEvent(st, chain->consumed[slotCur], 0));
       if (prof) HIP_TRY(hipEventRecord(evQt[0], st));
       if (launch_quadtree(QP, nframes, st, qtLds)) { set_err("cannot configure the quadtree kernel"); return ORBFE_ERR_HIP; }
       if (prof) HIP_TRY(hipEventRecord(evQt[1], st));
       if (prof) HIP_TRY(hipEventRecord(ev[0][4], st));
       launch_describe_slots(P, d_sel.p, nframes * selPerFrame, angOut, descOut, d_selCount.p, selPerFrame, selOff, st, four,
-                            kernelOut ? h_angle.p : nullptr, kernelOut ? h_desc.p : nullptr);
+                            kernelOut ? h_angle.p : nullptr, kernelOut ? h_desc.p : nullptr, chainOut ? &carry : nullptr);
       if (prof) HIP_TRY(hipEventRecord(ev[0][5], st));
       HIP_TRY(hipGetLastError());
+      if (chainOut) HIP_TRY(hipEventRecord(chain->ready[slotCur], st));
     }
     const int nslots = nframes * selPerFrame;
     pendingBow = false;
@@ -750,37 +795,17 @@
       pendingBow = true;
     }
     pendingMatched = false;
-    if (ms && ms->chain) {
-      orbfe_sfi_chain& ch = *ms->chain;
-      const int n0cap = selOff[1] - selOff[0];
-      if (ch.n0cap != n0cap || ch.device != device) { set_err("match chain belongs to a different extractor configuration"); return ORBFE_ERR_INVALID; }
-      if ((rc = d_sfiOrder.ensure((size_t)batchCap * n0cap))) return rc;
-      if ((rc = d_sfiOrderCount.ensure(batchCap))) return rc;
-      if ((rc = d_sfiPool.ensure((size_t)batchCap * n0cap * n0cap))) return rc;
-      if ((rc = d_sfiPcount.ensure((size_t)batchCap * n0cap))) return rc;
-      SfiParams SP{};
-      SP.sel = d_sel.p; SP.angle = d_angle.p; SP.desc = d_desc.p; SP.selCount = d_selCount.p;
-      SP.selPerFrame = selPerFrame; SP.n0cap = n0cap; SP.frameBase = 0;
-      const int prev = (int)((ch.seq + 1) & 1), cur = (int)(ch.seq & 1);
-      SP.carrySel = ch.sel[prev].p; SP.carryAngle = ch.angle[prev].p; SP.carryDesc = ch.desc[prev].p;
-      const bool iso = ch.isolated;
-      SP.carryCount = ch.count.p + ((ch.seq == 0 || iso || ch.restart) ? 2 : prev);
-      ch.restart = false;
-      SP.minX = ms->bounds[0]; SP.minY = ms->bounds[2];
-      SP.invW = static_cast<float>(64) / static_cast<float>(ms->bounds[1] - ms->bounds[0]);
-      SP.invH = static_cast<float>(48) / static_cast<float>(ms->bounds[3] - ms->bounds[2]);
-      SP.window = (float)ms->window; SP.nnratio = ms->nnratio; SP.checkOri = ms->checkOri;
-      SP.order = d_sfiOrder.p; SP.orderCount = d_sfiOrderCount.p; SP.pool = d_sfiPool.p; SP.pcount = d_sfiPcount.p;
-      SP.matches12 = kernelOut ? h_m12.p : d_m12.p; SP.nmatches = kernelOut ? h_nm.p : d_nm.p;
-      if (ch.seq > 0 && !iso) HIP_TRY(hipStreamWaitEvent(st, ch.ready[prev], 0));
-      launch_sfi(SP, nframes, st);
+    if (chain) {
+      if (chainIn) HIP_TRY(hipStreamWaitEvent(st, chain->ready[slotPrev], 0));
+      launch_sfi(SP, nframes, st, !small);
       HIP_TRY(hipGetLastError());
-      if (!iso) {
-        launch_sfi_carry(SP, nframes - 1, ch.sel[cur].p, ch.angle[cur].p, ch.desc[cur].p, ch.count.p + cur, st);
-        HIP_TRY(hipGetLastError());
-        HIP_TRY(hipEventRecord(ch.ready[cur], st));
-      }
-      ch.seq++;
+      if (chainIn) {
+        HIP_TRY(hipEventRecord(chain->consumed[slotPrev], st));
+        chain->consumedRecorded[slotPrev] = true;
+      }
+      chain->restart = false;
+      chain->seq++;
+      chain->ring++;
       pendingMatched = true;
     }
     if (!zeroCopy && !kernelOut) HIP_TRY(hipMemcpyAsync(h_outArena.p, d_outArena.p, outArenaBytes, hipMemcpyDeviceToHost, st));
@@ -1412,7 +1437,13 @@
   if (orbfe::fast_stamps(out, reset)) { set_err("reading the stamp counters failed"); return ORBFE_ERR_HIP; }
   return ORBFE_OK;
 }
-extern "C++" { namespace orbfe { int sfi_debug_read(int* out, int capRecords, int reset); } }
+extern "C++" { namespace orbfe { int sfi_debug_read(int* out, int capRecords, int reset); int sfi_serial_finishes(long long* out, int reset); } }
+int orbfe_debug_sfi_serial_finishes(int device, long long* count, int reset) {
+  if (!count) { set_err("NULL argument"); return ORBFE_ERR_INVALID; }
+  HIP_TRY(hipSetDevice(device));
+  if (orbfe::sfi_serial_finishes(count, reset)) { set_err("cannot read the serial-finish counter"); return ORBFE_ERR_HIP; }
+  return ORBFE_OK;
+}
 int orbfe_debug_sfi_records(orbfe_extractor* h, int32_t* out, int cap_records, int* n_out, int reset) {
   if (!h || !out || !n_out || cap_records < 0) { set_err("NULL argument"); return ORBFE_ERR_INVALID; }
   HIP_TRY(hipSetDevice(h->device));
@@ -1602,15 +1633,17 @@
   c->device = h->device;
   c->n0cap = h->selOff[1] - h->selOff[0];
   int rc = ORBFE_OK;
-  for (int i = 0; i < 2 && rc == ORBFE_OK; i++) {
+  for (int i = 0; i < orbfe_sfi_chain::kSlots && rc == ORBFE_OK; i++) {
     if ((rc = c->sel[i].ensure(c->n0cap))) break;
     if ((rc = c->angle[i].ensure(c->n0cap))) break;
     if ((rc = c->desc[i].ensure((size_t)c->n0cap * 32))) break;
-    if (hipEventCreateWithFlags(&c->ready[i], hipEventDisableTiming) != hipSuccess) { set_err("hipEventCreate failed"); rc = ORBFE_ERR_HIP; }
-  }
-  if (rc == ORBFE_OK) rc = c->count.ensure(4);
+    if (hipEventCreateWithFlags(&c->ready[i], hipEventDisableTiming) != hipSuccess ||
+        hipEventCreateWithFlags(&c->consumed[i], hipEventDisableTiming) != hipSuccess) { set_err("hipEventCreate failed"); rc = ORBFE_ERR_HIP; }
+  }
+  if (rc == ORBFE_OK) rc = c->count.ensure(orbfe_sfi_chain::kSlots + 1);
   if (rc == ORBFE_OK) {
-    const uint32_t init[4] = {0xffffffffu, 0xffffffffu, 0xffffffffu, 0xffffffffu};
+    uint32_t init[orbfe_sfi_chain::kSlots + 1];
+    for (uint32_t& v : init) v = 0xffffffffu;
     if (hipMemcpy(c->count.p, init, sizeof init, hipMemcpyHostToDevice) != hipSuccess) { set_err("hipMemcpy failed"); rc = ORBFE_ERR_HIP; }
   }
   if (rc != ORBFE_OK) { delete c; return rc; }
diff --git a/os1_amd/csrc/orbfe_internal.h b/os1_amd/csrc/orbfe_internal.h
--- a/os1_amd/csrc/orbfe_internal.h
+++ b/os1_amd/csrc/orbfe_internal.h
@@ -94,6 +94,13 @@
   uint32_t lf;
 };
 
+struct DescribeCarry {
+  SelKp* sel;
+  float* angle;
+  uint8_t* desc;
+  int frame;
+};
+
 struct ExtractView {
   const SelKp* sel;
   const float* angle;
@@ -105,6 +112,14 @@
   void* stream;
 };
 
+constexpr int kSfiGridCols = 64, kSfiGridRows = 48;
+#ifdef __HIPCC__
+__device__ __forceinline__ int sfi_grid_cell(uint32_t xy, float minX, float minY, float invW, float invH) {
+  const float x = (float)(xy & 0xffff), y = (float)(xy >> 16);
+  const int px = (int)roundf((x - minX) * invW), py = (int)roundf((y - minY) * invH);
+  return (px < 0 || px >= kSfiGridCols || py < 0 || py >= kSfiGridRows) ? -1 : px * kSfiGridRows + py;
+}
+#endif
 struct SfiParams {
   const SelKp* sel;
   const float* angle;
@@ -144,6 +159,12 @@
   int jump;
   int levelLocal;
   long long candBase[kMaxLevels];
+  uint16_t* sfiOrder;
+  int* sfiOrderCount;
+  int sfiN0cap;
+  float sfiMinX, sfiMinY, sfiInvW, sfiInvH;
+  uint32_t* carryCount;
+  int carryFrame;
 };
 
 
diff --git a/os1_amd/csrc/orbfe_kernels.hip b/os1_amd/csrc/orbfe_kernels.hip
--- a/os1_amd/csrc/orbfe_kernels.hip
+++ b/os1_amd/csrc/orbfe_kernels.hip
@@ -782,6 +782,10 @@
   uint8_t* descOut;
   float* angleOut2;
   uint8_t* descOut2;
+  SelKp* carrySel;
+  float* carryAngle;
+  uint8_t* carryDesc;
+  int carryBase, carryN;
   const uint8_t* const* frame0;
   const uint8_t* frameInline[2];
   long long stride0;
@@ -1036,18 +1040,28 @@
     words[j] = __ballot(t0 < t1);
   }
   uint8_t* descOut2 = A.descOut2;
+  const unsigned ci = (unsigned)(k - A.carryBase);
+  uint8_t* carryDesc = (A.carryDesc && ci < (unsigned)A.carryN) ? A.carryDesc + (long long)ci * 32 : nullptr;
   if (WAVES == 4) {
     if (lane == 0) {
       reinterpret_cast<unsigned long long*>(descOut + (long long)k * 32)[wave] = words[wave];
       if (descOut2) reinterpret_cast<unsigned long long*>(descOut2 + (long long)k * 32)[wave] = words[wave];
+      if (carryDesc) reinterpret_cast<unsigned long long*>(carryDesc)[wave] = words[wave];
     }
   } else if (lane < 4) {
     reinterpret_cast<unsigned long long*>(descOut + (long long)k * 32)[lane] = words[lane];
     if (descOut2) reinterpret_cast<unsigned long long*>(descOut2 + (long long)k * 32)[lane] = words[lane];
+    if (carryDesc) reinterpret_cast<unsigned long long*>(carryDesc)[lane] = words[lane];
   }
   if (tid == 0) {
     angleOut[k] = angle;
     if (A.angleOut2) A.angleOut2[k] = angle;
+    if (carryDesc) {
+      A.carryAngle[ci] = angle;
+      SelKp s;
+      s.xy = sw.x; s.lf = sw.y;
+      A.carrySel[ci] = s;
+    }
   }
 }
 
@@ -1234,11 +1248,16 @@
 
 void launch_describe_slots(const PyramidParams& P, const SelKp* sel, int nslots, float* angle, uint8_t* desc,
                            const uint32_t* selCount, int selPerFrame, const int* selOff, hipStream_t st, bool fourWaves, float* angle2,
-                           uint8_t* desc2) {
+                           uint8_t* desc2, const DescribeCarry* carry) {
   if (nslots <= 0) return;
   DescribeArgs A = describe_args(P, sel, nslots, angle, desc);
   A.angleOut2 = angle2;
   A.descOut2 = desc2;
+  if (carry && carry->desc) {
+    A.carrySel = carry->sel; A.carryAngle = carry->angle; A.carryDesc = carry->desc;
+    A.carryBase = carry->frame * selPerFrame + selOff[0];
+    A.carryN = selOff[1] - selOff[0];
+  }
   A.selCount = selCount;
   A.selPerFrame = selPerFrame;
   for (int l = 0; l <= P.nlevels; l++) A.selOff[l] = selOff[l];
diff --git a/os1_amd/csrc/orbfe_quadtree.hip b/os1_amd/csrc/orbfe_quadtree.hip
--- a/os1_amd/csrc/orbfe_quadtree.hip
+++ b/os1_amd/csrc/orbfe_quadtree.hip
@@ -132,7 +132,7 @@
 };
 
 template <int CAP, bool LC>
-__device__ __forceinline__ void qt3_problem(const QtParams& Q, Qt3Shared<CAP>& sh, uint32_t* candL, uint16_t* ownL, const int level, const int f,
+__device__ __forceinline__ int qt3_problem(const QtParams& Q, Qt3Shared<CAP>& sh, uint32_t* candL, uint16_t* ownL, const int level, const int f,
                                             const long long first, const int n) {
   constexpr int IPT = CAP >= kQt3Threads ? CAP / kQt3Threads : 1;
   const int tid = threadIdx.x;
@@ -147,7 +147,7 @@
       *selCount = 0;
       if (selCountHost) *selCountHost = 0;
     }
-    return;
+    return 0;
   }
   const long long eo = (long long)f * Q.candCap + first;
   const uint32_t* cand = Q.cand + eo;
@@ -661,6 +661,57 @@
     *selCount = (uint32_t)m;
     if (selCountHost) *selCountHost = (uint32_t)m;
   }
+  return m;
+}
+
+template <int CAP>
+__device__ void qt3_sfi_order(const QtParams& Q, Qt3Shared<CAP>& sh, const int f, int n) {
+  constexpr int kCells = kSfiGridCols * kSfiGridRows, kPer = kCells / kQt3Threads;
+  static_assert(kCells % kQt3Threads == 0, "cells per thread");
+  static_assert(sizeof(sh.nodes) >= sizeof(int) * (kCells + 1), "cell starts in the node arrays");
+  int* start = reinterpret_cast<int*>(&sh.nodes[0][0]);
+  int* cellOf = reinterpret_cast<int*>(sh.sortKeys);
+  int* arrival = cellOf + CAP;
+  int* bucket = reinterpret_cast<int*>(sh.cnt);
+  const int tid = threadIdx.x;
+  n = min(n, min(Q.sfiN0cap, CAP));
+  const SelKp* sel = Q.sel + (long long)f * Q.selPerFrame + Q.selOff[0];
+  __syncthreads();
+  for (int c = tid; c <= kCells; c += kQt3Threads) start[c] = 0;
+  __syncthreads();
+  for (int k = tid; k < n; k += kQt3Threads) {
+    const int c = sfi_grid_cell(sel[k].xy, Q.sfiMinX, Q.sfiMinY, Q.sfiInvW, Q.sfiInvH);
+    cellOf[k] = c;
+    if (c >= 0) arrival[k] = atomicAdd(&start[c], 1);
+  }
+  __syncthreads();
+  int loc[kPer], sum = 0;
+#pragma unroll
+  for (int i = 0; i < kPer; i++) { loc[i] = start[tid * kPer + i]; sum += loc[i]; }
+  const int incl = wave_incl_scan_i(sum);
+  if ((tid & 63) == 63) sh.wsumI[tid >> 6] = incl;
+  __syncthreads();
+  int base = incl - sum;
+  for (int w = 0; w < (tid >> 6); w++) base += sh.wsumI[w];
+#pragma unroll
+  for (int i = 0; i < kPer; i++) { start[tid * kPer + i] = base; base += loc[i]; }
+  if (tid == kQt3Threads - 1) start[kCells] = base;
+  __syncthreads();
+  for (int k = tid; k < n; k += kQt3Threads) {
+    const int c = cellOf[k];
+    if (c >= 0) bucket[start[c] + arrival[k]] = k;
+  }
+  __syncthreads();
+  uint16_t* order = Q.sfiOrder + (long long)f * Q.sfiN0cap;
+  for (int k = tid; k < n; k += kQt3Threads) {
+    const int c = cellOf[k];
+    if (c < 0) continue;
+    const int b0 = start[c], b1 = start[c + 1];
+    int rank = 0;
+    for (int j = b0; j < b1; j++) rank += bucket[j] < k;
+    order[b0 + rank] = (uint16_t)k;
+  }
+  if (tid == 0) Q.sfiOrderCount[f] = start[kCells];
 }
 
 template <int CAP>
@@ -671,8 +722,13 @@
   const uint32_t* ls = Q.levelStart + (long long)f * (kMaxLevels + 1);
   const long long first = Q.levelLocal ? Q.candBase[level] : (long long)ls[level];
   const int n = Q.levelLocal ? (int)ls[level] : (int)(ls[level + 1] - ls[level]);
-  if (n <= ldsCand) qt3_problem<CAP, true>(Q, sh, qtDyn, reinterpret_cast<uint16_t*>(qtDyn + ldsCand), level, f, first, n);
-  else qt3_problem<CAP, false>(Q, sh, nullptr, nullptr, level, f, first, n);
+  int m;
+  if (n <= ldsCand) m = qt3_problem<CAP, true>(Q, sh, qtDyn, reinterpret_cast<uint16_t*>(qtDyn + ldsCand), level, f, first, n);
+  else m = qt3_problem<CAP, false>(Q, sh, nullptr, nullptr, level, f, first, n);
+  if (level == 0) {
+    if (Q.carryCount && f == Q.carryFrame && threadIdx.x == 0) *Q.carryCount = (uint32_t)m;
+    if (Q.sfiOrder) qt3_sfi_order<CAP>(Q, sh, f, m);
+  }
 }
 
 template <int CAP>
diff --git a/os1_amd/csrc/orbfe_sfi.hip b/os1_amd/csrc/orbfe_sfi.hip
--- a/os1_amd/csrc/orbfe_sfi.hip
+++ b/os1_amd/csrc/orbfe_sfi.hip
@@ -6,7 +6,6 @@
 
 namespace orbfe {
 
-constexpr int kSfiGridCols = 64, kSfiGridRows = 48;
 constexpr int kSfiThLow = 50, kSfiHisto = 30;
 
 struct SfiFrame {
@@ -44,10 +43,7 @@
   for (int c = tid; c <= kCells; c += 256) start[c] = 0;
   __syncthreads();
   for (int k = tid; k < F.n; k += 256) {
-    const uint32_t xy = F.sel[k].xy;
-    const float x = (float)(xy & 0xffff), y = (float)(xy >> 16);
-    const int px = (int)roundf((x - S.minX) * S.invW), py = (int)roundf((y - S.minY) * S.invH);
-    const int c = (px < 0 || px >= kSfiGridCols || py < 0 || py >= kSfiGridRows) ? -1 : px * kSfiGridRows + py;
+    const int c = sfi_grid_cell(F.sel[k].xy, S.minX, S.minY, S.invW, S.invH);
     cellOf[k] = c;
     if (c >= 0) arrival[k] = atomicAdd(&start[c], 1);
   }
@@ -141,6 +137,7 @@
 
 
 __device__ int* g_sfiDbg;
+__device__ unsigned g_sfiSerialFinishes;
 constexpr int kSfiDbgRecords = 1 << 16;
 
 template <class PoolAt>
@@ -352,6 +349,7 @@
   if ((tid & 63) == 0 && nm) atomicAdd(&misc[0], nm);
   __syncthreads();
   if (tid == 0) S.nmatches[f] = misc[0];
+  if (dbgSerial && tid == 0) atomicAdd(&g_sfiSerialFinishes, 1u);
   if (g_sfiDbg && tid == 0) {
     const int r = atomicAdd(&g_sfiDbg[0], 1);
     if (r < kSfiDbgRecords) {
@@ -382,40 +380,41 @@
   return n;
 }
 
-__global__ __launch_bounds__(256) void k_sfi_carry(SfiParams S, int lastFrame, SelKp* cSel, float* cAngle, uint8_t* cDesc,
-                                                   uint32_t* cCount) {
-  const long long base = (long long)lastFrame * S.selPerFrame;
-  const int i = blockIdx.x * 256 + threadIdx.x;
-  if (i < S.n0cap) {
-    cSel[i] = S.sel[base + i];
-    cAngle[i] = S.angle[base + i];
-  }
-  if (i < S.n0cap * 8)
-    reinterpret_cast<uint32_t*>(cDesc)[i] = reinterpret_cast<const uint32_t*>(S.desc + base * 32)[i];
-  if (i == 0) *cCount = S.selCount[(long long)lastFrame * kMaxLevels];
-}
-
-void launch_sfi_carry(const SfiParams& S, int lastFrame, SelKp* cSel, float* cAngle, uint8_t* cDesc, uint32_t* cCount,
-                      hipStream_t st) {
-  hipLaunchKernelGGL(k_sfi_carry, dim3((S.n0cap * 8 + 255) / 256), dim3(256), 0, st, S, lastFrame, cSel, cAngle, cDesc, cCount);
-}
-
-void launch_sfi(const SfiParams& S, int nframes, hipStream_t st) {
+int sfi_serial_finishes(long long* out, int reset) {
+  unsigned v = 0;
+  if (hipDeviceSynchronize() != hipSuccess) return -1;
+  if (hipMemcpyFromSymbol(&v, HIP_SYMBOL(g_sfiSerialFinishes), sizeof v) != hipSuccess) return -1;
+  if (reset) {
+    const unsigned zero = 0;
+    if (hipMemcpyToSymbol(HIP_SYMBOL(g_sfiSerialFinishes), &zero, sizeof zero) != hipSuccess) return -1;
+  }
+  *out = (long long)v;
+  return 0;
+}
+
+#ifndef ORBFE_SFI_RESOLVE_THREADS
+#define ORBFE_SFI_RESOLVE_THREADS 512
+#endif
+#ifndef ORBFE_SFI_RESOLVE_LDS_POOL
+#define ORBFE_SFI_RESOLVE_LDS_POOL 8192
+#endif
+
+void launch_sfi(const SfiParams& S, int nframes, hipStream_t st, bool sorted) {
   sfi_debug_setup();
-  hipLaunchKernelGGL(k_sfi_sort, dim3(nframes), dim3(256), sizeof(int) * 3 * S.n0cap, st, S);
+  if (!sorted) hipLaunchKernelGGL(k_sfi_sort, dim3(nframes), dim3(256), sizeof(int) * 3 * S.n0cap, st, S);
   hipLaunchKernelGGL(k_sfi_candidates, dim3(S.n0cap, nframes), dim3(64), 0, st, S);
   const int fixedWords = 6 * S.n0cap + 1 + 32 + 2;
   int ldsPool = (60 * 1024 / 4) - fixedWords;
-  if (ldsPool > 8192) ldsPool = 8192;
-  if (const char* e = ORBFE_EXP_ENV("ORBFE_SFI_LDS_POOL")) ldsPool = std::min(ldsPool, std::max(0, atoi(e)));
+  if (ldsPool > ORBFE_SFI_RESOLVE_LDS_POOL) ldsPool = ORBFE_SFI_RESOLVE_LDS_POOL;
+  if (const char* e = ORBFE_EXP_ENV("ORBFE_SFI_LDS_POOL")) ldsPool = std::min((60 * 1024 / 4) - fixedWords, std::min(8192, std::max(0, atoi(e))));
   if (ldsPool < 0) ldsPool = 0;
   int maxRounds = 32;
   if (const char* e = getenv("ORBFE_SFI_MAX_ROUNDS")) maxRounds = atoi(e) < 1 ? 1 : atoi(e);
-  static const int threads = [] { const char* e = ORBFE_EXP_ENV("ORBFE_SFI_THREADS"); return e ? atoi(e) : 512; }();
-  if (threads == 256)
-    hipLaunchKernelGGL(k_sfi_resolve<256>, dim3(nframes), dim3(256), sizeof(int) * (fixedWords + ldsPool), st, S, ldsPool, maxRounds);
-  else
-    hipLaunchKernelGGL(k_sfi_resolve<512>, dim3(nframes), dim3(512), sizeof(int) * (fixedWords + ldsPool), st, S, ldsPool, maxRounds);
-}
-
-}
+  static const int threads = [] { const char* e = ORBFE_EXP_ENV("ORBFE_SFI_THREADS"); return e ? atoi(e) : ORBFE_SFI_RESOLVE_THREADS; }();
+  const size_t lds = sizeof(int) * (fixedWords + ldsPool);
+  if (threads == 128) hipLaunchKernelGGL(k_sfi_resolve<128>, dim3(nframes), dim3(128), lds, st, S, ldsPool, maxRounds);
+  else if (threads == 256) hipLaunchKernelGGL(k_sfi_resolve<256>, dim3(nframes), dim3(256), lds, st, S, ldsPool, maxRounds);
+  else hipLaunchKernelGGL(k_sfi_resolve<512>, dim3(nframes), dim3(512), lds, st, S, ldsPool, maxRounds);
+}
+
+}
```
